# nanoporetech/isONclust2

Hardware: AMD Instinct MI355X
Metric: reads/s clustered (sahlin mode, k=11 w=15) (higher is better)
Workload: dtype u32

## Files before the change

### include/isonclust2_hip.h

```cpp
#ifndef ISONCLUST2_HIP_H
#define ISONCLUST2_HIP_H

#include <stddef.h>
#include <stdint.h>

#ifdef __cplusplus
extern "C" {
#endif

typedef struct ioc_ctx ioc_ctx;

typedef enum {
    IOC_OK = 0,
    IOC_ERR_ARG = -1,
    IOC_ERR_HIP = -2,
    IOC_ERR_STATE = -3,
    IOC_ERR_CAPACITY = -4,
    IOC_ERR_TABLE = -5,
    IOC_ERR_NO_DEVICE = -6,
    IOC_ERR_INPUT = -7
} ioc_status;

enum { IOC_MODE_SAHLIN = 0, IOC_MODE_FAST = 1, IOC_MODE_FURIOUS = 2, IOC_MODE_NONE = 3 };

typedef struct {
    int32_t k;
    int32_t w;
    int32_t min_shared;
    int32_t mode;
    double min_fraction;
    double mapped_threshold;
    double min_prob_no_hits;
    double aligned_threshold;
} ioc_params;

int ioc_ctx_create(int device, ioc_ctx** out);
void ioc_ctx_destroy(ioc_ctx* ctx);
int ioc_ctx_trim(ioc_ctx* ctx);
int ioc_ctx_prewarm(ioc_ctx* ctx, int32_t alignment_mode);
const char* ioc_last_error(const ioc_ctx* ctx);
int ioc_set_stream(ioc_ctx* ctx, void* hip_stream);
int ioc_synchronize(ioc_ctx* ctx);

int ioc_set_params(ioc_ctx* ctx, const ioc_params* p, const int32_t gap_limit[225]);

int ioc_queries_upload(ioc_ctx* ctx, int32_t n, const int64_t* off_fwd, const int64_t* off_rev,
                       const uint32_t* min_val, const uint32_t* min_pos, int64_t total,
                       const uint32_t* hpc_len, const uint8_t* err_cell, const uint32_t* min_total);
int ioc_queries_bind_device(ioc_ctx* ctx, int32_t n, const int64_t* d_off_fwd, const int64_t* d_off_rev,
                            const uint32_t* d_min_val, const uint32_t* d_min_pos, int64_t total,
                            const uint32_t* d_hpc_len, const uint8_t* d_err_cell,
                            const uint32_t* d_min_total, const int64_t* h_off_fwd,
                            const int64_t* h_off_rev);

int ioc_left_load(ioc_ctx* ctx, int32_t n_clusters, const uint8_t* cls_err_cell, int64_t n_keys,
                  const uint32_t* keys, const int64_t* offs, const uint32_t* postings);

int ioc_index_update(ioc_ctx* ctx, int32_t cls, const uint32_t* old_min, int64_t n_old, const uint32_t* new_min,
                     int64_t n_new, uint8_t new_err_cell);
int ioc_left_export(ioc_ctx* ctx, int64_t* n_keys, int64_t* n_postings, uint32_t* keys, int64_t* offs,
                    uint32_t* postings);

int ioc_index_build(ioc_ctx* ctx);
int ioc_score(ioc_ctx* ctx);
int ioc_resolve(ioc_ctx* ctx, int32_t* n_iter);
int ioc_get_decisions(ioc_ctx* ctx, int32_t* target, int8_t* strand, uint8_t* flags);
int ioc_get_cuts(ioc_ctx* ctx, int32_t* cut);
int ioc_force_decision(ioc_ctx* ctx, int32_t query, int32_t target, int32_t strand);
int ioc_clear_forced(ioc_ctx* ctx);
int ioc_set_aln_verdicts(ioc_ctx* ctx, const int32_t* target, const int8_t* strand);
#define IOC_TIE_SLOTS 16
int ioc_get_ties(ioc_ctx* ctx, uint32_t* count, uint32_t* keys);

int ioc_scored_candidates(ioc_ctx* ctx, int32_t q, int32_t cap, uint32_t* key, uint32_t* size);
int ioc_query_candidates(ioc_ctx* ctx, int32_t query, int32_t cap, int32_t* target, int8_t* strand,
                         uint32_t* size, uint32_t* first_index, uint32_t* total_mapped);

int ioc_index_export(ioc_ctx* ctx, int64_t* n_keys, int64_t* n_postings, uint32_t* keys,
                     int64_t* offs, uint32_t* postings);

int ioc_qual_scores(ioc_ctx* ctx, int32_t n, const int64_t* offs, const uint8_t* qual, int32_t k,
                    double* score, double* err_rate);
int ioc_extract_minimizers(ioc_ctx* ctx, int32_t n, const int64_t* offs, const uint8_t* seq,
                           const uint8_t* qual, int32_t k, int32_t w, uint32_t* hpc_len,
                           double* hpc_err, int64_t* off_fwd, int64_t* off_rev, int32_t* status);
int ioc_extracted_hpc_download(ioc_ctx* ctx, char* hpc_seq, char* hpc_qual, int64_t cap);
int ioc_extracted_download(ioc_ctx* ctx, uint32_t* min_val, uint32_t* min_pos, int64_t cap);
int ioc_queries_from_extracted(ioc_ctx* ctx, const uint8_t* keep, const uint8_t* err_cell,
                               const uint32_t* min_total);

typedef struct {
    float ms_build;
    float ms_score;
    float ms_resolve;
    int32_t resolve_iters;
    int32_t n_queries;
    int64_t n_minimizers;
    int64_t n_index_postings;
    int64_t n_candidates;
    int64_t n_mapped_evals;
    int64_t postings_traversed;
    float ms_align_fwd;
    float ms_align_trace;
    int64_t n_align_pairs;
    int64_t n_align_cells;
    int64_t n_align_refused;
    int32_t score_oob;
    int32_t score_oob_probe;
    int64_t align_arena_bytes;
    int32_t align_slices;
    int32_t align_version;
    int64_t n_align_cells_computed;
} ioc_timings;
int ioc_get_timings(ioc_ctx* ctx, ioc_timings* out);
int ioc_count_reference_postings(ioc_ctx* ctx, int64_t* n_postings);

int ioc_host_gap_limits(const char* table_path, int32_t k, int32_t w, double min_prob_no_hits,
                        int32_t* gap_limit, double* p_shared);
uint8_t ioc_host_err_cell(double err_rate);
uint32_t ioc_host_min_total(uint32_t hpc_len, double mapped_threshold);

int ioc_host_align(const char* query, int32_t qlen, const char* ref, int32_t rlen, int32_t match,
                   int32_t mismatch, int32_t gap_open, int32_t gap_extend, char* comp, int32_t comp_cap,
                   int32_t* score_out);
int ioc_host_align_ops(const char* query, int32_t qlen, const char* ref, int32_t rlen, int32_t match,
                       int32_t mismatch, int32_t gap_open, int32_t gap_extend, char* ops, int32_t ops_cap,
                       int32_t* score_out);
int64_t ioc_host_ops_to_cigar(const char* ops, int64_t len, char* out, int64_t cap);
int32_t ioc_host_gap_open(double e1_plus_e2);
double ioc_host_aln_ratio(const char* comp, int32_t comp_len, double e, uint32_t slen, uint32_t k);

typedef struct {
    int32_t query;
    int32_t ref;
    int32_t ref_revcomp;
    int32_t reserved;
    double e;
} ioc_aln_pair;
int ioc_align_set_pool(ioc_ctx* ctx, int32_t n_seqs, const char* seqs, const int64_t* offs);
int ioc_align_pairs(ioc_ctx* ctx, int32_t n_pairs, const ioc_aln_pair* pairs, int32_t k, int32_t match,
                    int32_t mismatch, int32_t gap_extend, int32_t* out_score, int64_t* out_windows,
                    double* out_ratio);
int64_t ioc_align_ops_bound(ioc_ctx* ctx, int32_t n_pairs, const ioc_aln_pair* pairs);
int ioc_align_pairs_ops(ioc_ctx* ctx, int32_t n_pairs, const ioc_aln_pair* pairs, int32_t k, int32_t match,
                        int32_t mismatch, int32_t gap_extend, int32_t* out_score, int64_t* out_windows,
                        double* out_ratio, char* out_ops, int64_t ops_cap, int64_t* ops_off);
int ioc_align_set_verdict_threshold(ioc_ctx* ctx, double aligned_threshold);

int64_t ioc_queries_generation(const ioc_ctx* ctx);
int64_t ioc_gather_records_device(ioc_ctx* ctx, int32_t n_idx, const int32_t* entries, uint32_t* d_out_min,
                                  uint32_t* d_out_pos, int64_t cap, int64_t* off_fwd, int64_t* off_rev);

typedef struct {
    int32_t n;
    const int64_t* off_fwd;
    const int64_t* off_rev;
    const uint32_t* min_val;
    const uint32_t* min_pos;
    int64_t total;
    const uint32_t* raw_len;
    const uint32_t* hpc_len;
    const double* score;
    const double* raw_err;
    const double* hpc_err;
    const uint8_t* state;
    double min_qual;
    const char* raw_seq;
    const int64_t* raw_off;
    const int32_t* n_members;
    int32_t depth;
    int32_t min_cls_size;
    const uint8_t* is_cluster;
    int32_t minimizers_on_device;
} ioc_batch_view;

typedef struct {
    int32_t n_clusters;
    const double* cls_hpc_err;
    int64_t n_keys;
    const uint32_t* keys;
    const int64_t* offs;
    const uint32_t* postings;
    const char* rep_seq;
    const int64_t* rep_off;
    const double* cls_raw_err;
} ioc_left_view;

typedef struct {
    int64_t n_clusters;
    int64_t n_joined;
    int64_t n_gated;
    int64_t n_tie_replays;
    int64_t n_aln_invoked;
    int32_t resolve_iters;
    int32_t aln_rounds;
    int64_t n_aln_pairs;
    int64_t n_aln_order_dep;
    int64_t n_cons_invoked;
    int64_t n_cons_restarts;
} ioc_cluster_stats;

int ioc_cluster_batch(ioc_ctx* ctx, const ioc_params* p, const char* table_path,
                      const ioc_batch_view* right, int32_t* out_cls, int8_t* out_strand,
                      ioc_cluster_stats* stats);
int ioc_cluster_merge(ioc_ctx* ctx, const ioc_params* p, const char* table_path, const ioc_left_view* left,
                      const ioc_batch_view* right, int32_t* out_cls, int8_t* out_strand,
                      ioc_cluster_stats* stats);
typedef struct {
    const char* raw_seq;
    int32_t raw_len;
    char raw_qual;
    double raw_err;
    double raw_score;
    const char* hpc_seq;
    int32_t hpc_len;
    double hpc_err;
    const uint32_t* fwd_min;
    const uint32_t* fwd_pos;
    int32_t n_fwd;
    const uint32_t* rev_min;
    const uint32_t* rev_pos;
    int32_t n_rev;
    int32_t entry;
} ioc_rep_record;
typedef struct {
    void* user;
    int (*create)(void* user, int side, int idx, const char* seq, int len);
    int (*size)(void* user, int side, int idx);
    int (*add)(void* user, int side, int idx, const char* seq, int len, unsigned weight);
    int (*consensus)(void* user, int side, int idx, char* out, int cap);
    int (*purge)(void* user, int side, int idx, const char* seq, int len, unsigned weight);
    void (*rep_changed)(void* user, int32_t cls, const ioc_rep_record* rec);
    const struct ioc_consensus_spec_ops* spec;
} ioc_consensus_ops;
typedef struct ioc_consensus_spec_ops {
    int (*create_tagged)(void* user, int side, int idx, const char* seq, int len, int tag);
    int (*add_tagged)(void* user, int side, int idx, const char* seq, int len, unsigned weight, int tag);
    int (*consensus_deferred)(void* user, int side, int idx, int tag);
    int (*flush)(void* user, int safe_tag);
    int (*collect)(void* user, int side, int idx, int tag, char* out, int cap);
    int (*rollback)(void* user, int first_tag);
    int (*commit)(void* user);
} ioc_consensus_spec_ops;
typedef struct {
    int32_t cons_min_size;
    int32_t cons_max_size;
    int32_t cons_period;
    int32_t left_depth;
    const int32_t* left_sizes;
} ioc_consensus_args;
int ioc_cluster_consensus(ioc_ctx* ctx, const ioc_params* p, const char* table_path, const ioc_left_view* left,
                          const ioc_batch_view* right, const ioc_consensus_args* args, const ioc_consensus_ops* ops,
                          int32_t* out_cls, int8_t* out_strand, ioc_cluster_stats* stats);

#define IOC_POA_LOCAL 0
#define IOC_POA_GLOBAL 1
#define IOC_POA_SEMI_GLOBAL 2
typedef struct ioc_poa ioc_poa;
int ioc_poa_create(ioc_ctx* ctx, int32_t m, int32_t n, int32_t g, int32_t e, int32_t q, int32_t c, ioc_poa** out);
int ioc_poa_create_mode(ioc_ctx* ctx, int32_t mode, int32_t m, int32_t n, int32_t g, int32_t e, int32_t q, int32_t c, ioc_poa** out);
void ioc_poa_destroy(ioc_poa* poa);
void ioc_poa_bind(ioc_poa* poa, ioc_consensus_ops* ops);
int ioc_poa_graph_export(ioc_poa* poa, int side, int idx, int32_t* n_nodes, int32_t* n_edges, char* bases, int32_t* rank,
                         int32_t* edge_from, int32_t* edge_to, int64_t* edge_w);
int ioc_poa_last_alignment(ioc_poa* poa, int32_t cap, int32_t* nodes, int32_t* pos, int32_t* score);
int64_t ioc_poa_graph_save(ioc_poa* poa, int side, int idx, uint8_t* out, int64_t cap);
int ioc_poa_graph_load(ioc_poa* poa, int side, int idx, const uint8_t* in, int64_t len);
int ioc_poa_graph_load_many(ioc_poa* poa, int side, int32_t count, const int32_t* idx, const uint8_t* const* in, const int64_t* len);

int ioc_cluster_resident(ioc_ctx* ctx, int32_t* out_cls, int8_t* out_strand, ioc_cluster_stats* stats);
int ioc_resident_set_sequences(ioc_ctx* ctx, const char* raw_seq, const int64_t* raw_off, const double* raw_err);

#define IOC_DIST_ID_BYTES 128
int ioc_dist_unique_id(uint8_t* id );
int ioc_dist_init(ioc_ctx* ctx, const uint8_t* id, int32_t rank, int32_t world);
int ioc_dist_shutdown(ioc_ctx* ctx);
int ioc_dist_info(const ioc_ctx* ctx, int32_t* rank, int32_t* world);
int ioc_dist_allgather_device(ioc_ctx* ctx, const void* d_send, void* d_recv, int64_t bytes_per_rank);
int ioc_dist_allgatherv_device(ioc_ctx* ctx, const void* d_send, void* d_recv, const int64_t* counts, const int64_t* displs,
                               int32_t esize);
int ioc_dist_allgather_i64(ioc_ctx* ctx, int64_t mine, int64_t* all );
int ioc_dist_allgatherv_host(ioc_ctx* ctx, const void* send, int64_t bytes, void* recv, int64_t* sizes);
int ioc_dist_allreduce_max(ioc_ctx* ctx, double* x);
int ioc_dist_barrier(ioc_ctx* ctx);
typedef struct {
    float ms_exchange_lists;
    double ms_merge;
    int64_t bytes_lists;
    int64_t bytes_records;
    int32_t sharded;
    int32_t exchanges;
} ioc_dist_merge_times;
#define IOC_XCHG_MAX_U8 0
#define IOC_XCHG_MIN_U32 1
#define IOC_XCHG_SUM_I32 2
typedef int (*ioc_exchange_fn)(void* user, void* d_buf, int64_t count, int32_t kind, void* hip_stream);
int ioc_set_shard(ioc_ctx* ctx, int32_t world, int32_t rank, ioc_exchange_fn fn, void* user);
int32_t ioc_shard_exchanges(const ioc_ctx* ctx);
int64_t ioc_shard_aligned_pairs(const ioc_ctx* ctx);
int ioc_dist_exchange(ioc_ctx* ctx, void* d_buf, int64_t count, int32_t kind);
int ioc_dist_set_shard(ioc_ctx* ctx, int32_t on);

int ioc_dist_merge(ioc_ctx* ctx, const ioc_params* p, const char* table_path, const ioc_batch_view* reps, int32_t min_cls_size,
                   int64_t out_cap, int32_t* out_cls, int8_t* out_strand, int64_t* out_counts, ioc_cluster_stats* stats,
                   ioc_dist_merge_times* times);

#ifdef __cplusplus
}
#endif
#endif
```

### isonclust2_amd/_lib.py

```python
import ctypes as C
import os

HERE = os.path.dirname(os.path.abspath(__file__))
LIB_PATH = os.environ.get("IOC_LIB", os.path.join(HERE, "libisonclust2_hip.so"))
TABLE_PATH = os.path.join(HERE, "data", "pmin_shared.bin")


class IocError(RuntimeError):
    def __init__(self, code, msg):
        super().__init__(f"isonclust2_hip error {code}: {msg}")
        self.code = code


class Params(C.Structure):
    _fields_ = [("k", C.c_int32), ("w", C.c_int32), ("min_shared", C.c_int32), ("mode", C.c_int32),
                ("min_fraction", C.c_double), ("mapped_threshold", C.c_double),
                ("min_prob_no_hits", C.c_double), ("aligned_threshold", C.c_double)]


class BatchView(C.Structure):
    _fields_ = [("n", C.c_int32), ("off_fwd", C.POINTER(C.c_int64)), ("off_rev", C.POINTER(C.c_int64)),
                ("min_val", C.POINTER(C.c_uint32)), ("min_pos", C.POINTER(C.c_uint32)),
                ("total", C.c_int64), ("raw_len", C.POINTER(C.c_uint32)),
                ("hpc_len", C.POINTER(C.c_uint32)), ("score", C.POINTER(C.c_double)),
                ("raw_err", C.POINTER(C.c_double)), ("hpc_err", C.POINTER(C.c_double)),
                ("state", C.POINTER(C.c_uint8)), ("min_qual", C.c_double),
                ("raw_seq", C.c_char_p), ("raw_off", C.POINTER(C.c_int64)),
                ("n_members", C.POINTER(C.c_int32)), ("depth", C.c_int32), ("min_cls_size", C.c_int32),
                ("is_cluster", C.POINTER(C.c_uint8)), ("minimizers_on_device", C.c_int32)]


class LeftView(C.Structure):
    _fields_ = [("n_clusters", C.c_int32), ("cls_hpc_err", C.POINTER(C.c_double)), ("n_keys", C.c_int64),
                ("keys", C.POINTER(C.c_uint32)), ("offs", C.POINTER(C.c_int64)),
                ("postings", C.POINTER(C.c_uint32)), ("rep_seq", C.c_char_p),
                ("rep_off", C.POINTER(C.c_int64)), ("cls_raw_err", C.POINTER(C.c_double))]


class ClusterStats(C.Structure):
    _fields_ = [("n_clusters", C.c_int64), ("n_joined", C.c_int64), ("n_gated", C.c_int64),
                ("n_tie_replays", C.c_int64), ("n_aln_invoked", C.c_int64),
                ("resolve_iters", C.c_int32), ("aln_rounds", C.c_int32), ("n_aln_pairs", C.c_int64),
                ("n_aln_order_dep", C.c_int64), ("n_cons_invoked", C.c_int64), ("n_cons_restarts", C.c_int64)]

    def as_dict(self):
        return {n: int(getattr(self, n)) for n, _ in self._fields_}


class RepRecord(C.Structure):
    _fields_ = [("raw_seq", C.POINTER(C.c_char)), ("raw_len", C.c_int32), ("raw_qual", C.c_char), ("raw_err", C.c_double),
                ("raw_score", C.c_double), ("hpc_seq", C.POINTER(C.c_char)), ("hpc_len", C.c_int32), ("hpc_err", C.c_double),
                ("fwd_min", C.POINTER(C.c_uint32)), ("fwd_pos", C.POINTER(C.c_uint32)), ("n_fwd", C.c_int32),
                ("rev_min", C.POINTER(C.c_uint32)), ("rev_pos", C.POINTER(C.c_uint32)), ("n_rev", C.c_int32),
                ("entry", C.c_int32)]


CONS_CREATE = C.CFUNCTYPE(C.c_int, C.c_void_p, C.c_int, C.c_int, C.POINTER(C.c_char), C.c_int)
CONS_SIZE = C.CFUNCTYPE(C.c_int, C.c_void_p, C.c_int, C.c_int)
CONS_ADD = C.CFUNCTYPE(C.c_int, C.c_void_p, C.c_int, C.c_int, C.POINTER(C.c_char), C.c_int, C.c_uint)
CONS_CONSENSUS = C.CFUNCTYPE(C.c_int, C.c_void_p, C.c_int, C.c_int, C.POINTER(C.c_char), C.c_int)
CONS_PURGE = C.CFUNCTYPE(C.c_int, C.c_void_p, C.c_int, C.c_int, C.POINTER(C.c_char), C.c_int, C.c_uint)
CONS_REP_CHANGED = C.CFUNCTYPE(None, C.c_void_p, C.c_int32, C.POINTER(RepRecord))


class ConsensusOps(C.Structure):
    _fields_ = [("user", C.c_void_p), ("create", CONS_CREATE), ("size", CONS_SIZE), ("add", CONS_ADD),
                ("consensus", CONS_CONSENSUS), ("purge", CONS_PURGE), ("rep_changed", CONS_REP_CHANGED),
                ("spec", C.c_void_p)]


class ConsensusArgs(C.Structure):
    _fields_ = [("cons_min_size", C.c_int32), ("cons_max_size", C.c_int32), ("cons_period", C.c_int32),
                ("left_depth", C.c_int32), ("left_sizes", C.POINTER(C.c_int32))]


class AlnPair(C.Structure):
    _fields_ = [("query", C.c_int32), ("ref", C.c_int32), ("ref_revcomp", C.c_int32), ("reserved", C.c_int32),
                ("e", C.c_double)]


class DistMergeTimes(C.Structure):
    _fields_ = [("ms_exchange_lists", C.c_float), ("ms_merge", C.c_double), ("bytes_lists", C.c_int64), ("bytes_records", C.c_int64),
                ("sharded", C.c_int32), ("exchanges", C.c_int32)]


EXCHANGE_FN = C.CFUNCTYPE(C.c_int, C.c_void_p, C.c_void_p, C.c_int64, C.c_int32, C.c_void_p)
XCHG_MAX_U8, XCHG_MIN_U32, XCHG_SUM_I32 = 0, 1, 2


class Timings(C.Structure):
    _fields_ = [("ms_build", C.c_float), ("ms_score", C.c_float), ("ms_resolve", C.c_float),
                ("resolve_iters", C.c_int32), ("n_queries", C.c_int32), ("n_minimizers", C.c_int64),
                ("n_index_postings", C.c_int64), ("n_candidates", C.c_int64),
                ("n_mapped_evals", C.c_int64), ("postings_traversed", C.c_int64),
                ("ms_align_fwd", C.c_float), ("ms_align_trace", C.c_float), ("n_align_pairs", C.c_int64),
                ("n_align_cells", C.c_int64),
                ("n_align_refused", C.c_int64), ("score_oob", C.c_int32), ("score_oob_probe", C.c_int32),
                ("align_arena_bytes", C.c_int64), ("align_slices", C.c_int32), ("align_version", C.c_int32),
                ("n_align_cells_computed", C.c_int64)]

    def as_dict(self):
        return {n: getattr(self, n) for n, _ in self._fields_}


SYMBOLS = [
    "ioc_ctx_create", "ioc_ctx_destroy", "ioc_ctx_trim", "ioc_ctx_prewarm", "ioc_last_error", "ioc_set_stream", "ioc_synchronize",
    "ioc_set_params", "ioc_queries_upload", "ioc_queries_bind_device", "ioc_left_load",
    "ioc_index_build", "ioc_score", "ioc_resolve", "ioc_get_decisions", "ioc_get_cuts", "ioc_force_decision",
    "ioc_clear_forced", "ioc_query_candidates", "ioc_index_export", "ioc_qual_scores",
    "ioc_extract_minimizers", "ioc_extracted_download", "ioc_extracted_hpc_download", "ioc_queries_from_extracted",
    "ioc_get_timings", "ioc_count_reference_postings", "ioc_host_gap_limits", "ioc_host_err_cell", "ioc_host_min_total",
    "ioc_cluster_batch", "ioc_cluster_merge", "ioc_cluster_resident", "ioc_host_align", "ioc_host_gap_open",
    "ioc_host_aln_ratio", "ioc_host_align_ops", "ioc_host_ops_to_cigar", "ioc_align_set_pool", "ioc_align_pairs", "ioc_align_ops_bound",
    "ioc_align_pairs_ops", "ioc_set_aln_verdicts", "ioc_get_ties", "ioc_resident_set_sequences",
    "ioc_index_update", "ioc_left_export", "ioc_cluster_consensus",
    "ioc_poa_create", "ioc_poa_create_mode", "ioc_poa_destroy", "ioc_poa_bind", "ioc_poa_graph_export", "ioc_poa_last_alignment",
    "ioc_poa_graph_save", "ioc_poa_graph_load", "ioc_poa_graph_load_many", "ioc_gather_records_device", "ioc_queries_generation", "ioc_scored_candidates",
    "ioc_dist_unique_id", "ioc_dist_init", "ioc_dist_shutdown", "ioc_dist_info", "ioc_dist_allgather_device",
    "ioc_dist_allgatherv_device", "ioc_dist_allgather_i64", "ioc_dist_allgatherv_host", "ioc_dist_allreduce_max",
    "ioc_dist_barrier", "ioc_dist_merge", "ioc_set_shard", "ioc_shard_exchanges", "ioc_shard_aligned_pairs", "ioc_dist_exchange", "ioc_dist_set_shard", "ioc_align_set_verdict_threshold",
]

_lib = None


def load():
    global _lib
    if _lib is not None:
        return _lib
    if not os.path.exists(LIB_PATH):
        raise IocError(-100, f"{LIB_PATH} is missing: run `python -c 'import __graft_entry__ as g; g.build()'` "
                             "(hipcc --offload-arch=gfx950); there is no CPU fallback")
    try:
        import torch
    except Exception:
        pass
    L = C.CDLL(LIB_PATH)
    vp, i32, i64 = C.c_void_p, C.c_int32, C.c_int64
    pi64, pu32, pu8 = C.POINTER(C.c_int64), C.POINTER(C.c_uint32), C.POINTER(C.c_uint8)
    pi32, pi8, pd = C.POINTER(C.c_int32), C.POINTER(C.c_int8), C.POINTER(C.c_double)
    L.ioc_ctx_create.argtypes = [i32, C.POINTER(vp)]
    L.ioc_ctx_destroy.argtypes = [vp]
    L.ioc_ctx_destroy.restype = None
    L.ioc_last_error.argtypes = [vp]
    L.ioc_last_error.restype = C.c_char_p
    L.ioc_set_stream.argtypes = [vp, vp]
    L.ioc_synchronize.argtypes = [vp]
    L.ioc_set_params.argtypes = [vp, C.POINTER(Params), pi32]
    L.ioc_queries_upload.argtypes = [vp, i32, pi64, pi64, pu32, pu32, i64, pu32, pu8, pu32]
    L.ioc_queries_bind_device.argtypes = [vp, i32, vp, vp, vp, vp, i64, vp, vp, vp, pi64, pi64]
    L.ioc_gather_records_device.argtypes = [vp, i32, pi32, vp, vp, i64, pi64, pi64]
    L.ioc_gather_records_device.restype = i64
    L.ioc_scored_candidates.argtypes = [vp, i32, i32, pu32, pu32]
    L.ioc_queries_generation.argtypes = [vp]
    L.ioc_queries_generation.restype = i64
    L.ioc_left_load.argtypes = [vp, i32, pu8, i64, pu32, pi64, pu32]
    L.ioc_index_update.argtypes = [vp, i32, pu32, i64, pu32, i64, C.c_uint8]
    L.ioc_left_export.argtypes = [vp, pi64, pi64, pu32, pi64, pu32]
    L.ioc_index_build.argtypes = [vp]
    L.ioc_score.argtypes = [vp]
    L.ioc_resolve.argtypes = [vp, pi32]
    L.ioc_get_decisions.argtypes = [vp, pi32, pi8, pu8]
    L.ioc_get_cuts.argtypes = [vp, pi32]
    L.ioc_force_decision.argtypes = [vp, i32, i32, i32]
    L.ioc_clear_forced.argtypes = [vp]
    L.ioc_query_candidates.argtypes = [vp, i32, i32, pi32, pi8, pu32, pu32, pu32]
    L.ioc_index_export.argtypes = [vp, pi64, pi64, pu32, pi64, pu32]
    L.ioc_qual_scores.argtypes = [vp, i32, pi64, pu8, i32, pd, pd]
    L.ioc_extract_minimizers.argtypes = [vp, i32, pi64, pu8, pu8, i32, i32, pu32, pd, pi64, pi64, pi32]
    L.ioc_extracted_download.argtypes = [vp, pu32, pu32, i64]
    L.ioc_extracted_hpc_download.argtypes = [vp, C.c_char_p, C.c_char_p, i64]
    L.ioc_queries_from_extracted.argtypes = [vp, pu8, pu8, pu32]
    L.ioc_get_timings.argtypes = [vp, C.POINTER(Timings)]
    L.ioc_count_reference_postings.argtypes = [vp, pi64]
    L.ioc_host_gap_limits.argtypes = [C.c_char_p, i32, i32, C.c_double, pi32, pd]
    L.ioc_host_err_cell.argtypes = [C.c_double]
    L.ioc_host_err_cell.restype = C.c_uint8
    L.ioc_host_min_total.argtypes = [C.c_uint32, C.c_double]
    L.ioc_host_min_total.restype = C.c_uint32
    L.ioc_cluster_batch.argtypes = [vp, C.POINTER(Params), C.c_char_p, C.POINTER(BatchView), pi32, pi8,
                                    C.POINTER(ClusterStats)]
    L.ioc_cluster_merge.argtypes = [vp, C.POINTER(Params), C.c_char_p, C.POINTER(LeftView), C.POINTER(BatchView),
                                    pi32, pi8, C.POINTER(ClusterStats)]
    L.ioc_cluster_consensus.argtypes = [vp, C.POINTER(Params), C.c_char_p, C.POINTER(LeftView), C.POINTER(BatchView),
                                        C.POINTER(ConsensusArgs), C.POINTER(ConsensusOps), pi32, pi8, C.POINTER(ClusterStats)]
    L.ioc_poa_create.argtypes = [vp, i32, i32, i32, i32, i32, i32, C.POINTER(vp)]
    L.ioc_poa_create_mode.argtypes = [vp, i32, i32, i32, i32, i32, i32, i32, C.POINTER(vp)]
    L.ioc_poa_destroy.argtypes = [vp]
    L.ioc_poa_destroy.restype = None
    L.ioc_poa_bind.argtypes = [vp, C.POINTER(ConsensusOps)]
    L.ioc_poa_bind.restype = None
    L.ioc_poa_graph_export.argtypes = [vp, C.c_int, C.c_int, pi32, pi32, C.c_char_p, pi32, pi32, pi32, pi64]
    L.ioc_poa_last_alignment.argtypes = [vp, i32, pi32, pi32, pi32]
    L.ioc_poa_graph_save.argtypes = [vp, C.c_int, C.c_int, pu8, i64]
    L.ioc_poa_graph_save.restype = C.c_int64
    L.ioc_poa_graph_load.argtypes = [vp, C.c_int, C.c_int, pu8, i64]
    L.ioc_poa_graph_load_many.argtypes = [vp, C.c_int, C.c_int32, C.POINTER(C.c_int32), C.POINTER(pu8), C.POINTER(i64)]
    L.ioc_host_align.argtypes = [C.c_char_p, i32, C.c_char_p, i32, i32, i32, i32, i32, C.c_char_p, i32, pi32]
    L.ioc_host_align_ops.argtypes = [C.c_char_p, i32, C.c_char_p, i32, i32, i32, i32, i32, C.c_char_p, i32, pi32]
    L.ioc_host_ops_to_cigar.argtypes = [C.c_char_p, i64, C.c_char_p, i64]
    L.ioc_host_ops_to_cigar.restype = C.c_int64
    L.ioc_host_gap_open.argtypes = [C.c_double]
    L.ioc_host_aln_ratio.argtypes = [C.c_char_p, i32, C.c_double, C.c_uint32, C.c_uint32]
    L.ioc_host_aln_ratio.restype = C.c_double
    L.ioc_cluster_resident.argtypes = [vp, pi32, pi8, C.POINTER(ClusterStats)]
    L.ioc_resident_set_sequences.argtypes = [vp, C.c_char_p, pi64, pd]
    L.ioc_set_aln_verdicts.argtypes = [vp, pi32, pi8]
    L.ioc_get_ties.argtypes = [vp, C.POINTER(C.c_uint32), C.POINTER(C.c_uint32)]
    L.ioc_align_set_pool.argtypes = [vp, i32, C.c_char_p, C.POINTER(C.c_int64)]
    L.ioc_align_pairs.argtypes = [vp, i32, C.POINTER(AlnPair), i32, i32, i32, i32, pi32, C.POINTER(C.c_int64),
                                  C.POINTER(C.c_double)]
    L.ioc_align_ops_bound.argtypes = [vp, i32, C.POINTER(AlnPair)]
    L.ioc_align_ops_bound.restype = C.c_int64
    L.ioc_align_pairs_ops.argtypes = [vp, i32, C.POINTER(AlnPair), i32, i32, i32, i32, pi32, C.POINTER(C.c_int64),
                                      C.POINTER(C.c_double), C.c_void_p, i64, C.POINTER(C.c_int64)]
    L.ioc_dist_unique_id.argtypes = [pu8]
    L.ioc_dist_init.argtypes = [vp, pu8, i32, i32]
    L.ioc_dist_shutdown.argtypes = [vp]
    L.ioc_dist_info.argtypes = [vp, pi32, pi32]
    L.ioc_dist_allgather_device.argtypes = [vp, vp, vp, i64]
    L.ioc_dist_allgatherv_device.argtypes = [vp, vp, vp, pi64, pi64, i32]
    L.ioc_dist_allgather_i64.argtypes = [vp, i64, pi64]
    L.ioc_dist_allgatherv_host.argtypes = [vp, vp, i64, vp, pi64]
    L.ioc_dist_allreduce_max.argtypes = [vp, pd]
    L.ioc_dist_barrier.argtypes = [vp]
    L.ioc_dist_merge.argtypes = [vp, C.POINTER(Params), C.c_char_p, C.POINTER(BatchView), i32, i64, pi32, pi8, pi64,
                                 C.POINTER(ClusterStats), C.POINTER(DistMergeTimes)]
    L.ioc_set_shard.argtypes = [vp, i32, i32, EXCHANGE_FN, vp]
    L.ioc_shard_exchanges.argtypes = [vp]
    L.ioc_shard_aligned_pairs.argtypes = [vp]
    L.ioc_shard_aligned_pairs.restype = C.c_int64
    L.ioc_dist_exchange.argtypes = [vp, vp, i64, i32]
    L.ioc_dist_set_shard.argtypes = [vp, i32]
    L.ioc_align_set_verdict_threshold.argtypes = [vp, C.c_double]
    _lib = L
    return L
```

### isonclust2_amd/csrc/ioc_align_gpu.hip

```cpp
#include <hip/hip_runtime.h>

#include <algorithm>
#include <chrono>
#include <cmath>
#include <cstdint>
#include <cstring>
#include <numeric>
#include <string>
#include <type_traits>
#include <vector>

#include "ioc_internal.h"

namespace {

constexpr int ALN_C = 8;
constexpr int ALN_MAXW = 8;
constexpr int ALN_NEG = INT32_MIN / 4;
constexpr uint32_t ALN_LEN_SHIFT = 26;

struct AlnPairDev {
    uint32_t q_off, n;
    uint32_t r_off, m;
    int32_t gap_open, ilimit;
// ... 743 lines not shown
                if (lane == 0) __hip_atomic_store(&xflag[uint64_t(wave) * nstrips + p], 1u, __ATOMIC_RELAXED, __HIP_MEMORY_SCOPE_AGENT);
            }
        }
        if (rounds > 1 || nwaves > 1) __syncthreads();
    }
    __syncthreads();

    if (xbad && lane == 0) atomicOr(X.err, 1u);
    const bool reducer = cross ? (grp + 1u == X.groups && wv == 0) : wave == 0;
    if (live && reducer) {
        if (cross) {
            uint32_t okf = 1;
            if (lane == 0) {
                for (uint32_t b2 = 0; b2 < nwaves && okf; ++b2) {
                    if (min(n, b2 * tpb * TILE) >= n) break;
                    uint32_t seen = 0;
                    for (uint32_t it = 0; it < (1u << 22); ++it) {
                        seen = __hip_atomic_load(&xflag[uint64_t(b2) * nstrips + (nstrips - 1u)], __ATOMIC_RELAXED, __HIP_MEMORY_SCOPE_AGENT);
                        if (seen) break;
                        __builtin_amdgcn_s_sleep(8);
                    }
                    if (!seen) okf = 0;
                }
                if (!okf) atomicOr(X.err, 1u);
            }
            __builtin_amdgcn_fence(__ATOMIC_ACQUIRE, "agent");
        }
        int br = 0;
        uint32_t bj = 0;
        for (uint32_t e = lane; e < nstrips * 64u; e += 64) {
            {
                const uint32_t ep = e >> 6, el = e & 63u;
                const uint32_t cpl = (narrow_last && ep + 1u == nstrips) ? 8u : uint32_t(FW_C);
                if (uint64_t(ep) * strip_cols + el * cpl >= m) continue;
            }
            const int2 x = mylrow[e];
            if (x.x > br || (x.x == br && uint32_t(x.y) < bj)) {
                br = x.x;
                bj = uint32_t(x.y);
            }
        }
        for (int o = 32; o > 0; o >>= 1) {
            const int s = __shfl_xor(br, o);
            const uint32_t j = __shfl_xor(bj, o);
            if (s > br || (s == br && j < bj)) {
                br = s;
                bj = j;
            }
        }
        if (lane == 0) {
            int fin = ALN_NEG;
            uint32_t bi = 0, bjj = m;
            for (uint32_t b2 = 0; b2 < nwaves; ++b2) {
                if (min(n, b2 * tpb * TILE) >= n) break;
                const int2 bb = cross ? X.best[uint64_t(pslot - X.first_pair) * nwaves + b2] : int2{s_best[slot * wpp + b2][0], s_best[slot * wpp + b2][1]};
                if (bb.x > fin) {
                    fin = bb.x;
                    bi = uint32_t(bb.y);
                }
            }
            if (br > fin) {
                fin = br;
                bi = n;
                bjj = bj;
            }
            ends[pid] = int4{fin, int(bi), int(bjj), 0};
        }
    }
}

struct WinStat {
    uint32_t wb = 0, pushed = 0, cnt = 0;
    __device__ __forceinline__ void push(uint32_t bit, uint32_t kmask, uint32_t k, int il)
    {
        wb = ((wb << 1) | bit) & kmask;
        ++pushed;
        if (pushed > k && int(__popc(wb)) >= il) ++cnt;
    }
    __device__ __forceinline__ void push_run(unsigned long long bits, uint32_t m, uint32_t kmask, uint32_t k, int il, uint32_t lane)
    {
        const unsigned long long upto = __brevll(bits << (63u - lane));
        const unsigned long long old = lane + 1u < 64u ? (unsigned long long)wb << (lane + 1u) : 0ull;
        const uint32_t win = uint32_t(old | upto) & kmask;
        const bool hit = lane < m && pushed + lane + 1u > k && int(__popc(win)) >= il;
        cnt += uint32_t(__popcll(__ballot(hit)));
        wb = uint32_t(__builtin_amdgcn_readlane(int(win), int(m - 1u)));
        pushed += m;
    }
    __device__ void blanks(uint32_t g, uint32_t kmask, uint32_t k, int il)
    {
        const uint32_t t = g < k ? g : k;
        for (uint32_t x = 0; x < t; ++x) push(0u, kmask, k, il);
        if (g > t) {
            const uint32_t rest = g - t;
            const uint32_t first_counted = pushed >= k ? 0u : k - pushed;
            pushed += rest;
            if (il <= 0 && rest > first_counted) cnt += rest - first_counted;
        }
    }
};

struct AlnOpsDev {
    uint8_t* buf;
    const uint64_t* end;
    uint32_t* len;
};

struct NoOpsDev {};
template <bool EMIT>
struct OpsOut {
    using Dev = NoOpsDev;
    __device__ __forceinline__ void begin(Dev, uint32_t, uint32_t) {}
    __device__ __forceinline__ void run(unsigned long long, uint32_t, uint32_t) {}
    __device__ __forceinline__ void step(uint8_t, uint32_t) {}
    __device__ __forceinline__ void fill(uint8_t, uint32_t, uint32_t) {}
    __device__ __forceinline__ void end(Dev, uint32_t, uint32_t) {}
    __device__ __forceinline__ void none(Dev, uint32_t) {}
};
template <>
struct OpsOut<true> {
    using Dev = AlnOpsDev;
    uint8_t* cur = nullptr;
    uint8_t* lo = nullptr;
    __device__ __forceinline__ void begin(const Dev& od, uint32_t pid, uint32_t room)
    {
        cur = od.buf + od.end[pid];
        lo = cur - room;
    }
    __device__ __forceinline__ void run(unsigned long long bits, uint32_t m, uint32_t lane)
    {
        if (lane < m && cur - 1 - lane >= lo) cur[-1 - int(lane)] = (bits >> lane) & 1ull ? uint8_t('=') : uint8_t('X');
        cur -= m;
    }
    __device__ __forceinline__ void step(uint8_t op, uint32_t lane)
    {
        if (lane == 0 && cur > lo) cur[-1] = op;
        cur -= 1;
    }
    __device__ __forceinline__ void fill(uint8_t op, uint32_t g, uint32_t lane)
    {
        const uint64_t room = uint64_t(cur > lo ? cur - lo : 0);
        for (uint32_t x = lane; x < g && x < room; x += 64) cur[-1 - int64_t(x)] = op;
        cur -= g;
    }
    __device__ __forceinline__ void end(const Dev& od, uint32_t pid, uint32_t lane)
    {
        if (lane == 0) od.len[pid] = cur >= lo ? uint32_t((od.buf + od.end[pid]) - cur) : 0xFFFFFFFFu;
    }
    __device__ __forceinline__ void none(const Dev& od, uint32_t pid) { od.len[pid] = 0u; }
};

constexpr int TR_WAVES = 4;
__device__ __forceinline__ void tr_wave_sync()
{
    __builtin_amdgcn_fence(__ATOMIC_RELEASE, "workgroup");
    __builtin_amdgcn_wave_barrier();
    __builtin_amdgcn_fence(__ATOMIC_ACQUIRE, "workgroup");
}

#define ALN_TRACE_KERNEL k_align_trace
#define ALN_TRACE_EMIT 0
#include "ioc_align_trace.inc"
#undef ALN_TRACE_KERNEL
#undef ALN_TRACE_EMIT
#define ALN_TRACE_KERNEL k_align_trace_ops
#define ALN_TRACE_EMIT 1
#include "ioc_align_trace.inc"
#undef ALN_TRACE_KERNEL
#undef ALN_TRACE_EMIT

__global__ void __launch_bounds__(256)
k_seq_flags(const uint8_t* __restrict__ pool, const int64_t* __restrict__ offs, uint8_t* __restrict__ flags)
{
    __shared__ uint32_t s_any;
    if (threadIdx.x == 0) s_any = 0;
    __syncthreads();
    const int64_t a = offs[blockIdx.x], b = offs[blockIdx.x + 1];
    uint32_t any = 0;
    for (int64_t i = a + threadIdx.x; i < b; i += 256) {
        const uint8_t ch = pool[i];
        any |= (ch != 'A' && ch != 'C' && ch != 'G' && ch != 'T') ? 1u : 0u;
    }
    if (any) s_any = 1;
    __syncthreads();
    if (threadIdx.x == 0) flags[blockIdx.x] = uint8_t(s_any);
}

int reserve(ioc_ctx* c, DevBuf& b, size_t bytes)
{
    if (bytes == 0) bytes = 16;
    if (b.cap >= bytes) return IOC_OK;
    if (b.p) {
        if (hipStreamSynchronize(c->stream) != hipSuccess) return ioc_fail(c, IOC_ERR_HIP, "stream synchronize failed");
        (void)hipFree(b.p);
        b.p = nullptr;
        b.cap = 0;
    }
    const size_t want = bytes + bytes / 8 + 256;
    const hipError_t e = hipMalloc(&b.p, want);
    if (e != hipSuccess) {
        b.p = nullptr;
        return ioc_fail(c, IOC_ERR_CAPACITY, "hipMalloc(" + std::to_string(want) + " B) failed: " + hipGetErrorString(e));
    }
    b.cap = want;
    ioc_poison(b.p, want);
    return IOC_OK;
}

#define ACHK(c, call)                                                                             \
    do {                                                                                          \
        hipError_t e__ = (call);                                                                  \
        if (e__ != hipSuccess)                                                                    \
            return ioc_fail((c), IOC_ERR_HIP, std::string(#call) + ": " + hipGetErrorString(e__)); \
    } while (0)

#include "ioc_align_v2.inc"


struct EventSet {
    std::vector<hipEvent_t> v;
    ~EventSet()
    {
        for (auto& e : v)
            if (e) (void)hipEventDestroy(e);
    }
};

void add_elapsed(ioc_ctx* c, const std::vector<hipEvent_t>& evs, size_t used)
{
    for (size_t x = 0; x + 2 < used && x + 2 < evs.size(); x += 3) {
        float a = 0, b = 0;
        if (hipEventElapsedTime(&a, evs[x], evs[x + 1]) == hipSuccess) c->tm.ms_align_fwd += a;
        if (hipEventElapsedTime(&b, evs[x + 1], evs[x + 2]) == hipSuccess) c->tm.ms_align_trace += b;
    }
}

int compute_units(const ioc_ctx* c)
{
    int n_cu = 256;
    (void)hipDeviceGetAttribute(&n_cu, hipDeviceAttributeMultiprocessorCount, c->device);
    return n_cu < 1 ? 256 : n_cu;
}

int ck_budget(ioc_ctx* c, uint64_t* budget)
{
    size_t free_b = 0, total_b = 0;
    ACHK(c, hipMemGetInfo(&free_b, &total_b));
    *budget = uint64_t(free_b + c->a_ck.cap) / 2;
    if (const char* e = getenv("IOC_ALIGN_CK_BUDGET_MB")) *budget = uint64_t(atoll(e)) << 20;
    return IOC_OK;
}


struct AlnOpsHost {
    uint8_t* buf;
    const int64_t* base;
    int64_t* len;
    double* ms_copy;
    int64_t* copied;
};

struct OpsRun {
    const AlnOpsHost* host;
    const uint32_t* back;
    std::vector<uint64_t> end;
    AlnOpsDev dev{};
    std::vector<uint8_t> stage;
    std::vector<uint32_t> len;
};

int ops_reserve(ioc_ctx* c, OpsRun& o, uint64_t max_slice_bytes)
{
    const size_t np = o.end.size(), tab = (np * 12 + 15) & ~size_t(15);
    const int r = reserve(c, c->a_ops, tab + size_t(max_slice_bytes));
    if (r != IOC_OK) return r;
    uint8_t* p = static_cast<uint8_t*>(c->a_ops.p);
    o.dev = AlnOpsDev{p + tab, reinterpret_cast<const uint64_t*>(p), reinterpret_cast<uint32_t*>(p + np * 8)};
    ACHK(c, hipMemcpyAsync(p, o.end.data(), np * 8, hipMemcpyHostToDevice, c->stream));
    return IOC_OK;
}

int ops_fetch(ioc_ctx* c, OpsRun& o, const std::vector<AlnPairDev>& dp, const uint32_t* ord, uint32_t cnt, uint64_t bytes)
{
    ACHK(c, hipStreamSynchronize(c->stream));
    const auto t0 = std::chrono::steady_clock::now();
    o.len.resize(dp.size());
    if (o.stage.size() < bytes) o.stage.resize(size_t(bytes));
    ACHK(c, hipMemcpy(o.len.data(), o.dev.len, dp.size() * 4, hipMemcpyDeviceToHost));
    ACHK(c, hipMemcpy(o.stage.data(), o.dev.buf, size_t(bytes), hipMemcpyDeviceToHost));
    for (uint32_t x = 0; x < cnt; ++x) {
        const uint32_t pid = ord[x], i = o.back[pid];
        const uint64_t L = o.len[pid];
        if (L == 0 || L > uint64_t(dp[pid].n) + dp[pid].m || L > o.end[pid]) continue;
        memcpy(o.host->buf + o.host->base[i], o.stage.data() + (o.end[pid] - L), size_t(L));
        o.host->len[i] = int64_t(L);
    }
    *o.host->ms_copy += std::chrono::duration<double, std::milli>(std::chrono::steady_clock::now() - t0).count();
    *o.host->copied += int64_t(bytes);
    return IOC_OK;
}


constexpr int P16_GUARD = 28000;

struct CorridorModel {
    const ioc_ctx* c;
    AlnParams P;
    double frac;
    bool fixed;
    bool fit_ok;
    double pair_frac(const AlnPairDev& d) const
    {
        if (fixed || !(P.match > 0)) return frac;
        const double e = double(d.e_sum);
        if (!(e > 0.0) || !(e < 1.0)) return frac;
        const int go = std::max(2, std::min(5, d.gap_open));
        double rho = double(P.match) - e * (double(P.match - P.mismatch) / 3.0 + 2.0 / 3.0 * double(go + P.match)), margin = 0.02;
        const ioc_ctx::CorridorFit& f = c->aln_fit[go - 2];
        if (fit_ok && f.n >= 64.0 && e >= f.e_lo - 0.02 && e <= f.e_hi + 0.02) {
            const double me = f.se / f.n, mr = f.sr / f.n, vee = f.see / f.n - me * me, ver = f.ser / f.n - me * mr, vrr = f.srr / f.n - mr * mr;
            const double slope = vee > 1e-9 ? ver / vee : 0.0;
            const double sd = std::sqrt(std::max(0.0, vrr - slope * ver));
            rho = mr + slope * (e - me) - 4.5 * std::max(sd, 0.004);
            margin = 0.003;
        }
        return std::max(0.03, std::min(0.45, 1.0 - rho / double(P.match) + margin));
    }
};

CorridorModel corridor_model(const ioc_ctx* c, const AlnParams& P, bool corridor)
{
    CorridorModel m{c, P, corridor ? 0.2 : 0.0, false, false};
    if (const char* e = getenv("IOC_ALIGN_CORRIDOR")) {
        m.frac = corridor ? std::max(0.0, std::min(1.0, atof(e))) : 0.0;
        m.fixed = true;
    }
    m.fit_ok = c->aln_fit_sig[0] == P.match && c->aln_fit_sig[1] == P.mismatch && c->aln_fit_sig[2] == P.gap_extend && !getenv("IOC_ALIGN_CORRIDOR_NO_FIT");
    return m;
}

uint32_t band_target(uint32_t ncouples, uint32_t few_limit, int occ, int n_cu)
{
    const uint32_t waves = uint32_t(occ) * uint32_t(n_cu) * uint32_t(V2_WAVES);
    uint32_t want = std::max(12u, std::min(uint32_t(V2_MAX_BANDS), (waves + ncouples - 1u) / std::max(1u, ncouples)));
    if (few_limit && ncouples <= few_limit) want = std::min(want, 17u);
    return want;
}

struct V2Plan {
    uint32_t cnt = 0, np = 0, ncouples = 0;
    std::vector<V2Couple> cps;
    std::vector<V2PairCk> pck;
    std::vector<V2PairEnd> pend;
    std::vector<uint64_t> cwords;
    uint32_t lrow_total = 0, best_total = 0, max_strips = 1;
    uint64_t tiles_skipped = 0, tiles_all = 0;
    std::vector<std::pair<uint32_t, uint32_t>> slices;
    uint64_t arena_words = 0, prof_total = 0;
    std::vector<std::vector<V2Item>> items;
    std::vector<uint32_t> n_probe;
    uint32_t max_items = 0, max_flags = 0, max_pairs = 0;
};

void plan_bands(V2Couple& cp, uint32_t ncoarse, uint32_t want_bands, bool corridor)
{
    const uint32_t wb = (corridor && ncoarse >= 16u) ? std::max(want_bands, 17u) : want_bands;
    const uint32_t reg = std::max<uint32_t>(want_bands > 16u ? 1u : 2u, (ncoarse + wb - 1) / wb);
    std::vector<uint32_t> hts;
    for (uint32_t left = ncoarse; left;) {
        const uint32_t hgt = std::min(reg, left);
        hts.push_back(hgt);
        left -= hgt;
    }
    while (hts.size() > size_t(V2_MAX_BANDS)) {
        const size_t mid = hts.size() / 2;
        hts[mid - 1] += hts[mid];
        hts.erase(hts.begin() + long(mid));
    }
    cp.nbands = uint32_t(hts.size());
    cp.tpb = reg;
    uint32_t acc = 0;
    for (uint32_t b = 0; b <= uint32_t(V2_MAX_BANDS); ++b) {
        cp.bstart[b] = uint16_t(std::min<uint32_t>(acc, 0xFFFFu));
        if (b < cp.nbands) acc += hts[b];
    }
}

uint32_t plan_corridor(V2Couple& cp, const std::vector<AlnPairDev>& dp, const CorridorModel& cm, uint32_t nmax, uint32_t mmax, int32_t cert[2])
{
    const AlnParams& P = cm.P;
    constexpr uint32_t probe_rows = 1024;
    cp.corridor = 0;
    for (uint32_t b = 0; b < uint32_t(V2_MAX_BANDS); ++b) {
        cp.plo[b] = 0;
        cp.phi[b] = uint16_t(std::min<uint32_t>(65535u, cp.nstrips - 1u));
    }
    const uint32_t strip_cols = 64u * FW_C;
    double frac = 0.0;
    for (int h = 0; h < 2; ++h)
        if (cp.pid[h] != 0xFFFFFFFFu) frac = std::max(frac, cm.pair_frac(dp[cp.pid[h]]));
    if (cm.frac <= 0.0) frac = 0.0;
    const uint32_t B = uint32_t(frac * double(std::max(nmax, mmax)));
    cp.b0 = B;
    int64_t beff = INT64_MAX;
    uint32_t skipped = 0;
    uint16_t lo[V2_MAX_BANDS], hi[V2_MAX_BANDS];
    bool fits = cm.frac > 0.0 && B >= strip_cols && cp.nstrips <= 65535u && cp.nbands <= uint32_t(V2_MAX_BANDS) && P.match > 0 && P.mismatch <= P.match &&
                P.gap_extend >= 0;
    for (int h = 0; fits && h < 2; ++h)
        if (cp.pid[h] != 0xFFFFFFFFu) fits = dp[cp.pid[h]].gap_open >= 0;
    for (uint32_t b = 0; fits && b < cp.nbands; ++b) {
        const uint32_t r0 = uint32_t(cp.bstart[b]) * uint32_t(CK2), r1 = std::min(nmax, uint32_t(cp.bstart[b + 1u]) * uint32_t(CK2));
        const uint32_t c_lo = r0 > B ? r0 - B : 0u, c_hi = std::min<uint64_t>(mmax, uint64_t(r1) + B);
        if (c_hi <= c_lo) {
            fits = false;
            break;
        }
        lo[b] = uint16_t(c_lo / strip_cols);
        hi[b] = uint16_t((c_hi - 1u) / strip_cols);
        skipped += lo[b] + (cp.nstrips - 1u - hi[b]);
        if (lo[b] > 0) beff = std::min<int64_t>(beff, int64_t(r0) - int64_t(lo[b]) * strip_cols);
        if ((uint64_t(hi[b]) + 1u) * strip_cols < mmax) beff = std::min<int64_t>(beff, int64_t(hi[b] + 1u) * strip_cols - int64_t(r1));
    }
    uint32_t pb = 0, ps = 0;
    if (fits) {
        while (pb + 1u < cp.nbands && uint32_t(cp.bstart[pb + 1u]) * uint32_t(CK2) < probe_rows) ++pb;
        const uint32_t R = uint32_t(cp.bstart[pb + 1u]) * uint32_t(CK2);
        ps = (R - 1u) / strip_cols;
        fits = pb + 1u < cp.nbands && R >= probe_rows;
        for (uint32_t b = 0; fits && b <= pb; ++b) fits = lo[b] == 0 && hi[b] >= ps;
        for (int h = 0; fits && h < 2; ++h)
            if (cp.pid[h] != 0xFFFFFFFFu) fits = dp[cp.pid[h]].n >= R && dp[cp.pid[h]].m > ps * strip_cols;
    }
    cp.probe_band = uint16_t(pb);
    cp.probe_strip = uint16_t(ps);
    if (fits && skipped * 5u >= cp.nbands * cp.nstrips && beff > 0 && beff < INT64_MAX) {
        cp.corridor = 1;
        for (uint32_t b = 0; b < cp.nbands; ++b) {
            cp.plo[b] = lo[b];
            cp.phi[b] = hi[b];
        }
    }
    for (int h = 0; h < 2; ++h) {
        cert[h] = INT32_MIN;
        if (cp.pid[h] == 0xFFFFFFFFu || !cp.corridor) continue;
        const AlnPairDev& d = dp[cp.pid[h]];
        cert[h] = int32_t(std::min<int64_t>(INT32_MAX, int64_t(P.match) * std::max<int64_t>(0, int64_t(std::max(d.n, d.m)) - beff - 1)));
    }
    return cp.corridor ? skipped : 0u;
}

uint64_t couple_words(V2Couple& cp, uint32_t nmax, uint32_t mmax)
{
    auto up4 = [](uint64_t x) { return (x + 3u) & ~uint64_t(3); };
    cp.mpad = uint32_t((uint64_t(mmax) + 15u) & ~uint64_t(15));
    cp.nq = (nmax + 3u) / 4u;
    const uint64_t ncr = (nmax - 1u) / CK2, ncc = (mmax - 1u) / CK2;
    uint64_t w = 0;
    cp.rdat = w;
    w += up4(ncr * 2u * cp.mpad);
    cp.rbase = w;
    w += up4(ncr * (cp.mpad / 16u) * 2u);
    cp.cdat = w;
    w += up4(ncc * uint64_t(cp.nq) * 8u);
    cp.cbase = w;
    w += up4(ncc * uint64_t(cp.nq) * 2u);
    return w;
}

void plan_couples(V2Plan& pl, const std::vector<AlnPairDev>& dp, const uint32_t* order, const CorridorModel& cm, uint32_t want_bands)
{
    pl.cps.resize(pl.ncouples);
    pl.pck.resize(pl.np);
    pl.pend.resize(pl.np);
    pl.cwords.resize(pl.ncouples);
    for (uint32_t k2 = 0; k2 < pl.ncouples; ++k2) {
        V2Couple& cp = pl.cps[k2];
        cp.pid[0] = order[2u * k2];
        cp.pid[1] = 2u * k2 + 1u < pl.cnt ? order[2u * k2 + 1u] : 0xFFFFFFFFu;
        uint32_t nmax = 0, mmax = 0;
        for (int h = 0; h < 2; ++h)
            if (cp.pid[h] != 0xFFFFFFFFu) {
                nmax = std::max(nmax, dp[cp.pid[h]].n);
                mmax = std::max(mmax, dp[cp.pid[h]].m);
            }
        cp.nstrips = (mmax + 64u * FW_C - 1) / (64u * FW_C);
        plan_bands(cp, (nmax + CK2 - 1) / CK2, want_bands, cm.frac > 0.0);
        int32_t cert[2];
        pl.tiles_skipped += plan_corridor(cp, dp, cm, nmax, mmax, cert);
        pl.tiles_all += uint64_t(cp.nbands) * cp.nstrips;
        pl.cwords[k2] = couple_words(cp, nmax, mmax);
        cp.prof = 0;
        pl.max_strips = std::max(pl.max_strips, cp.nstrips);
        for (int h = 0; h < 2; ++h) {
            cp.lrow0[h] = pl.lrow_total;
            cp.best0[h] = pl.best_total;
            if (cp.pid[h] == 0xFFFFFFFFu) continue;
            const AlnPairDev& d = dp[cp.pid[h]];
            const uint32_t nstr = (d.m + 64u * FW_C - 1) / (64u * FW_C);
            pl.pend[cp.pid[h]] = V2PairEnd{pl.lrow_total, pl.best_total, cp.nbands, k2, cert[h]};
            pl.lrow_total += nstr * 64u;
            pl.best_total += cp.nbands;
        }
    }
}

void slice_couples(V2Plan& pl, uint64_t budget, const std::vector<uint64_t>& cops)
{
    for (uint32_t first = 0; first < pl.ncouples;) {
        uint64_t used = 0;
        uint32_t k2 = first;
        uint64_t prof_used = 0;
        uint64_t ops_used = 0;
        while (k2 < pl.ncouples) {
            const uint64_t prof_k = uint64_t(pl.cps[k2].nstrips) * 2u * 5u * 64u, ops_k = cops.empty() ? 0u : cops[k2];
            if (k2 != first && (used + pl.cwords[k2]) * 4ull + (prof_used + prof_k) * sizeof(uint4) + ops_used + ops_k > budget) break;
            V2Couple& cp = pl.cps[k2];
            cp.prof = prof_used;
            prof_used += prof_k;
            cp.rdat += used;
            cp.rbase += used;
            cp.cdat += used;
            cp.cbase += used;
            for (int h = 0; h < 2; ++h)
                if (cp.pid[h] != 0xFFFFFFFFu) pl.pck[cp.pid[h]] = V2PairCk{cp.rdat, cp.rbase, cp.cdat, cp.cbase, cp.mpad, cp.nq, uint32_t(h), k2};
            used += pl.cwords[k2];
            ops_used += ops_k;
            ++k2;
        }
        pl.arena_words = std::max(pl.arena_words, used);
        pl.prof_total = std::max(pl.prof_total, prof_used);
        pl.slices.emplace_back(first, k2 - first);
        first = k2;
    }
}

void tile_lists(V2Plan& pl)
{
    pl.items.resize(pl.slices.size());
    pl.n_probe.assign(pl.slices.size(), 0);
    for (size_t si = 0; si < pl.slices.size(); ++si) {
        const uint32_t k_lo = pl.slices[si].first, k_hi = pl.slices[si].first + pl.slices[si].second;
        uint32_t nf = 0;
        auto& it = pl.items[si];
        uint32_t maxdiag = 0;
        size_t total_items = 0;
        for (uint32_t k2 = k_lo; k2 < k_hi; ++k2) {
            V2Couple& cp = pl.cps[k2];
            cp.flag0 = nf;
            nf += cp.nbands * cp.nstrips;
            total_items += size_t(cp.nbands) * cp.nstrips;
            maxdiag = std::max(maxdiag, cp.nbands + cp.nstrips - 2u);
        }
        it.reserve(total_items + 64u * pl.slices[si].second);
        for (uint32_t dg = 0; dg <= maxdiag; ++dg) {
            bool any = false;
            for (uint32_t k2 = k_lo; k2 < k_hi; ++k2) {
                const V2Couple& cp = pl.cps[k2];
                if (!cp.corridor || dg > uint32_t(cp.probe_band) + cp.probe_strip) continue;
                any = true;
                const uint32_t b_lo = dg >= uint32_t(cp.probe_strip) + 1u ? dg - cp.probe_strip : 0u, b_hi = std::min<uint32_t>(dg, cp.probe_band);
                for (uint32_t b = b_lo; b <= b_hi; ++b) it.push_back(V2Item{k2, uint16_t(b), uint16_t(dg - b)});
            }
            if (!any && dg > 64u) break;
        }
        pl.n_probe[si] = uint32_t(it.size());
        for (uint32_t dg = 0; dg <= maxdiag; ++dg)
            for (uint32_t k2 = k_lo; k2 < k_hi; ++k2) {
                const V2Couple& cp = pl.cps[k2];
                if (dg > cp.nbands + cp.nstrips - 2u) continue;
                const uint32_t b_lo = dg >= cp.nstrips ? dg - cp.nstrips + 1u : 0u, b_hi = std::min(dg, cp.nbands - 1u);
                for (uint32_t b = b_lo; b <= b_hi; ++b) it.push_back(V2Item{k2, uint16_t(b), uint16_t(dg - b)});
            }
        pl.max_items = std::max<uint32_t>(pl.max_items, uint32_t(it.size()));
        pl.max_flags = std::max(pl.max_flags, nf);
        pl.max_pairs = std::max(pl.max_pairs, std::min(pl.cnt, 2u * k_hi) - 2u * k_lo);
    }
}

struct V2Opts {
    int n_cu, occ, guard;
    uint32_t few_limit;
    uint32_t deadline;
    unsigned long long deadline_cycles;
    uint32_t help_wgs;
    bool side_help;
};

struct V2Dev {
    V2Couple* cps;
    V2PairCk* pck;
    V2PairEnd* pend;
    V2Item* items;
    int2 *lrow, *best;
    uint32_t* ctl;
    size_t ctl_words;
    V2Scratch *scratch, *hscratch;
    uint32_t* resume;
    uint32_t* park;
    uint32_t* early;
    uint32_t* gate;
    uint32_t* split;
    size_t resume_words;
};

int v2_tables(ioc_ctx* c, const V2Plan& pl, uint32_t help_wgs, V2Dev& t)
{
    hipStream_t s = c->stream;
    int r;
    const uint32_t ncouples = pl.ncouples, np = pl.np;
    const size_t tab_bytes = size_t(ncouples) * sizeof(V2Couple) + size_t(np) * (sizeof(V2PairCk) + sizeof(V2PairEnd)) + size_t(pl.max_items) * sizeof(V2Item) + 256;
    if ((r = reserve(c, c->a_cko, tab_bytes)) != IOC_OK) return r;
    uint8_t* tb = static_cast<uint8_t*>(c->a_cko.p);
    t.cps = reinterpret_cast<V2Couple*>(tb);
    t.pck = reinterpret_cast<V2PairCk*>(tb + size_t(ncouples) * sizeof(V2Couple));
    t.pend = reinterpret_cast<V2PairEnd*>(reinterpret_cast<uint8_t*>(t.pck) + size_t(np) * sizeof(V2PairCk));
    t.items = reinterpret_cast<V2Item*>(reinterpret_cast<uint8_t*>(t.pend) + size_t(np) * sizeof(V2PairEnd));
    ACHK(c, hipMemcpyAsync(t.cps, pl.cps.data(), size_t(ncouples) * sizeof(V2Couple), hipMemcpyHostToDevice, s));
    ACHK(c, hipMemcpyAsync(t.pck, pl.pck.data(), size_t(np) * sizeof(V2PairCk), hipMemcpyHostToDevice, s));
    ACHK(c, hipMemcpyAsync(t.pend, pl.pend.data(), size_t(np) * sizeof(V2PairEnd), hipMemcpyHostToDevice, s));
    if ((r = reserve(c, c->a_prof, size_t(pl.prof_total) * sizeof(uint4) + 256)) != IOC_OK) return r;
    if ((r = reserve(c, c->a_ends2, size_t(np) * sizeof(int4))) != IOC_OK) return r;
    if ((r = reserve(c, c->a_lrow, (size_t(pl.lrow_total) + pl.best_total + 16) * sizeof(int2))) != IOC_OK) return r;
    t.lrow = static_cast<int2*>(c->a_lrow.p);
    t.best = t.lrow + pl.lrow_total;
    t.ctl_words = ((16 + 2 * size_t(pl.max_flags) + np + 1) & ~size_t(1)) + 2;
    if ((r = reserve(c, c->a_xflags, t.ctl_words * 4)) != IOC_OK) return r;
    t.ctl = static_cast<uint32_t*>(c->a_xflags.p);
    const size_t n_scratch = size_t(pl.max_pairs) + size_t(help_wgs) * V2_NHELP * V2_HBUF;
    t.resume_words = size_t(np) * V2_RESUME_WORDS + 2u * (size_t(pl.max_pairs) + 1u) + 4u + size_t(np) * V2_SPLIT_WORDS;
    if ((r = reserve(c, c->a_bnd, n_scratch * sizeof(V2Scratch) + t.resume_words * 4)) != IOC_OK) return r;
    t.scratch = static_cast<V2Scratch*>(c->a_bnd.p);
    t.hscratch = t.scratch + pl.max_pairs;
    t.resume = reinterpret_cast<uint32_t*>(t.scratch + n_scratch);
    t.park = t.resume + size_t(np) * V2_RESUME_WORDS;
    t.early = t.park + size_t(pl.max_pairs) + 1u;
    t.gate = t.early + size_t(pl.max_pairs) + 1u;
    t.split = t.gate + 4u;
    return IOC_OK;
}

uint32_t v2_per_cu(const V2Plan& pl, size_t si, const V2Opts& o, bool few_couples)
{
    if (few_couples) return uint32_t(o.occ);
    uint64_t tiles = 0;
    uint32_t diags = 1;
    for (uint32_t k2 = pl.slices[si].first; k2 < pl.slices[si].first + pl.slices[si].second; ++k2) {
        const V2Couple& cp = pl.cps[k2];
        for (uint32_t b = 0; b < cp.nbands; ++b) tiles += uint32_t(cp.phi[b]) - uint32_t(cp.plo[b]) + 1u;
        diags = std::max(diags, cp.nbands + cp.nstrips - 1u);
    }
    const double x = double(tiles) / double(diags) / double(uint32_t(o.n_cu) * uint32_t(V2_WAVES));
    return x < 1.0 ? 1u : x < 2.75 ? std::min(2u, uint32_t(o.occ)) : uint32_t(o.occ);
}

int v2_slice(ioc_ctx* c, const V2Plan& pl, const V2Dev& t, size_t si, const V2Opts& o, const AlnParams& P, const uint32_t* d_order,
             int32_t* d_score, uint32_t* d_count, const hipEvent_t* ev, uint32_t* xe, const AlnOpsDev* od)
{
    hipStream_t s = c->stream;
    const uint32_t k_first = pl.slices[si].first, n_couples = pl.slices[si].second;
    const uint32_t first_pair = 2u * k_first, n_pairs = std::min(pl.cnt, 2u * (k_first + n_couples)) - first_pair;
    const uint32_t n_items = uint32_t(pl.items[si].size()), n_probe = pl.n_probe[si];
    const AlnPairDev* d_pairs = static_cast<const AlnPairDev*>(c->a_pairs.p);
    const uint8_t* d_pool = static_cast<const uint8_t*>(c->a_pool.p);
    uint32_t* d_ctl = t.ctl;
    const bool few_couples = n_couples <= o.few_limit;
    const uint32_t prog_every = few_couples ? 1u : 0u;
    ACHK(c, hipMemcpyAsync(t.items, pl.items[si].data(), size_t(n_items) * sizeof(V2Item), hipMemcpyHostToDevice, s));
    ACHK(c, hipMemcpyAsync(t.cps + k_first, pl.cps.data() + k_first, size_t(n_couples) * sizeof(V2Couple), hipMemcpyHostToDevice, s));
    hipLaunchKernelGGL(k_fwd2_prof, dim3(n_couples, pl.max_strips), dim3(128), 0, s, d_pairs, t.cps + k_first, d_pool, P, static_cast<uint4*>(c->a_prof.p));
    ACHK(c, hipGetLastError());
    ACHK(c, hipMemsetAsync(d_ctl, 0, t.ctl_words * 4, s));
    ACHK(c, hipMemsetAsync(t.resume, 0, t.resume_words * 4, s));
    if (pl.tiles_skipped)
        ACHK(c, hipMemsetAsync(t.lrow, 0x80, (size_t(pl.lrow_total) + pl.best_total) * sizeof(int2), s));
    if (getenv("IOC_ALIGN_V2_FAKE_TIMEOUT")) {
        const uint32_t one = 1;
        ACHK(c, hipMemcpyAsync(d_ctl + 1, &one, 4, hipMemcpyHostToDevice, s));
    }
    ACHK(c, hipEventRecord(ev[0], s));
    auto fwd = [&](decltype(&k_fwd2) kernel, uint32_t n_wg, const V2Item* items, uint32_t n) {
        hipLaunchKernelGGL(kernel, dim3(n_wg), dim3(64 * V2_WAVES), 0, s, d_pairs, t.cps, items, n, d_ctl, d_ctl + 16, d_ctl + 1, d_pool, P,
                           static_cast<uint32_t*>(c->a_ck.p), t.lrow, t.best, d_ctl + 16 + 2 * pl.max_flags, o.guard, static_cast<const uint4*>(c->a_prof.p),
                           reinterpret_cast<unsigned long long*>(d_ctl + t.ctl_words - 2), few_couples ? d_ctl + 16 + pl.max_flags : static_cast<uint32_t*>(nullptr),
                           prog_every);
    };
    if (n_probe) {
        fwd(k_fwd2, std::max(1u, std::min(uint32_t(o.occ) * uint32_t(o.n_cu), (n_probe + V2_WAVES - 1) / V2_WAVES)), t.items, n_probe);
        ACHK(c, hipGetLastError());
        hipLaunchKernelGGL(k_fwd2_probe, dim3(n_couples), dim3(64), 0, s, d_pairs, t.cps + k_first, t.pend, static_cast<const uint32_t*>(c->a_ck.p), P);
        ACHK(c, hipGetLastError());
        ACHK(c, hipMemsetAsync(d_ctl, 0, 4, s));
    }
    const uint32_t n_main = n_items - n_probe, per_cu = v2_per_cu(pl, si, o, few_couples);
    const uint32_t n_wg = std::max(1u, std::min(per_cu * uint32_t(o.n_cu), (n_main + V2_WAVES - 1) / V2_WAVES));
    fwd((per_cu <= 2 && !getenv("IOC_ALIGN_V2_NO_W2")) ? k_fwd2_w2 : k_fwd2, n_wg, t.items + n_probe, n_main);
    ACHK(c, hipGetLastError());
    const uint32_t n_help = std::min<uint32_t>(n_pairs, o.help_wgs);
    hipLaunchKernelGGL(k_fwd2_ends, dim3(n_pairs), dim3(64), 0, s, d_pairs, t.cps, d_order + first_pair, n_pairs, t.pend, t.lrow, t.best,
                       d_ctl + 16 + 2 * pl.max_flags, static_cast<int4*>(c->a_ends2.p), t.resume, t.early, o.side_help ? int(P.match) : 0, n_help);
    ACHK(c, hipGetLastError());
    ACHK(c, hipEventRecord(ev[1], s));
    auto help = [&](hipStream_t hs, uint32_t* list, uint32_t which, uint32_t* gate) {
        if (od)
            hipLaunchKernelGGL(k_trace2_help_ops, dim3(n_help), dim3(64 * V2_HWAVES), 0, hs, d_pairs, d_order + first_pair, d_pool, P,
                               static_cast<const uint32_t*>(c->a_ck.p), t.cps, t.pck, static_cast<const int4*>(c->a_ends2.p), t.scratch, t.hscratch,
                               t.resume, list, t.split, d_score, d_count, n_pairs, which, gate, *od);
        else
            hipLaunchKernelGGL(k_trace2_help, dim3(n_help), dim3(64 * V2_HWAVES), 0, hs, d_pairs, d_order + first_pair, d_pool, P,
                               static_cast<const uint32_t*>(c->a_ck.p), t.cps, t.pck, static_cast<const int4*>(c->a_ends2.p), t.scratch, t.hscratch,
                               t.resume, list, t.split, d_score, d_count, n_pairs, which, gate);
    };
    if (o.side_help) {
        ACHK(c, hipEventRecord(c->ev_side[0], s));
        ACHK(c, hipStreamWaitEvent(c->side_stream, c->ev_side[0], 0));
        help(c->side_stream, t.early, 2u, t.gate);
        ACHK(c, hipGetLastError());
        ACHK(c, hipEventRecord(c->ev_side[1], c->side_stream));
        hipLaunchKernelGGL(k_trace2_gate, dim3(1), dim3(1), 0, s, t.early, t.gate, n_help);
        ACHK(c, hipGetLastError());
    }
    if (od)
        hipLaunchKernelGGL(k_trace2_ops, dim3((n_pairs + TR_WAVES - 1) / TR_WAVES), dim3(64 * TR_WAVES), 0, s, d_pairs, d_order + first_pair, d_pool, P,
                           static_cast<const uint32_t*>(c->a_ck.p), t.cps, t.pck, static_cast<const int4*>(c->a_ends2.p), t.scratch, t.resume, t.park,
                           t.split, d_score, d_count, n_pairs, o.deadline, o.deadline_cycles, *od);
    else
        hipLaunchKernelGGL(k_trace2, dim3((n_pairs + TR_WAVES - 1) / TR_WAVES), dim3(64 * TR_WAVES), 0, s, d_pairs, d_order + first_pair, d_pool, P,
                           static_cast<const uint32_t*>(c->a_ck.p), t.cps, t.pck, static_cast<const int4*>(c->a_ends2.p), t.scratch, t.resume, t.park,
                           t.split, d_score, d_count, n_pairs, o.deadline, o.deadline_cycles);
    ACHK(c, hipGetLastError());
    if (o.side_help) ACHK(c, hipStreamWaitEvent(s, c->ev_side[1], 0));
    if (o.deadline) {
        help(s, t.park, 1u, nullptr);
        ACHK(c, hipGetLastError());
    }
    ACHK(c, hipEventRecord(ev[2], s));
    unsigned long long cells_done = 0;
    ACHK(c, hipMemcpyAsync(xe, d_ctl + 1, 4, hipMemcpyDeviceToHost, s));
    ACHK(c, hipMemcpyAsync(&cells_done, d_ctl + t.ctl_words - 2, 8, hipMemcpyDeviceToHost, s));
    ACHK(c, hipStreamSynchronize(s));
    c->tm.n_align_cells_computed += int64_t(cells_done);
    return IOC_OK;
}

int v2_report(ioc_ctx* c, const std::vector<AlnPairDev>& dp, const uint32_t* order, const V2Plan& pl, const V2Dev& t, size_t si, uint32_t deadline)
{
    const bool rates = getenv("IOC_V2_TRACE_RATES") != nullptr, times = getenv("IOC_V2_TRACE_TIMES") != nullptr;
    if (!rates && !times) return IOC_OK;
    const uint32_t np = pl.np, first_pair = 2u * pl.slices[si].first;
    const uint32_t n_pairs = std::min(pl.cnt, 2u * (pl.slices[si].first + pl.slices[si].second)) - first_pair;
    std::vector<int4> he(np);
    ACHK(c, hipMemcpy(he.data(), c->a_ends2.p, size_t(np) * sizeof(int4), hipMemcpyDeviceToHost));
    if (rates)
        for (uint32_t x = 0; x < n_pairs; ++x) {
            const uint32_t pid = order[first_pair + x];
            const AlnPairDev& d = dp[pid];
            fprintf(stderr, "[rate] e %.5f n %u m %u score %d per_base %.5f go %d flags %d corridor %u\n", double(d.e_sum), d.n, d.m, he[pid].x,
                    double(he[pid].x) / double(std::max(d.n, d.m)), d.gap_open, he[pid].w, pl.cps[pl.pend[pid].couple].corridor);
        }
    if (!times) return IOC_OK;
    std::vector<uint32_t> rw(size_t(np) * V2_RESUME_WORDS);
    ACHK(c, hipMemcpy(rw.data(), t.resume, rw.size() * 4, hipMemcpyDeviceToHost));
    std::vector<uint32_t> ids(n_pairs);
    for (uint32_t x = 0; x < n_pairs; ++x) ids[x] = order[first_pair + x];
    auto rec = [&](uint32_t pid, uint32_t w) { return rw[size_t(pid) * V2_RESUME_WORDS + w]; };
    auto cost = [&](uint32_t pid) { return (double(rec(pid, 8)) + double(rec(pid, 12))) * 256.0; };
    std::sort(ids.begin(), ids.end(), [&](uint32_t a, uint32_t b) { return cost(a) > cost(b); });
    double sum = 0;
    uint32_t parked = 0;
    for (uint32_t pid : ids) {
        sum += cost(pid);
        parked += rec(pid, 6) ? 1u : 0u;
    }
    fprintf(stderr, "[ioc] k_trace2: %u pairs, %u walks went on in the second launch (deadline %u blocks); mean %.3e cycles (s_memtime), slowest first:\n", n_pairs, parked,
            deadline, sum / n_pairs);
    auto line = [&](const char* tag, uint32_t pid) {
        const AlnPairDev& d = dp[pid];
        fprintf(stderr, "[ioc]   %s pair %u: %.3e + %.3e cycles, n %u m %u, blocks %u (%u on the diagonal) + %u (%u by helpers), tiles %u + %u, gap steps %u, windows %u\n", tag, pid,
                double(rec(pid, 8)) * 256.0, double(rec(pid, 12)) * 256.0, d.n, d.m, rec(pid, 9) & 0xFFFFu, rec(pid, 9) >> 16, rec(pid, 13) & 0xFFFFu, rec(pid, 13) >> 16,
                rec(pid, 10), rec(pid, 14), rec(pid, 11), rec(pid, 15));
    };
    {
        double pk_max = -1e9, un_min = 1e9, pk_sum = 0, un_sum = 0;
        uint32_t npk = 0, nun = 0;
        std::vector<double> pks, uns;
        for (uint32_t pid : ids) {
            const AlnPairDev& d = dp[pid];
            const double q = double(he[pid].x) / double(std::max(1u, std::min(d.n, d.m)));
            if (rec(pid, 6)) {
                pk_max = std::max(pk_max, q), pk_sum += q, ++npk;
                pks.push_back(q);
            } else {
                un_min = std::min(un_min, q), un_sum += q, ++nun;
                uns.push_back(q);
            }
        }
        std::sort(pks.begin(), pks.end());
        std::sort(uns.begin(), uns.end());
        auto qt = [](const std::vector<double>& v, double f) { return v.empty() ? 0.0 : v[std::min(v.size() - 1, size_t(f * double(v.size())))]; };
        fprintf(stderr, "[ioc]   forward score / shorter length: parked walks (%u) mean %.3f, 50 %% %.3f, 90 %% %.3f, 99 %% %.3f, max %.3f | others (%u) min %.3f, 1 %% %.3f, 10 %% %.3f, mean %.3f\n", npk,
                npk ? pk_sum / npk : 0.0, qt(pks, 0.5), qt(pks, 0.9), qt(pks, 0.99), pk_max, nun, un_min, qt(uns, 0.01), qt(uns, 0.1), nun ? un_sum / nun : 0.0);
    }
    for (uint32_t x = 0; x < std::min(n_pairs, 10u); ++x) line("", ids[x]);
    for (uint32_t qx : {n_pairs / 4u, n_pairs / 2u, 3u * n_pairs / 4u}) line("rank", ids[qx]);
    std::vector<uint32_t> sw(size_t(np) * V2_SPLIT_WORDS);
    ACHK(c, hipMemcpy(sw.data(), t.split, sw.size() * 4, hipMemcpyDeviceToHost));
    for (uint32_t l = 0; l < 2u; ++l) {
        auto cyc = [&](uint32_t pid) { return double(rec(pid, l ? 12 : 8)) * 256.0; };
        auto spl = [&](uint32_t pid, uint32_t w) { return sw[size_t(pid) * V2_SPLIT_WORDS + l * (V2_SPLIT_WORDS / 2u) + w]; };
        std::vector<uint32_t> in;
        for (uint32_t pid : ids)
            if (rec(pid, l ? 12 : 8)) in.push_back(pid);
        std::sort(in.begin(), in.end(), [&](uint32_t a, uint32_t b) { return cyc(a) > cyc(b); });
        double tot[8] = {};
        for (uint32_t pid : in) {
            tot[0] += cyc(pid);
            for (uint32_t w = 0; w < 3u; ++w) tot[1 + w] += double(spl(pid, w)) * 256.0;
            tot[4] += double(spl(pid, 3) & 0xFFFFu);
            tot[5] += double(spl(pid, 4));
            tot[6] += double(spl(pid, 5));
            tot[7] += double(spl(pid, 6));
        }
        const double nn = double(std::max<size_t>(1, in.size()));
        fprintf(stderr, "[ioc] split of %s: %zu walks; mean %.3e cycles: blocks %.1f %%, tile recomputation %.1f %%, walk loop %.1f %%; %.1f cycles per tile step; "
                        "blocks of <= 64 columns: %.2f per walk, %.1f %% of the block steps recomputed by walkers\n",
                l ? "k_trace2_help" : "k_trace2", in.size(), tot[0] / nn, 100.0 * tot[1] / std::max(1.0, tot[0]), 100.0 * tot[2] / std::max(1.0, tot[0]),
                100.0 * tot[3] / std::max(1.0, tot[0]), tot[2] / std::max(1.0, tot[7]), tot[4] / nn, 100.0 * tot[6] / std::max(1.0, tot[5]));
        for (size_t x = 0; x < std::min<size_t>(in.size(), 10); ++x) {
            const uint32_t pid = in[x];
            const uint32_t nb = l ? rec(pid, 13) & 0xFFFFu : rec(pid, 9) & 0xFFFFu;
            fprintf(stderr, "[ioc]   split pair %u: %.3e cycles: blocks %.3e, tiles %.3e, walk %.3e; blocks %u (<= 64 columns %u, <= 64 rows %u), own block steps %u (%u in thin), tiles %u, tile steps %u\n",
                    pid, cyc(pid), double(spl(pid, 0)) * 256.0, double(spl(pid, 1)) * 256.0, double(spl(pid, 2)) * 256.0, nb, spl(pid, 3) & 0xFFFFu, spl(pid, 3) >> 16,
                    spl(pid, 4), spl(pid, 5), rec(pid, l ? 14 : 10), spl(pid, 6));
        }
    }
    return IOC_OK;
}

int align_v2_run(ioc_ctx* c, const std::vector<AlnPairDev>& dp, const uint32_t* order, uint32_t cnt, const uint32_t* d_order,
                 const AlnParams& P, int32_t* d_score, uint32_t* d_count, bool corridor, bool* fell_back, OpsRun* ops)
{
    *fell_back = false;
    if (cnt == 0) return IOC_OK;
    int r;
    const auto t_plan0 = std::chrono::steady_clock::now();
    V2Opts o{};
    o.n_cu = compute_units(c);
    uint64_t budget = 0;
    if ((r = ck_budget(c, &budget)) != IOC_OK) return r;
    o.guard = P16_GUARD;
    if (const char* e = getenv("IOC_ALIGN_V2_GUARD")) o.guard = std::max(1, std::min(P16_GUARD, atoi(e)));
    o.few_limit = 128;
    if (const char* e = getenv("IOC_ALIGN_V2_FEW")) o.few_limit = uint32_t(std::max(0, atoi(e)));
    if (hipOccupancyMaxActiveBlocksPerMultiprocessor(&o.occ, reinterpret_cast<const void*>(k_fwd2), 64 * V2_WAVES, 0) != hipSuccess) o.occ = 0;
    (void)hipGetLastError();
    if (o.occ < 1) o.occ = 3;

    V2Plan pl;
    pl.cnt = cnt;
    pl.np = uint32_t(dp.size());
    pl.ncouples = (cnt + 1u) / 2u;
    plan_couples(pl, dp, order, corridor_model(c, P, corridor), band_target(pl.ncouples, o.few_limit, o.occ, o.n_cu));
    std::vector<uint64_t> cops;
    if (ops) {
        cops.assign(pl.ncouples, 0);
        for (uint32_t x = 0; x < cnt; ++x) cops[x / 2u] += uint64_t(dp[order[x]].n) + dp[order[x]].m;
    }
    slice_couples(pl, budget, cops);
    std::vector<uint64_t> slice_ops(pl.slices.size(), 0);
    if (ops) {
        ops->end.assign(dp.size(), 0);
        uint64_t most = 0;
        for (size_t si = 0; si < pl.slices.size(); ++si) {
            const uint32_t x0 = 2u * pl.slices[si].first, x1 = std::min(cnt, 2u * (pl.slices[si].first + pl.slices[si].second));
            for (uint32_t x = x0; x < x1; ++x) ops->end[order[x]] = slice_ops[si] += uint64_t(dp[order[x]].n) + dp[order[x]].m;
            most = std::max(most, slice_ops[si]);
        }
        if ((r = ops_reserve(c, *ops, most)) != IOC_OK) return r;
    }
    const auto t_res0 = std::chrono::steady_clock::now();
    if ((r = reserve(c, c->a_ck, size_t(pl.arena_words) * 4)) != IOC_OK) return r;
    c->tm.align_arena_bytes = int64_t(pl.arena_words) * 4;
    c->tm.align_slices = int32_t(pl.slices.size());
    c->tm.align_version = 2;
    if (getenv("IOC_TRACE"))
        fprintf(stderr, "[ioc]   aligner v2: %u couples, checkpoint arena %.1f MB (%zu slice(s)) reserved in %.3f ms; corridor: %llu of %llu tiles skipped\n", pl.ncouples,
                double(pl.arena_words) * 4e-6, pl.slices.size(), std::chrono::duration<double, std::milli>(std::chrono::steady_clock::now() - t_res0).count(),
                (unsigned long long)pl.tiles_skipped, (unsigned long long)pl.tiles_all);
    tile_lists(pl);

    o.deadline = 4;
    if (const char* e = getenv("IOC_TRACE2_DEADLINE")) o.deadline = uint32_t(std::max(0, atoi(e)));
    if (const char* e = getenv("IOC_TRACE2_CYCLES")) o.deadline_cycles = (unsigned long long)std::max(0.0, atof(e));
    o.help_wgs = o.deadline ? std::min<uint32_t>(pl.max_pairs, uint32_t(o.n_cu)) : 0u;
    V2Dev t{};
    if ((r = v2_tables(c, pl, o.help_wgs, t)) != IOC_OK) return r;
    o.side_help = o.deadline && !(getenv("IOC_TRACE2_EARLY") && atoi(getenv("IOC_TRACE2_EARLY")) == 0);
    if (o.side_help && !c->side_stream) {
        ACHK(c, hipStreamCreateWithFlags(&c->side_stream, hipStreamNonBlocking));
        for (auto& e : c->ev_side) ACHK(c, hipEventCreateWithFlags(&e, hipEventDisableTiming));
    }
    EventSet evs;
    evs.v.assign(pl.slices.size() * 3, nullptr);
    for (auto& e : evs.v) ACHK(c, hipEventCreate(&e));
    if (getenv("IOC_TRACE"))
        fprintf(stderr, "[ioc]   aligner v2: planning (couples, corridors, tile lists, tables) took the host %.3f ms\n",
                std::chrono::duration<double, std::milli>(std::chrono::steady_clock::now() - t_plan0).count());
    size_t evi = 0;
    bool bad = false;
    for (size_t si = 0; si < pl.slices.size() && !bad; ++si, evi += 3) {
        uint32_t xe = 0;
        if ((r = v2_slice(c, pl, t, si, o, P, d_order, d_score, d_count, &evs.v[evi], &xe, ops ? &ops->dev : nullptr)) != IOC_OK) return r;
        if (ops && !xe) {
            const uint32_t x0 = 2u * pl.slices[si].first, x1 = std::min(cnt, 2u * (pl.slices[si].first + pl.slices[si].second));
            if ((r = ops_fetch(c, *ops, dp, order + x0, x1 - x0, slice_ops[si])) != IOC_OK) return r;
        }
        if ((r = v2_report(c, dp, order, pl, t, si, o.deadline)) != IOC_OK) return r;
        bad = xe != 0;
    }
    add_elapsed(c, evs.v, evi);
    if (getenv("IOC_TRACE"))
        fprintf(stderr, "[ioc]   aligner v2: forward %.3f ms, traceback %.3f ms (device, all slices so far)%s\n", c->tm.ms_align_fwd,
                c->tm.ms_align_trace, bad ? " — a wait ran out: falling back to version 1" : "");
    *fell_back = bad;
    return IOC_OK;
}


enum class AlnRoute { normal, every_tile, v1_only };

struct AlnOut {
    int32_t* score;
    int64_t* windows;
    double* ratio;
    const AlnOpsHost* ops = nullptr;
    void set(size_t i, int32_t s, int64_t w, double r) const
    {
        if (score) score[i] = s;
        if (windows) windows[i] = w;
        if (ratio) ratio[i] = r;
    }
};

struct AlnBatch {
    std::vector<AlnPairDev> dp;
    std::vector<uint32_t> back;
    std::vector<uint32_t> order;
    uint32_t max_n = 1, max_m = 1;
};

int prepare_pairs(ioc_ctx* c, int32_t n_pairs, const ioc_aln_pair* pairs, const AlnParams& P, const AlnOut& out, AlnBatch& b)
{
    const int32_t n_seqs = c->aln_offs.empty() ? 0 : int32_t(c->aln_offs.size() - 1);
    const int32_t k = int32_t(P.k);
    b.dp.reserve(size_t(n_pairs));
    for (int32_t i = 0; i < n_pairs; ++i) {
        const ioc_aln_pair& a = pairs[i];
        if (a.query < 0 || a.query >= n_seqs || a.ref < 0 || a.ref >= n_seqs)
            return ioc_fail(c, IOC_ERR_ARG, "alignment pair refers to a sequence outside the pool");
        const int64_t n = c->aln_offs[size_t(a.query) + 1] - c->aln_offs[size_t(a.query)];
        const int64_t m = c->aln_offs[size_t(a.ref) + 1] - c->aln_offs[size_t(a.ref)];
        if (n + m >= (int64_t(1) << ALN_LEN_SHIFT))
            return ioc_fail(c, IOC_ERR_CAPACITY, "GPU aligner: sequences above 2^26 bases");
        const double limit = std::floor((1.0 - a.e) * double(k));
        const int32_t il = limit < -1.0 ? -1 : limit > 64.0 ? 64 : int32_t(limit);
        if (n == 0 || m == 0) {
            const int64_t len = n + m;
            const int64_t cnt = (il <= 0 && len > k) ? len - k : 0;
            out.set(size_t(i), 0, cnt, n == 0 ? 0.0 : double(cnt) / double(n));
            if (out.ops) {
                memset(out.ops->buf + out.ops->base[i], n ? 'i' : 'd', size_t(len));
                out.ops->len[i] = len;
            }
            continue;
        }
        AlnPairDev d{};
        d.q_off = uint32_t(c->aln_offs[size_t(a.query)]);
        d.n = uint32_t(n);
        d.r_off = uint32_t(c->aln_offs[size_t(a.ref)]);
        d.m = uint32_t(m);
        d.gap_open = ioc_host_gap_open(a.e);
        d.e_sum = float(a.e);
        d.ilimit = il;
        d.rc = a.ref_revcomp ? 1u : 0u;
        d.stop_at = 0;
        if (c->aln_verdict_thr > 0.0 && n > 0 && !out.ops) {
            double a0 = std::ceil(c->aln_verdict_thr * double(n));
            while (a0 > 0 && (a0 - 1.0) / double(n) >= c->aln_verdict_thr) a0 -= 1.0;
            while (a0 / double(n) < c->aln_verdict_thr) a0 += 1.0;
            d.stop_at = a0 >= 1.0 && a0 < 4.0e9 ? uint32_t(a0) : 0u;
        }
        {
            const int gd = d.gap_open - P.gap_extend, cm = P.match + 2 * P.gap_extend + gd, cx = P.mismatch + 2 * P.gap_extend + gd;
            const bool ok = !c->aln_other[size_t(a.query)] && !c->aln_other[size_t(a.ref)] && cm >= 0 && cm <= 255 &&
                            cx >= 0 && cx <= 255 && !getenv("IOC_ALIGN_NO_PROFILE");
            d.pad = ok ? 1u : 0u;
        }
        b.dp.push_back(d);
        b.back.push_back(uint32_t(i));
        b.max_n = std::max(b.max_n, d.n);
        b.max_m = std::max(b.max_m, d.m);
    }
    return IOC_OK;
}

void order_pairs(AlnBatch& b, const ioc_aln_pair* pairs)
{
    const std::vector<AlnPairDev>& dp = b.dp;
    const uint32_t np = uint32_t(dp.size());
    std::vector<uint32_t>& order = b.order;
    order.resize(np);
    std::iota(order.begin(), order.end(), 0u);
    std::stable_sort(order.begin(), order.end(), [&](uint32_t x, uint32_t y) {
        return uint64_t(dp[x].n) * dp[x].m > uint64_t(dp[y].n) * dp[y].m;
    });
    {
        auto rows = [&](uint32_t x) { return uint64_t((dp[x].n + 511u) / 512u); };
        auto cols = [&](uint32_t x) { return uint64_t((dp[x].m + 511u) / 512u); };
        std::stable_sort(order.begin(), order.end(), [&](uint32_t x, uint32_t y) {
            const uint64_t tx = rows(x) * cols(x), ty = rows(y) * cols(y);
            if (tx != ty) return tx > ty;
            if (rows(x) != rows(y)) return rows(x) > rows(y);
            return dp[x].e_sum > dp[y].e_sum;
        });
    }
    {
        std::vector<int32_t> hp;
        for (uint32_t x = 0; x < np; ++x)
            if (pairs[b.back[x]].reserved > 0) hp.push_back(pairs[b.back[x]].reserved);
        if (hp.size() >= 8 && !getenv("IOC_ALIGN_NO_HINTS")) {
            std::nth_element(hp.begin(), hp.begin() + long(hp.size() / 2), hp.end());
            const int64_t med = hp[hp.size() / 2];
            std::stable_partition(order.begin(), order.end(), [&](uint32_t x) {
                const int64_t h = pairs[b.back[x]].reserved;
                return !(h > 0 && h * 4 < med);
            });
        }
    }
    std::stable_partition(order.begin(), order.end(), [&](uint32_t x) { return dp[x].pad != 0; });
}

struct WavePlan {
    uint32_t waves;
    bool few_pairs;
};
WavePlan plan_waves(const AlnBatch& b, bool carry)
{
    const uint32_t np = uint32_t(b.dp.size());
    uint32_t waves = ALN_MAXW;
    if (const char* e = getenv("IOC_ALIGN_WAVES")) {
        const int v = atoi(e);
        if (v >= 1 && v <= ALN_MAXW) waves = uint32_t(v);
    } else {
        while (waves > 1 && uint64_t(np) * waves > 4096) waves >>= 1;
        if (carry) {
            while (waves > 1 && uint64_t(waves / 2) * 64 * ALN_C >= b.max_m) waves >>= 1;
        } else {
            const uint32_t strips = (b.max_m + 64 * FW_C - 1) / (64 * FW_C), tiles = (b.max_n + TILE - 1) / TILE;
            while (waves > 1 && (strips < 2 * waves || tiles < 2 * waves)) waves >>= 1;
        }
    }
    const bool few_pairs = !carry && !getenv("IOC_ALIGN_WAVES") && np <= 64 && waves >= 4 && !getenv("IOC_ALIGN_NO_CROSS_TAIL");
    return WavePlan{few_pairs ? 4u : waves, few_pairs};
}

int run_v2(ioc_ctx* c, const AlnBatch& b, const AlnParams& P, int32_t* d_score, uint32_t* d_count, AlnRoute route, uint32_t* n_v2, const AlnOpsHost* oh)
{
    const uint32_t np = uint32_t(b.dp.size());
    uint32_t n = 0;
    while (n < np && b.dp[b.order[n]].pad != 0) ++n;
    bool fell_back = false;
    OpsRun ops{oh, b.back.data()};
    const int r = align_v2_run(c, b.dp, b.order.data(), n, static_cast<const uint32_t*>(c->a_order.p), P, d_score, d_count, route != AlnRoute::every_tile,
                               &fell_back, oh ? &ops : nullptr);
    if (r != IOC_OK) return r;
    if (fell_back) {
        c->tm.n_align_refused += n;
        n = 0;
    }
    *n_v2 = n;
    return IOC_OK;
}

int run_carry(ioc_ctx* c, const AlnBatch& b, uint32_t waves, const AlnParams& P, int32_t* d_score, uint32_t* d_count)
{
    const uint32_t np = uint32_t(b.dp.size()), NT = waves * 64;
    const uint64_t bnd_stride = 2ull * 6ull * b.max_n;
    const uint64_t lrow_entries = uint64_t((b.max_m + NT * ALN_C - 1) / (NT * ALN_C)) * NT;
    const uint64_t lrow_stride = lrow_entries * 4ull;
    const uint64_t budget = 8ull << 30;
    const uint64_t per_pair = (bnd_stride + lrow_stride) * 4ull;
    const uint32_t slice = uint32_t(std::min<uint64_t>(np, std::max<uint64_t>(1, budget / per_pair)));
    int r;
    if ((r = reserve(c, c->a_bnd, size_t(slice) * bnd_stride * 4)) != IOC_OK) return r;
    if ((r = reserve(c, c->a_lrow, size_t(slice) * lrow_stride * 4)) != IOC_OK) return r;
    for (uint32_t first = 0; first < np; first += slice) {
        const uint32_t cnt = std::min(slice, np - first);
        hipLaunchKernelGGL(k_align_carry, dim3(cnt), dim3(NT), 0, c->stream, static_cast<const AlnPairDev*>(c->a_pairs.p),
                           static_cast<const uint32_t*>(c->a_order.p) + first, static_cast<const uint8_t*>(c->a_pool.p), P,
                           static_cast<uint32_t*>(c->a_bnd.p), bnd_stride, static_cast<uint32_t*>(c->a_lrow.p), lrow_stride, d_score, d_count);
        ACHK(c, hipGetLastError());
    }
    return IOC_OK;
}


size_t fwd_lds_limit(ioc_ctx* c, bool prof, const void* kfn, size_t fallback, size_t* stat)
{
    hipFuncAttributes fa{};
    *stat = fallback;
    if (hipFuncGetAttributes(&fa, kfn) == hipSuccess) *stat = fa.sharedSizeBytes;
    size_t& lim = prof ? c->aln_lds_max : c->aln_lds_max2;
    if (lim == 0) {
        int mx = 0;
        (void)hipDeviceGetAttribute(&mx, hipDeviceAttributeMaxSharedMemoryPerBlock, c->device);
        lim = 64 * 1024 > *stat ? 64 * 1024 - *stat : 1;
        if (mx > 72 * 1024 && hipFuncSetAttribute(kfn, hipFuncAttributeMaxDynamicSharedMemorySize, mx - int(*stat)) == hipSuccess)
            lim = size_t(mx) - *stat;
        (void)hipGetLastError();
    }
    return lim;
}

struct V1Plan {
    std::vector<AlnCk> cko;
    std::vector<std::pair<uint32_t, uint32_t>> slices;
    uint64_t arena = 0;
    uint32_t max_cnt = 0;
    std::vector<uint64_t> ops_end, slice_ops;
    uint64_t ops_most = 0;
};
uint64_t v1_row_units(const AlnPairDev& d) { return uint64_t((d.n - 1) / TILE) * row_pitch(d.m); }

V1Plan plan_v1(const AlnBatch& b, uint32_t n_v2, uint64_t budget, bool emit)
{
    const std::vector<AlnPairDev>& dp = b.dp;
    const uint32_t np = uint32_t(dp.size());
    V1Plan pl;
    pl.cko.resize(np);
    if (emit) pl.ops_end.assign(np, 0);
    for (uint32_t first = n_v2; first < np;) {
        uint64_t used = 0, ops_used = 0;
        uint32_t cnt = 0;
        while (first + cnt < np) {
            const AlnPairDev& d = dp[b.order[first + cnt]];
            const uint64_t u = v1_row_units(d) + uint64_t((d.m - 1) / TILE) * col_pitch(d.n);
            const uint64_t ops_u = emit ? uint64_t(d.n) + d.m : 0u;
            if (cnt > 0 && (used + u) * 8ull + ops_used + ops_u > budget) break;
            if (cnt > 0 && d.pad != dp[b.order[first]].pad) break;
            pl.cko[b.order[first + cnt]] = AlnCk{used, used + v1_row_units(d)};
            used += u;
            ops_used += ops_u;
            if (emit) pl.ops_end[b.order[first + cnt]] = ops_used;
            ++cnt;
        }
        pl.slice_ops.push_back(ops_used);
        pl.ops_most = std::max(pl.ops_most, ops_used);
        pl.arena = std::max(pl.arena, used);
        pl.slices.emplace_back(first, cnt);
        pl.max_cnt = std::max(pl.max_cnt, cnt);
        first += cnt;
    }
    return pl;
}

struct V1Fwd {
    ioc_ctx* c;
    bool prof;
    AlnParams P;
    uint64_t lrow_stride;
    int operator()(const uint32_t* o, uint32_t cnt, uint32_t wv, uint32_t wgw, uint32_t nwg, uint32_t nmain, uint32_t wtail, size_t lds,
                   uint32_t lrow_first, const AlnCross& X) const
    {
        const AlnPairDev* dpairs = static_cast<const AlnPairDev*>(c->a_pairs.p);
        const uint8_t* dpool = static_cast<const uint8_t*>(c->a_pool.p);
        int2* dck = static_cast<int2*>(c->a_ck.p);
        const AlnCk* dcko = static_cast<const AlnCk*>(c->a_cko.p);
        int2* lr = static_cast<int2*>(c->a_lrow.p) + uint64_t(lrow_first) * lrow_stride;
        int4* dends = static_cast<int4*>(c->a_ends2.p);
        if (prof)
            hipLaunchKernelGGL(k_align_fwd<true>, dim3(nwg), dim3(wgw * 64), lds, c->stream, dpairs, o, cnt, wv, nmain, wtail, dpool, P, dck, dcko, lr,
                               lrow_stride, dends, X);
        else
            hipLaunchKernelGGL(k_align_fwd<false>, dim3(nwg), dim3(wgw * 64), lds, c->stream, dpairs, o, cnt, wv, nmain, wtail, dpool, P, dck, dcko, lr,
                               lrow_stride, dends, X);
        ACHK(c, hipGetLastError());
        return IOC_OK;
    }
};

int v1_cross_tail(ioc_ctx* c, const AlnBatch& b, const V1Fwd& fwd, const std::pair<uint32_t, uint32_t>& sl, uint32_t waves, uint32_t wg_waves,
                  uint32_t n_main, uint32_t ppw, uint32_t groups, bool inl, size_t lds_pad, const void* kfn)
// ... 26 lines not shown
    }
    uint32_t xe = 0;
    ACHK(c, hipMemcpyAsync(&xe, X.err, 4, hipMemcpyDeviceToHost, s));
    ACHK(c, hipStreamSynchronize(s));
    if (xe) {
        if ((r = fwd(ord + first_cnt, rest, 4, 4, rest, rest, 4, 0, first_cnt, AlnCross{})) != IOC_OK) return r;
        c->tm.n_align_refused += rest;
    }
    return IOC_OK;
}

int v1_slice(ioc_ctx* c, const AlnBatch& b, const std::pair<uint32_t, uint32_t>& sl, const WavePlan& wp, const AlnParams& P, int n_cu,
             uint64_t lrow_stride, int32_t* d_score, uint32_t* d_count, const hipEvent_t* ev, const AlnOpsDev* od)
{
    hipStream_t s = c->stream;
    const uint32_t waves = wp.waves;
    const uint32_t* ord = static_cast<const uint32_t*>(c->a_order.p) + sl.first;
    const bool prof = b.dp[b.order[sl.first]].pad != 0;
    const void* kfn = prof ? reinterpret_cast<const void*>(k_align_fwd<true>) : reinterpret_cast<const void*>(k_align_fwd<false>);
    const V1Fwd fwd{c, prof, P, lrow_stride};
    size_t lds_pad = 0;
    const uint32_t wg_waves = waves > 4 ? waves : 4, ppw = wg_waves / waves;
    uint32_t n_wg = (sl.second + ppw - 1) / ppw, n_main = n_wg, wpp_tail = waves;
    {
        int occ = 0;
        if (hipOccupancyMaxActiveBlocksPerMultiprocessor(&occ, kfn, int(wg_waves * 64), 0) != hipSuccess) occ = 0;
        (void)hipGetLastError();
        const uint32_t gen = uint32_t(occ > 0 ? occ : 3) * uint32_t(n_cu);
        if (n_wg > gen && n_wg < gen + gen / 2 && 2 * waves <= wg_waves) {
            n_main = gen;
            wpp_tail = 2 * waves;
            const uint32_t rest = sl.second - n_main * ppw, ppw_tail = wg_waves / wpp_tail;
            n_wg = n_main + (rest + ppw_tail - 1) / ppw_tail;
        }
    }
    const uint32_t per_cu = (n_main + uint32_t(n_cu) - 1) / uint32_t(n_cu);
    if (per_cu * wg_waves < 32) {
        size_t stat = 0;
        const size_t lim = fwd_lds_limit(c, prof, kfn, 48 * 1024, &stat);
        const size_t want = size_t(160u * 1024u) * (2 * per_cu + 1) / (2 * per_cu * (per_cu + 1));
        lds_pad = want > stat + 1024 ? (want - stat - 512) & ~size_t(255) : 0;
        lds_pad = std::min(lds_pad, lim > 1 ? lim : 0);
    }
    ACHK(c, hipEventRecord(ev[0], s));
    uint32_t groups = 1;
    const bool force_cross = getenv("IOC_ALIGN_FORCE_CROSS") != nullptr || (wp.few_pairs && waves == 4);
    if (force_cross && wg_waves == 4) {
        n_main = 0;
        n_wg = 1;
    }
    const bool inl = !force_cross;
    if (n_main < n_wg && wg_waves == 4 && !getenv("IOC_ALIGN_NO_CROSS_TAIL")) {
        const AlnPairDev& big = b.dp[b.order[sl.first]];
        const uint32_t strips = (big.m + 64 * FW_C - 1) / (64 * FW_C), tiles = (big.n + TILE - 1) / TILE;
        groups = force_cross ? 4 : 2;
        if (const char* eg = getenv("IOC_ALIGN_CROSS_GROUPS")) groups = uint32_t(std::max(1, std::min(4, atoi(eg))));
        while (groups > 1 && (strips < 4 * groups || tiles < 8 * groups)) groups >>= 1;
        const uint32_t rest = sl.second - n_main * ppw;
        while (groups > 1 && uint64_t(rest) * groups > uint64_t(inl ? 2 : 1) * uint64_t(n_cu)) groups >>= 1;
    }
    int r;
    if (groups > 1) {
        if ((r = v1_cross_tail(c, b, fwd, sl, waves, wg_waves, n_main, ppw, groups, inl, lds_pad, kfn)) != IOC_OK) return r;
    } else {
        if (force_cross && n_main == 0) {
            n_wg = (sl.second + ppw - 1) / ppw;
            n_main = n_wg;
        }
        if ((r = fwd(ord, sl.second, waves, wg_waves, n_wg, n_main, wpp_tail, lds_pad, 0, AlnCross{})) != IOC_OK) return r;
    }
    ACHK(c, hipEventRecord(ev[1], s));
    const uint32_t tr_wg = (sl.second + TR_WAVES - 1) / TR_WAVES;
    if (od)
        hipLaunchKernelGGL(k_align_trace_ops, dim3(tr_wg), dim3(64 * TR_WAVES), 0, s, static_cast<const AlnPairDev*>(c->a_pairs.p), ord,
                           static_cast<const uint8_t*>(c->a_pool.p), P, static_cast<const int2*>(c->a_ck.p), static_cast<const AlnCk*>(c->a_cko.p),
                           static_cast<const int4*>(c->a_ends2.p), d_score, d_count, sl.second, *od);
    else
        hipLaunchKernelGGL(k_align_trace, dim3(tr_wg), dim3(64 * TR_WAVES), 0, s, static_cast<const AlnPairDev*>(c->a_pairs.p), ord,
                           static_cast<const uint8_t*>(c->a_pool.p), P, static_cast<const int2*>(c->a_ck.p), static_cast<const AlnCk*>(c->a_cko.p),
                           static_cast<const int4*>(c->a_ends2.p), d_score, d_count, sl.second);
    ACHK(c, hipGetLastError());
    ACHK(c, hipEventRecord(ev[2], s));
    return IOC_OK;
}

int run_v1(ioc_ctx* c, const AlnBatch& b, uint32_t n_v2, const WavePlan& wp, const AlnParams& P, int32_t* d_score, uint32_t* d_count, const AlnOpsHost* oh)
{
    hipStream_t s = c->stream;
    const uint32_t np = uint32_t(b.dp.size());
    int r;
    uint64_t budget = 0;
    if ((r = ck_budget(c, &budget)) != IOC_OK) return r;
    const uint64_t lrow_stride = uint64_t((b.max_m + 64 * FW_C - 1) / (64 * FW_C)) * 64;
    for (const AlnPairDev& d : b.dp)
        if (v1_row_units(d) >= (uint64_t(1) << 29))
            return ioc_fail(c, IOC_ERR_CAPACITY, "alignment of " + std::to_string(d.n) + " x " + std::to_string(d.m) + " bases: row checkpoints above 4 GB per pair");
    V1Plan pl = plan_v1(b, n_v2, budget, oh != nullptr);
    OpsRun ops{oh, b.back.data()};
    if (oh) {
        ops.end.swap(pl.ops_end);
        if ((r = ops_reserve(c, ops, pl.ops_most)) != IOC_OK) return r;
    }
    const auto t_res0 = std::chrono::steady_clock::now();
    if ((r = reserve(c, c->a_ck, size_t(pl.arena) * 8)) != IOC_OK) return r;
    c->tm.align_arena_bytes = int64_t(pl.arena) * 8;
    c->tm.align_slices = int32_t(pl.slices.size());
    c->tm.align_version = 1;
    if (getenv("IOC_TRACE"))
        fprintf(stderr, "[ioc]   aligner: checkpoint arena %.1f MB (%zu slice(s)) reserved in %.3f ms\n", double(pl.arena) * 8e-6, pl.slices.size(),
                std::chrono::duration<double, std::milli>(std::chrono::steady_clock::now() - t_res0).count());
    if ((r = reserve(c, c->a_cko, size_t(np) * sizeof(AlnCk))) != IOC_OK) return r;
    if ((r = reserve(c, c->a_ends2, size_t(np) * sizeof(int4))) != IOC_OK) return r;
    if ((r = reserve(c, c->a_lrow, size_t(pl.max_cnt) * lrow_stride * 8)) != IOC_OK) return r;
    ACHK(c, hipMemcpyAsync(c->a_cko.p, pl.cko.data(), size_t(np) * sizeof(AlnCk), hipMemcpyHostToDevice, s));
    const int n_cu = compute_units(c);
    EventSet evs;
    evs.v.assign(pl.slices.size() * 3, nullptr);
    for (auto& e : evs.v) ACHK(c, hipEventCreate(&e));
    for (size_t si = 0; si < pl.slices.size(); ++si) {
        if ((r = v1_slice(c, b, pl.slices[si], wp, P, n_cu, lrow_stride, d_score, d_count, &evs.v[3 * si], oh ? &ops.dev : nullptr)) != IOC_OK) return r;
        if (oh && (r = ops_fetch(c, ops, b.dp, b.order.data() + pl.slices[si].first, pl.slices[si].second, pl.slice_ops[si])) != IOC_OK) return r;
    }
    ACHK(c, hipStreamSynchronize(s));
    add_elapsed(c, evs.v, evs.v.size());
    if (getenv("IOC_TRACE"))
        fprintf(stderr, "[ioc]   aligner: forward %.3f ms, traceback %.3f ms (device, all slices so far)\n", c->tm.ms_align_fwd, c->tm.ms_align_trace);
    return IOC_OK;
}


void learn_corridor(ioc_ctx* c, const AlnBatch& b, const AlnParams& P, const std::vector<int32_t>& hs, const std::vector<uint32_t>& hc)
{
    if (c->aln_fit_sig[0] != P.match || c->aln_fit_sig[1] != P.mismatch || c->aln_fit_sig[2] != P.gap_extend) {
        for (auto& f : c->aln_fit) f = ioc_ctx::CorridorFit();
        c->aln_fit_sig[0] = P.match, c->aln_fit_sig[1] = P.mismatch, c->aln_fit_sig[2] = P.gap_extend;
    }
    for (size_t x = 0; x < b.dp.size(); ++x) {
        const AlnPairDev& d = b.dp[x];
        const uint32_t len = std::max(d.n, d.m);
        if (hc[x] == 0xFFFFFFFFu || len < 4096u || !(d.e_sum > 0.0f) || std::min(d.n, d.m) * 10u < len * 9u) continue;
        const double rho = double(hs[x]) / double(len), e = double(d.e_sum);
        if (rho * 2.0 < double(P.match)) continue;
        ioc_ctx::CorridorFit& f = c->aln_fit[std::max(2, std::min(5, d.gap_open)) - 2];
        if (f.n >= 1e6) continue;
        f.n += 1.0, f.se += e, f.sr += rho, f.see += e * e, f.ser += e * rho, f.srr += rho * rho;
        f.e_lo = std::min(f.e_lo, e), f.e_hi = std::max(f.e_hi, e);
    }
}

int read_results(ioc_ctx* c, const AlnBatch& b, uint32_t n_v2, const int32_t* d_score, const uint32_t* d_count, std::vector<int32_t>& hs,
                 std::vector<uint32_t>& hc)
{
    const uint32_t np = uint32_t(b.dp.size());
    c->tm.n_align_pairs += np;
    for (auto& d : b.dp) c->tm.n_align_cells += int64_t(d.n) * int64_t(d.m);
    for (uint32_t x = n_v2; x < np; ++x)
        c->tm.n_align_cells_computed += int64_t(b.dp[b.order[x]].n) * int64_t(b.dp[b.order[x]].m);
    hs.resize(np);
    hc.resize(np);
    ACHK(c, hipMemcpyAsync(hs.data(), d_score, size_t(np) * 4, hipMemcpyDeviceToHost, c->stream));
    ACHK(c, hipMemcpyAsync(hc.data(), d_count, size_t(np) * 4, hipMemcpyDeviceToHost, c->stream));
    ACHK(c, hipStreamSynchronize(c->stream));
    return IOC_OK;
}


int align_pairs(ioc_ctx* c, int32_t n_pairs, const ioc_aln_pair* pairs, int32_t k, int32_t match, int32_t mismatch, int32_t gap_extend,
                const AlnOut& out, AlnRoute route);

int align_again(ioc_ctx* c, const ioc_aln_pair* pairs, const std::vector<int32_t>& idx, const AlnParams& P, AlnRoute route, const AlnOut& out)
{
    std::vector<ioc_aln_pair> sub(idx.size());
    std::vector<int32_t> sc(idx.size());
    std::vector<int64_t> sw(idx.size());
    std::vector<double> sr(idx.size());
    for (size_t x = 0; x < idx.size(); ++x) sub[x] = pairs[idx[x]];
    std::vector<int64_t> sbase, slen(out.ops ? idx.size() : 0, 0);
    AlnOpsHost soh{};
    if (out.ops) {
        for (int32_t i : idx) sbase.push_back(out.ops->base[i]);
        soh = AlnOpsHost{out.ops->buf, sbase.data(), slen.data(), out.ops->ms_copy, out.ops->copied};
    }
    const int r = align_pairs(c, int32_t(sub.size()), sub.data(), int32_t(P.k), P.match, P.mismatch, P.gap_extend,
                              AlnOut{sc.data(), sw.data(), sr.data(), out.ops ? &soh : nullptr}, route);
    if (r != IOC_OK) return r;
    for (size_t x = 0; x < idx.size(); ++x) {
        out.set(size_t(idx[x]), sc[x], sw[x], sr[x]);
        if (out.ops) out.ops->len[idx[x]] = slen[x];
    }
    return IOC_OK;
}

int scatter_results(ioc_ctx* c, const AlnBatch& b, const ioc_aln_pair* pairs, bool v2, const AlnParams& P, const std::vector<int32_t>& hs,
                    const std::vector<uint32_t>& hc, const AlnOut& out)
{
    std::vector<int32_t> again;
    std::vector<int32_t> again_full;
    for (size_t x = 0; x < b.dp.size(); ++x) {
        const uint32_t i = b.back[x];
        if (v2 && hc[x] == 0xFFFFFFFFu && hs[x] == INT32_MIN) {
            again.push_back(int32_t(i));
            continue;
        }
        if (v2 && hc[x] == 0xFFFFFFFFu && hs[x] == INT32_MIN + 1) {
            again_full.push_back(int32_t(i));
            continue;
        }
        out.set(i, hs[x], int64_t(hc[x]), double(hc[x]) / double(b.dp[x].n));
    }
    int r;
    if (!again_full.empty()) {
        const int64_t pairs_so_far = c->tm.n_align_pairs, cells_so_far = c->tm.n_align_cells;
        if ((r = align_again(c, pairs, again_full, P, AlnRoute::every_tile, out)) != IOC_OK) return r;
        c->tm.n_align_pairs = pairs_so_far;
        c->tm.n_align_cells = cells_so_far;
        if (getenv("IOC_TRACE")) fprintf(stderr, "[ioc]   aligner v2: %zu of %zu pairs run again without a corridor\n", again_full.size(), b.dp.size());
    }
    if (!again.empty()) {
        if ((r = align_again(c, pairs, again, P, AlnRoute::v1_only, out)) != IOC_OK) return r;
        c->tm.n_align_refused += int64_t(again.size());
    }
    return IOC_OK;
}

int align_pairs(ioc_ctx* c, int32_t n_pairs, const ioc_aln_pair* pairs, int32_t k, int32_t match, int32_t mismatch, int32_t gap_extend,
                const AlnOut& out, AlnRoute route)
{
    if (!c || n_pairs < 0 || (n_pairs > 0 && !pairs)) return IOC_ERR_ARG;
    if (k < 1 || k > 32) return ioc_fail(c, IOC_ERR_CAPACITY, "GPU aligner: window length k must be in 1..32");
    ACHK(c, hipSetDevice(c->device));
    if (n_pairs == 0) return IOC_OK;
    const AlnParams P{match, mismatch, gap_extend, uint32_t(k), 1u << (32 - k)};
    AlnBatch b;
    int r;
    if ((r = prepare_pairs(c, n_pairs, pairs, P, out, b)) != IOC_OK) return r;
    const uint32_t np = uint32_t(b.dp.size());
    if (np == 0) return IOC_OK;
    order_pairs(b, pairs);
    const char* ev = getenv("IOC_ALIGN_VARIANT");
    const bool carry = ev && strcmp(ev, "carry") == 0 && !out.ops;
    const WavePlan wp = plan_waves(b, carry);
    if ((r = reserve(c, c->a_pairs, size_t(np) * sizeof(AlnPairDev))) != IOC_OK) return r;
    if ((r = reserve(c, c->a_order, size_t(np) * 4)) != IOC_OK) return r;
    if ((r = reserve(c, c->a_out, size_t(np) * 8)) != IOC_OK) return r;
    ACHK(c, hipMemcpyAsync(c->a_pairs.p, b.dp.data(), size_t(np) * sizeof(AlnPairDev), hipMemcpyHostToDevice, c->stream));
    ACHK(c, hipMemcpyAsync(c->a_order.p, b.order.data(), size_t(np) * 4, hipMemcpyHostToDevice, c->stream));
    int32_t* d_score = static_cast<int32_t*>(c->a_out.p);
    uint32_t* d_count = reinterpret_cast<uint32_t*>(d_score + np);
    const char* arena_mode = getenv("IOC_ALIGN_ARENA");
    const bool v2 = route != AlnRoute::v1_only && !carry && !getenv("IOC_ALIGN_V1") && !(arena_mode && strcmp(arena_mode, "fat") == 0);
    uint32_t n_v2 = 0;
    if (v2 && (r = run_v2(c, b, P, d_score, d_count, route, &n_v2, out.ops)) != IOC_OK) return r;
    if (carry)
        r = run_carry(c, b, wp.waves, P, d_score, d_count);
    else if (n_v2 < np)
        r = run_v1(c, b, n_v2, wp, P, d_score, d_count, out.ops);
    if (r != IOC_OK) return r;
    std::vector<int32_t> hs;
    std::vector<uint32_t> hc;
    if ((r = read_results(c, b, n_v2, d_score, d_count, hs, hc)) != IOC_OK) return r;
    if (v2 && route == AlnRoute::normal) learn_corridor(c, b, P, hs, hc);
    return scatter_results(c, b, pairs, v2, P, hs, hc, out);
}

}

extern "C" {

int ioc_align_set_pool(ioc_ctx* c, int32_t n_seqs, const char* seqs, const int64_t* offs)
{
    if (!c || n_seqs < 0 || (n_seqs > 0 && (!seqs || !offs))) return IOC_ERR_ARG;
    ACHK(c, hipSetDevice(c->device));
    c->res_pool_ready = false;
    c->aln_offs.assign(offs, offs + (n_seqs > 0 ? n_seqs + 1 : 0));
    if (n_seqs == 0) return IOC_OK;
    if (offs[0] != 0) return ioc_fail(c, IOC_ERR_ARG, "sequence pool offsets must start at 0");
    for (int32_t i = 0; i < n_seqs; ++i)
        if (offs[i + 1] < offs[i]) return ioc_fail(c, IOC_ERR_ARG, "sequence pool offsets must be ascending");
    const int64_t total = offs[n_seqs];
    if (total >= (int64_t(1) << 32)) return ioc_fail(c, IOC_ERR_CAPACITY, "sequence pool above 4 GiB");
    int r = reserve(c, c->a_pool, size_t(total));
    if (r != IOC_OK) return r;
    ACHK(c, hipMemcpyAsync(c->a_pool.p, seqs, size_t(total), hipMemcpyHostToDevice, c->stream));
    if ((r = reserve(c, c->a_ends, size_t(n_seqs + 1) * 8 + size_t(n_seqs))) != IOC_OK) return r;
    int64_t* d_offs = static_cast<int64_t*>(c->a_ends.p);
    uint8_t* d_flags = reinterpret_cast<uint8_t*>(d_offs + n_seqs + 1);
    ACHK(c, hipMemcpyAsync(d_offs, offs, size_t(n_seqs + 1) * 8, hipMemcpyHostToDevice, c->stream));
    hipLaunchKernelGGL(k_seq_flags, dim3(uint32_t(n_seqs)), dim3(256), 0, c->stream,
                       static_cast<const uint8_t*>(c->a_pool.p), d_offs, d_flags);
    ACHK(c, hipGetLastError());
    c->aln_other.assign(size_t(n_seqs), 0);
    ACHK(c, hipMemcpyAsync(c->aln_other.data(), d_flags, size_t(n_seqs), hipMemcpyDeviceToHost, c->stream));
    ACHK(c, hipStreamSynchronize(c->stream));
    return IOC_OK;
}

int ioc_align_set_verdict_threshold(ioc_ctx* c, double aligned_threshold)
{
    if (!c) return IOC_ERR_ARG;
    c->aln_verdict_thr = aligned_threshold > 0.0 ? aligned_threshold : -1.0;
    return IOC_OK;
}

int ioc_align_pairs(ioc_ctx* c, int32_t n_pairs, const ioc_aln_pair* pairs, int32_t k, int32_t match, int32_t mismatch,
                    int32_t gap_extend, int32_t* out_score, int64_t* out_windows, double* out_ratio)
{
    return align_pairs(c, n_pairs, pairs, k, match, mismatch, gap_extend, AlnOut{out_score, out_windows, out_ratio}, AlnRoute::normal);
}

int64_t ioc_align_ops_bound(ioc_ctx* c, int32_t n_pairs, const ioc_aln_pair* pairs)
{
    if (!c || n_pairs < 0 || (n_pairs > 0 && !pairs)) return IOC_ERR_ARG;
    const int64_t n_seqs = c->aln_offs.empty() ? 0 : int64_t(c->aln_offs.size()) - 1;
    int64_t bound = 0;
    for (int32_t i = 0; i < n_pairs; ++i) {
        const ioc_aln_pair& a = pairs[i];
        if (a.query < 0 || a.query >= n_seqs || a.ref < 0 || a.ref >= n_seqs) return ioc_fail(c, IOC_ERR_ARG, "alignment pair refers to a sequence outside the pool");
        bound += (c->aln_offs[size_t(a.query) + 1] - c->aln_offs[size_t(a.query)]) + (c->aln_offs[size_t(a.ref) + 1] - c->aln_offs[size_t(a.ref)]);
    }
    return bound;
}

int ioc_align_pairs_ops(ioc_ctx* c, int32_t n_pairs, const ioc_aln_pair* pairs, int32_t k, int32_t match, int32_t mismatch,
                        int32_t gap_extend, int32_t* out_score, int64_t* out_windows, double* out_ratio, char* out_ops, int64_t ops_cap,
                        int64_t* ops_off)
{
    if (!c || n_pairs < 0 || (n_pairs > 0 && !pairs) || !ops_off || ops_cap < 0 || (ops_cap > 0 && !out_ops)) return IOC_ERR_ARG;
    const int64_t bound = ioc_align_ops_bound(c, n_pairs, pairs);
    if (bound < 0) return int(bound);
    if (ops_cap < bound) return ioc_fail(c, IOC_ERR_CAPACITY, "ioc_align_pairs_ops: ops_cap " + std::to_string(ops_cap) + " below the bound " + std::to_string(bound));
    std::vector<int64_t> base(size_t(n_pairs) + 1, 0), len(size_t(n_pairs), 0);
    for (int32_t i = 0; i < n_pairs; ++i)
        base[size_t(i) + 1] = base[size_t(i)] + (c->aln_offs[size_t(pairs[i].query) + 1] - c->aln_offs[size_t(pairs[i].query)]) +
                              (c->aln_offs[size_t(pairs[i].ref) + 1] - c->aln_offs[size_t(pairs[i].ref)]);
    double ms_copy = 0;
    int64_t copied = 0;
    const AlnOpsHost oh{reinterpret_cast<uint8_t*>(out_ops), base.data(), len.data(), &ms_copy, &copied};
    const int r = align_pairs(c, n_pairs, pairs, k, match, mismatch, gap_extend, AlnOut{out_score, out_windows, out_ratio, &oh}, AlnRoute::normal);
    if (r != IOC_OK) return r;
    ops_off[0] = 0;
    for (int32_t i = 0; i < n_pairs; ++i) {
        if (len[size_t(i)] > 0 && ops_off[i] != base[size_t(i)]) memmove(out_ops + ops_off[i], out_ops + base[size_t(i)], size_t(len[size_t(i)]));
        ops_off[i + 1] = ops_off[i] + len[size_t(i)];
    }
    if (getenv("IOC_TRACE"))
        fprintf(stderr, "[ioc]   aligner: operation bytes: %.1f MB copied from the device in %.3f ms, %.1f MB packed\n", double(copied) * 1e-6, ms_copy,
                double(ops_off[n_pairs]) * 1e-6);
    return IOC_OK;
}

hipError_t iock_warm_align()
{
    hipFuncAttributes a;
    return hipFuncGetAttributes(&a, reinterpret_cast<const void*>(k_fwd2_ends));
}

}
```

### isonclust2_amd/csrc/ioc_align_v2.inc

```

constexpr int CK2 = 512;
constexpr int V2_WAVES = 4;
constexpr int V2_BLK_C = 8;
constexpr int V2_MAX_BANDS = 40;
static_assert(CK2 % TILE == 0 && CK2 == 64 * V2_BLK_C, "block geometry");

struct V2Couple {
    uint32_t pid[2];
    uint32_t nbands, nstrips;
    uint32_t tpb;
    uint32_t flag0;
    uint32_t mpad;
    uint32_t nq;
    uint64_t rdat;
    uint64_t rbase;
    uint64_t cdat;
    uint64_t cbase;
    uint64_t prof;
    uint32_t lrow0[2];
    uint32_t best0[2];
    uint16_t bstart[V2_MAX_BANDS + 1];
    uint16_t plo[V2_MAX_BANDS], phi[V2_MAX_BANDS];
    uint32_t corridor;
    uint16_t probe_band, probe_strip;
    uint32_t b0;
};

struct V2Item {
    uint32_t couple;
    uint16_t band, strip;
};

struct V2PairCk {
    uint64_t rdat, rbase, cdat, cbase;
    uint32_t mpad, nq, half, couple;
};


__device__ __forceinline__ bool v2_wait(const uint32_t* flag, uint32_t* err)
{
    uint32_t seen = 0;
    for (uint32_t it = 0; it < (1u << 22); ++it) {
        seen = uint32_t(__builtin_amdgcn_readfirstlane(int(__hip_atomic_load(flag, __ATOMIC_RELAXED, __HIP_MEMORY_SCOPE_AGENT))));
        if (seen) break;
        if ((it & 255u) == 255u && __builtin_amdgcn_readfirstlane(int(__hip_atomic_load(err, __ATOMIC_RELAXED, __HIP_MEMORY_SCOPE_AGENT)))) break;
        __builtin_amdgcn_s_sleep(8);
    }
    if (!seen) __hip_atomic_store(err, 1u, __ATOMIC_RELAXED, __HIP_MEMORY_SCOPE_AGENT);
    return seen != 0;
}

__device__ __forceinline__ bool v2_wait_rows(const uint32_t* prog, const uint32_t* flag, uint32_t need, uint32_t* err, uint32_t& avail)
{
    bool ok = false;
    for (uint32_t it = 0; it < (1u << 22); ++it) {
        const uint32_t f = uint32_t(__builtin_amdgcn_readfirstlane(int(__hip_atomic_load(flag, __ATOMIC_RELAXED, __HIP_MEMORY_SCOPE_AGENT))));
        const uint32_t g = uint32_t(__builtin_amdgcn_readfirstlane(int(__hip_atomic_load(prog, __ATOMIC_RELAXED, __HIP_MEMORY_SCOPE_AGENT))));
        if (f || g >= need) {
            ok = true;
            avail = f ? 0xFFFFFFFFu : g;
            break;
        }
        if ((it & 255u) == 255u && __builtin_amdgcn_readfirstlane(int(__hip_atomic_load(err, __ATOMIC_RELAXED, __HIP_MEMORY_SCOPE_AGENT)))) break;
        __builtin_amdgcn_s_sleep(4);
    }
    if (!ok) __hip_atomic_store(err, 1u, __ATOMIC_RELAXED, __HIP_MEMORY_SCOPE_AGENT);
    return ok;
}

__device__ __forceinline__ uint32_t v2_dequeue(uint32_t* queue)
{
    uint32_t x = 0, one = 1;
    unsigned long long save;
    asm volatile(
        "s_mov_b64 %1, exec\n\t"
        "s_mov_b64 exec, 1\n\t"
        "global_atomic_add %0, %2, %3, off sc0\n\t"
        "s_waitcnt vmcnt(0)\n\t"
        "s_mov_b64 exec, %1"
        : "+v"(x), "=&s"(save)
        : "v"(queue), "v"(one)
        : "memory");
    return uint32_t(__builtin_amdgcn_readfirstlane(int(x)));
}

typedef unsigned short v2u __attribute__((ext_vector_type(2)));
__device__ __forceinline__ v2u as_v2u(uint32_t x) { return __builtin_bit_cast(v2u, x); }
__device__ __forceinline__ uint32_t u32_of(v2u x) { return __builtin_bit_cast(uint32_t, x); }
__device__ __forceinline__ uint32_t umax2(uint32_t a, uint32_t b) { return u32_of(__builtin_elementwise_max(as_v2u(a), as_v2u(b))); }
__device__ __forceinline__ uint32_t umin2(uint32_t a, uint32_t b) { return u32_of(__builtin_elementwise_min(as_v2u(a), as_v2u(b))); }
__device__ __forceinline__ uint32_t usubs2(uint32_t a, uint32_t b) { return u32_of(__builtin_elementwise_sub_sat(as_v2u(a), as_v2u(b))); }
__device__ __forceinline__ uint32_t clampu16(int v) { return uint32_t(min(max(v, 0), 65535)); }
__device__ __forceinline__ uint32_t packu(uint32_t lo, uint32_t hi) { return lo | (hi << 16); }
__device__ __forceinline__ int v2_half(uint32_t w, int h) { return h ? int(w >> 16) : int(w & 0xFFFFu); }
constexpr int U16_BIAS = 32768;

__device__ __forceinline__ void cells_u16(uint32_t (&Hq)[FW_C], uint32_t (&F)[FW_C], const uint4& xa, const uint4& xb, uint32_t& hql, uint32_t& el,
                                          uint32_t dgq, uint32_t gd2)
{
    const uint32_t xl[FW_C / 4] = {xa.x, xa.y, xa.z, xa.w}, xh[FW_C / 4] = {xb.x, xb.y, xb.z, xb.w};
    uint32_t T[FW_C];
#pragma unroll
    for (int c = 0; c < FW_C; ++c) {
        const uint32_t Fn = umax2(F[c], Hq[c]);
        const uint32_t sel = 0x0c000c00u | uint32_t(4 + (c & 3)) << 16 | uint32_t(c & 3);
        const uint32_t inc = __builtin_amdgcn_perm(xh[c >> 2], xl[c >> 2], sel);
        T[c] = umax2((c ? Hq[c - 1] : dgq) + inc, Fn);
        F[c] = Fn;
    }
    uint32_t e = el, h = hql;
#pragma unroll
    for (int c = 0; c < FW_C; ++c) {
        e = umax2(e, h);
        h = umax2(T[c], e) - gd2;
        Hq[c] = h;
    }
    hql = h;
    el = e;
}

__device__ __forceinline__ uint32_t v2_par(uint32_t lds_byte_addr)
{
    uint32_t x;
    asm volatile("ds_read_b32 %0, %1\n\ts_waitcnt lgkmcnt(0)" : "=v"(x) : "v"(lds_byte_addr) : "memory");
    return x;
}

__device__ __forceinline__ void v2_lds_store(uint32_t lds_byte_addr, uint32_t v)
{
    asm volatile("ds_write_b32 %0, %1\n\ts_waitcnt lgkmcnt(0)" : : "v"(lds_byte_addr), "v"(v) : "memory");
}

enum V2Par : uint32_t {
    VP_N0 = 0, VP_N1, VP_M0, VP_M1, VP_GD0, VP_GD1, VP_LROW0, VP_LROW1, VP_BEST0, VP_BEST1, VP_PID0, VP_PID1,
    VP_RDAT_LO, VP_RDAT_HI, VP_RBASE_LO, VP_RBASE_HI, VP_CDAT_LO, VP_CDAT_HI, VP_CBASE_LO, VP_CBASE_HI,
    VP_MPAD, VP_NQ, VP_FLAG, VP_BAND, VP_STRIP, VP_COLIN_LO, VP_COLIN_HI, VP_RHI0, VP_RHI1, VP_COUNT = 32
};

__global__ void __launch_bounds__(128)
k_fwd2_prof(const AlnPairDev* __restrict__ pairs, const V2Couple* __restrict__ couples, const uint8_t* __restrict__ pool, AlnParams P, uint4* __restrict__ prof)
{
    const V2Couple& cp = couples[blockIdx.x];
    const uint32_t p = blockIdx.y;
    if (p >= cp.nstrips) return;
    const uint32_t h = threadIdx.x >> 6, lane = threadIdx.x & 63u;
    const bool have = cp.pid[h] != 0xFFFFFFFFu;
    const AlnPairDev pr = pairs[have ? cp.pid[h] : cp.pid[0]];
    const uint32_t m = have ? pr.m : 0u;
    const uint8_t* r = pool + pr.r_off;
    const int ge = P.gap_extend, gd = pr.gap_open - ge;
    const int cm = P.match + 2 * ge + gd, cx = P.mismatch + 2 * ge + gd;
    const uint32_t jb = p * (64u * FW_C) + lane * FW_C;
    uint32_t rpk[FW_C / 4];
#pragma unroll
    for (int c4 = 0; c4 < FW_C / 4; ++c4) {
        uint32_t w = 0;
#pragma unroll
        for (int e = 0; e < 4; ++e) w |= (have ? ref_byte(r, m, pr.rc, jb + c4 * 4 + e) : 0u) << (8 * e);
        rpk[c4] = w;
    }
    const uint32_t bases = 'A' | ('C' << 8) | ('G' << 16) | ('T' << 24);
    uint4* out = prof + cp.prof + (uint64_t(p) * 2u + h) * 5u * 64u + lane;
#pragma unroll
    for (int code = 0; code < 5; ++code) {
        const uint32_t b = code < 4 ? (bases >> (8 * code)) & 0xFFu : 0x100u;
        uint32_t w4[FW_C / 4];
#pragma unroll
        for (int c4 = 0; c4 < FW_C / 4; ++c4) {
            uint32_t w = 0;
#pragma unroll
            for (int e = 0; e < 4; ++e) w |= uint32_t(((rpk[c4] >> (8 * e)) & 0xFFu) == b ? cm : cx) << (8 * e);
            w4[c4] = w;
        }
        out[uint32_t(code) * 64u] = uint4{w4[0], w4[1], w4[2], w4[3]};
    }
}

static __device__ __forceinline__ void
v2_fwd_body(const AlnPairDev* __restrict__ pairs, const V2Couple* __restrict__ couples, const V2Item* __restrict__ items, uint32_t n_items,
       uint32_t* __restrict__ queue, uint32_t* __restrict__ flags, uint32_t* __restrict__ err, const uint8_t* __restrict__ pool, AlnParams P,
       uint32_t* __restrict__ arena, int2* __restrict__ lrow, int2* __restrict__ bandbest, uint32_t* __restrict__ ovf_out, int guard,
       const uint4* __restrict__ prof, unsigned long long* __restrict__ cells_done, uint32_t* __restrict__ prog, uint32_t prog_every)
{
    __shared__ __attribute__((aligned(16))) uint32_t s_look_all[V2_WAVES][3][128];
    __shared__ __attribute__((aligned(16))) uint32_t s_prof_all[V2_WAVES][2][5][64][4];
    __shared__ uint32_t s_par_all[V2_WAVES][VP_COUNT];
    const uint32_t lane = threadIdx.x & 63u;
    const uint32_t wv = uint32_t(__builtin_amdgcn_readfirstlane(int(threadIdx.x >> 6)));
    uint32_t(*s_look)[128] = s_look_all[wv];
    uint32_t* s_par = s_par_all[wv];
    const uint32_t par_addr = uint32_t(reinterpret_cast<uintptr_t>(s_par));
    auto par = [&](uint32_t k) -> uint32_t { return v2_par(par_addr + 4u * k); };
    auto par64 = [&](uint32_t k) -> uint64_t { return uint64_t(par(k)) | (uint64_t(par(k + 1u)) << 32); };
    constexpr uint32_t strip_cols = 64u * FW_C;
    const int ge = P.gap_extend;
    auto qcode = [](uint32_t ch) -> uint32_t {
        const uint32_t code = ch == 'A' ? 0u : ch == 'C' ? 1u : ch == 'G' ? 2u : ch == 'T' ? 3u : 4u;
        return code * 1024u;
    };
    uint32_t it = v2_dequeue(queue);
    while (it < n_items) {
        uint32_t band, p, r_lo, nblk[2];
        bool vh[2], last_band[2];
        bool left_ok = true;
        bool top_none = false;
        bool left_rows = false;
        uint32_t left_idx = 0, nblk_band = 0, left_avail = 0;
        const uint8_t* q[2];
        int base[2];
        uint32_t gd2;
        uint32_t Hp[FW_C], F[FW_C];
        uint32_t dg;
        uint64_t cb_off = 0;
        uint64_t co_off = 0;
        uint64_t rd_off = 0;
        uint64_t rb_off = 0;
        uint32_t mpad = 0, ncr = 0;
        {
            const V2Item item = items[it];
            const V2Couple cp = couples[item.couple];
            band = item.band;
            p = item.strip;
            if (p < cp.plo[band] || p > cp.phi[band] ||
                __builtin_amdgcn_readfirstlane(int(__hip_atomic_load(&flags[cp.flag0 + band * cp.nstrips + p], __ATOMIC_RELAXED, __HIP_MEMORY_SCOPE_AGENT))) != 0) {
                it = v2_dequeue(queue);
                continue;
            }
            const bool top_in = band > 0 && p >= cp.plo[band - 1u] && p <= cp.phi[band - 1u];
            const bool left_in = p > cp.plo[band];
            left_ok = p == 0 || left_in;
            top_none = band > 0 && !top_in;
            const bool corner_in = band > 0 && p > 0 && p - 1u >= cp.plo[band - 1u] && p - 1u <= cp.phi[band - 1u];
            if (top_in) (void)v2_wait(&flags[cp.flag0 + (band - 1u) * cp.nstrips + p], err);
            left_rows = prog != nullptr && left_in;
            left_idx = cp.flag0 + band * cp.nstrips + (p - 1u);
            {
                const uint32_t rows_b = min(max(cp.pid[0] != 0xFFFFFFFFu ? pairs[cp.pid[0]].n : 0u, cp.pid[1] != 0xFFFFFFFFu ? pairs[cp.pid[1]].n : 0u),
                                            uint32_t(cp.bstart[band + 1u]) * uint32_t(CK2));
                const uint32_t r0_b = uint32_t(cp.bstart[band]) * uint32_t(CK2);
                nblk_band = rows_b > r0_b ? (rows_b - r0_b + FW_R - 1) / FW_R : 0u;
            }
            if (left_in && !left_rows) (void)v2_wait(&flags[left_idx], err);
            if (left_rows) (void)v2_wait_rows(&prog[left_idx], &flags[left_idx], min(32u, nblk_band), err, left_avail);
            __builtin_amdgcn_fence(__ATOMIC_ACQUIRE, "agent");
            r_lo = uint32_t(cp.bstart[band]) * uint32_t(CK2);
            const uint32_t jb = p * strip_cols + lane * FW_C;
            uint32_t n[2], m[2], r_hi[2];
            int gd[2];
#pragma unroll
            for (int h = 0; h < 2; ++h) {
                const bool have = cp.pid[h] != 0xFFFFFFFFu;
                const AlnPairDev pr = pairs[have ? cp.pid[h] : cp.pid[0]];
                n[h] = have ? pr.n : 0u;
                m[h] = have ? pr.m : 0u;
                q[h] = pool + pr.q_off;
                gd[h] = pr.gap_open - ge;
                r_hi[h] = min(n[h], uint32_t(cp.bstart[band + 1u]) * uint32_t(CK2));
                nblk[h] = r_hi[h] > r_lo ? (r_hi[h] - r_lo + FW_R - 1) / FW_R : 0u;
                const uint32_t nstr = (m[h] + strip_cols - 1) / strip_cols;
                vh[h] = have && p < nstr && nblk[h] > 0;
                last_band[h] = vh[h] && r_hi[h] == n[h];
            }
            gd2 = packu(uint32_t(gd[0]), uint32_t(gd[1]));
            mpad = cp.mpad;
            rd_off = cp.rdat + jb;
            rb_off = cp.rbase + uint64_t(jb / 16u) * 2u;
            {
                uint32_t nmx = max(n[0], n[1]);
                ncr = nmx ? (nmx - 1u) / uint32_t(CK2) : 0u;
            }
            {
                const uint64_t e0 = uint64_t((jb + FW_C) / CK2 - ((jb + FW_C) >= uint32_t(CK2) ? 1u : 0u)) * cp.nq + r_lo / 4u;
                co_off = cp.cdat + e0 * 8u;
                cb_off = cp.cbase + e0 * 2u;
            }
            const uint64_t colin = p ? uint64_t(p * (strip_cols / CK2) - 1u) * cp.nq : 0;
            __builtin_amdgcn_fence(__ATOMIC_RELEASE, "workgroup");
            __builtin_amdgcn_wave_barrier();
            if (lane == 0) {
                s_par[VP_N0] = n[0];
                s_par[VP_N1] = n[1];
                s_par[VP_M0] = m[0];
                s_par[VP_M1] = m[1];
                s_par[VP_GD0] = uint32_t(gd[0]);
                s_par[VP_GD1] = uint32_t(gd[1]);
                s_par[VP_LROW0] = cp.lrow0[0];
                s_par[VP_LROW1] = cp.lrow0[1];
                s_par[VP_BEST0] = cp.best0[0];
                s_par[VP_BEST1] = cp.best0[1];
                s_par[VP_PID0] = cp.pid[0];
                s_par[VP_PID1] = cp.pid[1];
                s_par[VP_RDAT_LO] = uint32_t(cp.rdat);
                s_par[VP_RDAT_HI] = uint32_t(cp.rdat >> 32);
                s_par[VP_RBASE_LO] = uint32_t(cp.rbase);
                s_par[VP_RBASE_HI] = uint32_t(cp.rbase >> 32);
                s_par[VP_CDAT_LO] = uint32_t(cp.cdat);
                s_par[VP_CDAT_HI] = uint32_t(cp.cdat >> 32);
                s_par[VP_CBASE_LO] = uint32_t(cp.cbase);
                s_par[VP_CBASE_HI] = uint32_t(cp.cbase >> 32);
                s_par[VP_MPAD] = cp.mpad;
                s_par[VP_NQ] = cp.nq;
                s_par[VP_FLAG] = cp.flag0 + band * cp.nstrips + p;
                s_par[VP_BAND] = band;
                s_par[VP_STRIP] = p;
                s_par[VP_COLIN_LO] = uint32_t(colin);
                s_par[VP_COLIN_HI] = uint32_t(colin >> 32);
                s_par[VP_RHI0] = r_hi[0];
                s_par[VP_RHI1] = r_hi[1];
            }
            int Ha[2][FW_C], Fa[2][FW_C], dga[2];
#pragma unroll
            for (int h = 0; h < 2; ++h) {
                if (!vh[h]) {
#pragma unroll
                    for (int c = 0; c < FW_C; ++c) Ha[h][c] = Fa[h][c] = 0;
                    dga[h] = 0;
                } else if (r_lo > 0 && !top_in) {
#pragma unroll
                    for (int c = 0; c < FW_C; ++c) Ha[h][c] = Fa[h][c] = ALN_NEG;
                    dga[h] = ALN_NEG;
                } else if (r_lo == 0) {
                    const int b0 = ge * int(jb) - gd[h];
#pragma unroll
                    for (int c = 0; c < FW_C; ++c) {
                        Ha[h][c] = b0 + ge * (c + 1);
                        Fa[h][c] = ALN_NEG;
                    }
                    dga[h] = b0;
                } else {
                    const uint32_t ckr = r_lo / CK2 - 1u;
                    const uint32_t* rh = arena + cp.rdat + uint64_t(2u * ckr) * cp.mpad;
                    const uint32_t* rf = rh + cp.mpad;
                    const int2* rb = reinterpret_cast<const int2*>(arena + cp.rbase) + uint64_t(ckr) * (cp.mpad / 16u);
                    const int2 bb = jb < cp.mpad ? rb[jb / 16u] : int2{0, 0};
                    const int bs = h ? bb.y : bb.x;
#pragma unroll
                    for (int c = 0; c < FW_C; ++c) {
                        int2 v{0, 0};
                        if (jb + c < m[h]) v = int2{v2_half(rh[jb + c], h) + bs, v2_half(rf[jb + c], h) + bs};
                        Ha[h][c] = v.x;
                        Fa[h][c] = v.y;
                    }
                    if (lane == 0 && p > 0 && !corner_in) {
                        dga[h] = ALN_NEG;
                    } else if (jb > 0 && jb <= m[h]) {
                        const int2 bl = rb[(jb - 1u) / 16u];
                        dga[h] = v2_half(rh[jb - 1u], h) + (h ? bl.y : bl.x);
                    } else {
                        dga[h] = ge * int(r_lo) - gd[h];
                    }
                }
                if (vh[h] && r_lo > 0 && !top_in) {
                    const uint64_t e = colin + r_lo / 4u;
                    const uint32_t* d = arena + cp.cdat + e * 8u;
                    const int2 bb = reinterpret_cast<const int2*>(arena + cp.cbase)[e];
                    base[h] = v2_half(d[0], h) + (h ? bb.y : bb.x) - U16_BIAS;
                } else
                base[h] = __builtin_amdgcn_readfirstlane(Ha[h][0]) - U16_BIAS;
            }
#pragma unroll
            for (int c = 0; c < FW_C; ++c) {
                const bool in0 = vh[0] && jb + c < m[0], in1 = vh[1] && jb + c < m[1];
                Hp[c] = packu(in0 ? clampu16(Ha[0][c] - base[0]) : uint32_t(U16_BIAS), in1 ? clampu16(Ha[1][c] - base[1]) : uint32_t(U16_BIAS));
                F[c] = packu(in0 ? clampu16(Fa[0][c] - base[0]) : uint32_t(U16_BIAS), in1 ? clampu16(Fa[1][c] - base[1]) : uint32_t(U16_BIAS));
            }
            dg = packu(clampu16(dga[0] - base[0]), clampu16(dga[1] - base[1]));
            {
                const uint4* pp = prof + cp.prof + uint64_t(p) * (2u * 5u * 64u) + lane;
#pragma unroll
                for (int h = 0; h < 2; ++h)
#pragma unroll
                    for (int code = 0; code < 5; ++code) {
                        const uint4 w = pp[(uint32_t(h) * 5u + uint32_t(code)) * 64u];
                        *reinterpret_cast<uint4*>(&s_prof_all[wv][h][code][lane][0]) = w;
                    }
            }
        }
        const uint32_t jb = p * strip_cols + lane * FW_C;
        const uint32_t nsteps = max(nblk[0], nblk[1]) + 63u;
        uint32_t lanef = 0;
        int lastc[2];
        uint32_t ncl[2];
        bool strip_has_lastc = false;
        __builtin_amdgcn_fence(__ATOMIC_RELEASE, "workgroup");
        __builtin_amdgcn_wave_barrier();
        __builtin_amdgcn_fence(__ATOMIC_ACQUIRE, "workgroup");
        {
            const uint32_t jr = jb + FW_C;
            bool any_right = false;
#pragma unroll
            for (int h = 0; h < 2; ++h) {
                const uint32_t mh = par(VP_M0 + h);
                const bool hc = vh[h] && jb < mh;
                ncl[h] = vh[h] ? min(64u, (mh - p * strip_cols + FW_C - 1) / FW_C) : 0u;
                lastc[h] = (vh[h] && mh - 1 >= jb && mh - 1 < jb + FW_C) ? int(mh - 1 - jb) : -1;
                strip_has_lastc = strip_has_lastc || (vh[h] && uint64_t(p + 1u) * strip_cols >= mh);
                any_right = any_right || (vh[h] && jr < mh);
                lanef |= (hc ? 1u : 0u) << h;
                lanef |= (lastc[h] >= 0 ? 4u : 0u) << h;
            }
            if ((jr % CK2) == 0 && any_right) lanef |= 16u;
        }
        const uint8_t* profA = reinterpret_cast<const uint8_t*>(&s_prof_all[wv][0][0][lane][0]);
        const uint8_t* profB = reinterpret_cast<const uint8_t*>(&s_prof_all[wv][1][0][lane][0]);
        auto left_edge = [&](int h, uint32_t row) {
            int2 v{ge * int(row + 1) - int(par(VP_GD0 + h)), ALN_NEG};
            if (!left_ok) v = int2{ALN_NEG, ALN_NEG};
            else if (vh[h] && p > 0 && row < par(VP_RHI0 + h)) {
                const uint64_t e = par64(VP_COLIN_LO) + row / 4u;
                const uint32_t* d = arena + par64(VP_CDAT_LO) + e * 8u;
                const int2 bb = reinterpret_cast<const int2*>(arena + par64(VP_CBASE_LO))[e];
                const int bs = h ? bb.y : bb.x;
                v = int2{v2_half(d[row & 3u], h) + bs, v2_half(d[4u + (row & 3u)], h) + bs};
            }
            return v;
        };
        uint32_t qn = 0;
        int2 en[2] = {{0, 0}, {0, 0}};
        uint32_t hl[FW_R], el[FW_R];
        uint32_t qc[FW_R];
#pragma unroll
        for (int rr = 0; rr < FW_R; ++rr) {
            hl[rr] = packu(U16_BIAS, U16_BIAS);
            el[rr] = 0;
            qc[rr] = 0;
        }
        auto publish = [&](uint32_t blk) {
            s_look[0][(blk & 1u) * 64u + lane] = packu(clampu16(en[0].x - base[0]), clampu16(en[1].x - base[1]));
            s_look[1][(blk & 1u) * 64u + lane] = packu(clampu16(en[0].y - base[0]), clampu16(en[1].y - base[1]));
            s_look[2][(blk & 1u) * 64u + lane] = qn;
        };
        auto fetch = [&](uint32_t blk) {
            const uint32_t row = r_lo + blk * 64u + lane;
            uint32_t qq[2];
#pragma unroll
            for (int h = 0; h < 2; ++h) {
                qq[h] = qcode((vh[h] && row < par(VP_RHI0 + h)) ? q[h][row] : 0u);
                en[h] = left_edge(h, row);
            }
            qn = qq[0] | (qq[1] << 16);
        };
        fetch(0);
        publish(0);
        fetch(1);
        __builtin_amdgcn_fence(__ATOMIC_RELEASE, "workgroup");
        __builtin_amdgcn_wave_barrier();
        __builtin_amdgcn_fence(__ATOMIC_ACQUIRE, "workgroup");
        uint4 nxh, nxe, nxq;
        nxh = *reinterpret_cast<const uint4*>(&s_look[0][0]);
        nxe = *reinterpret_cast<const uint4*>(&s_look[1][0]);
        nxq = *reinterpret_cast<const uint4*>(&s_look[2][0]);
        {
            const uint32_t q4[FW_R] = {nxq.x, nxq.y, nxq.z, nxq.w};
#pragma unroll
            for (int rr = 0; rr < FW_R; ++rr) qc[rr] = from_left_or(qc[rr], q4[rr]);
        }
        int bc[2] = {ALN_NEG, ALN_NEG};
        uint32_t bc_i[2] = {0, 0};
        uint32_t ovf = 0;

        auto step = [&](const uint32_t s, auto first) __attribute__((always_inline)) {
            if (decltype(first)::value && (s & (64 / FW_R - 1)) == 0) {
                if (s) {
                    int dl[2];
#pragma unroll
                    for (int h = 0; h < 2; ++h) {
                        const uint32_t lr = s + 1u > nblk[h] ? min(63u, s + 1u - nblk[h]) : 0u;
                        const int ref = __builtin_amdgcn_readlane(int(Hp[0]), int(lr));
                        dl[h] = max(v2_half(uint32_t(ref), h) - U16_BIAS, 0);
                        if (!vh[h] || lr >= ncl[h]) dl[h] = 0;
                        base[h] += dl[h];
                    }
                    const uint32_t d2 = packu(uint32_t(dl[0]), uint32_t(dl[1]));
                    {
                        uint32_t mx = Hp[0], mn = Hp[0];
#pragma unroll
                        for (int c = 1; c < FW_C; ++c) {
                            mx = umax2(mx, Hp[c]);
                            mn = umin2(mn, Hp[c]);
                        }
                        const int bi = int(s) - int(lane);
#pragma unroll
                        for (int h = 0; h < 2; ++h) {
                            const int hi_v = v2_half(mx, h) - U16_BIAS, lo_v = v2_half(mn, h) - U16_BIAS;
                            if ((lanef >> h & 1u) && bi >= (top_none ? 1 : 0) && uint32_t(bi) < nblk[h] && (hi_v > guard || lo_v < -guard)) {
#ifdef IOC_V2_GUARD_DEBUG
                                if (!(ovf >> h & 1u)) printf("guard: item %u band %u strip %u half %d lane %u step %u hi %d lo %d left_ok %d base %d\n", it, band, p, h, lane, s, hi_v, lo_v, int(left_ok), base[h]);
#endif
                                ovf |= 1u << h;
                            }
                        }
                    }
#pragma unroll
                    for (int c = 0; c < FW_C; ++c) {
                        Hp[c] = usubs2(Hp[c], d2);
                        F[c] = usubs2(F[c], d2);
                    }
                    dg = usubs2(dg, d2);
#pragma unroll
                    for (int rr = 0; rr < FW_R; ++rr) {
                        hl[rr] = usubs2(hl[rr], d2);
                        el[rr] = usubs2(el[rr], d2);
                    }
                    nxh = uint4{usubs2(nxh.x, d2), usubs2(nxh.y, d2), usubs2(nxh.z, d2), usubs2(nxh.w, d2)};
                    nxe = uint4{usubs2(nxe.x, d2), usubs2(nxe.y, d2), usubs2(nxe.z, d2), usubs2(nxe.w, d2)};
                    const uint32_t cur = ((s / (64 / FW_R)) & 1u) * 64u + lane;
                    s_look[0][cur] = usubs2(s_look[0][cur], d2);
                    s_look[1][cur] = usubs2(s_look[1][cur], d2);
                }
                const uint32_t blk = s / (64 / FW_R) + 1u;
                if (prog != nullptr && s >= 64u && (prog_every <= 1u || (s / 16u) % prog_every == 0u)) {
                    asm volatile("s_waitcnt vmcnt(0)" ::: "memory");
                    __builtin_amdgcn_fence(__ATOMIC_RELEASE, "agent");
                    asm volatile("s_waitcnt vmcnt(0)" ::: "memory");
                    __hip_atomic_store(&prog[uint32_t(__builtin_amdgcn_readfirstlane(int(par(VP_FLAG))))], s - 63u, __ATOMIC_RELAXED, __HIP_MEMORY_SCOPE_AGENT);
                }
                publish(blk);
                if (left_rows) {
                    const uint32_t need_rows = min(16u * (blk + 2u), nblk_band);
                    if (need_rows > left_avail) {
                        (void)v2_wait_rows(&prog[left_idx], &flags[left_idx], need_rows, err, left_avail);
                        __builtin_amdgcn_fence(__ATOMIC_ACQUIRE, "agent");
                    }
                }
                fetch(blk + 1u);
            }
            {
                const uint32_t h4[FW_R] = {nxh.x, nxh.y, nxh.z, nxh.w}, e4[FW_R] = {nxe.x, nxe.y, nxe.z, nxe.w};
#pragma unroll
                for (int rr = 0; rr < FW_R; ++rr) {
                    hl[rr] = from_left_or(hl[rr], h4[rr]);
                    el[rr] = from_left_or(el[rr], e4[rr]);
                }
                const uint32_t nx = ((s + 1u) * FW_R) & 127u;
                nxh = *reinterpret_cast<const uint4*>(&s_look[0][nx]);
                nxe = *reinterpret_cast<const uint4*>(&s_look[1][nx]);
                nxq = *reinterpret_cast<const uint4*>(&s_look[2][nx]);
            }
            const int bi = int(s) - int(lane);
            bool act[2];
#pragma unroll
            for (int h = 0; h < 2; ++h) act[h] = (lanef >> h & 1u) && bi >= 0 && uint32_t(bi) < nblk[h];
            if (act[0] || act[1]) {
                const bool special = strip_has_lastc || (last_band[0] && s + 1u >= nblk[0] && s + 1u - nblk[0] < 64u) ||
                                     (last_band[1] && s + 1u >= nblk[1] && s + 1u - nblk[1] < 64u);
                auto row_cells = [&](int rr) __attribute__((always_inline)) {
                    const uint32_t hl_in = hl[rr];
                    const uint4 xa = *reinterpret_cast<const uint4*>(profA + (qc[rr] & 0xFFFFu));
                    const uint4 xb = *reinterpret_cast<const uint4*>(profB + (qc[rr] >> 16));
                    cells_u16(Hp, F, xa, xb, hl[rr], el[rr], dg, gd2);
                    dg = hl_in;
                };
#pragma unroll
                for (int rr = 0; rr < FW_R; ++rr) {
                    row_cells(rr);
                    if (special) {

#pragma unroll
                        for (int h = 0; h < 2; ++h) {
                            const uint32_t i = r_lo + uint32_t(bi) * FW_R + rr;
                            const uint32_t nh = par(VP_N0 + h), mh = par(VP_M0 + h);
                            const int gdh = int(par(VP_GD0 + h));
                            if (act[h] && i < nh) {
                                if (lastc[h] >= 0) {
                                    const uint32_t lc = uint32_t(lastc[h]);
                                    const bool b0 = lc & 1u, b1 = lc & 2u, b2 = lc & 4u, b3 = lc & 8u;
                                    const uint32_t s0 = b0 ? Hp[1] : Hp[0], s1 = b0 ? Hp[3] : Hp[2], s2 = b0 ? Hp[5] : Hp[4], s3 = b0 ? Hp[7] : Hp[6],
                                                   s4 = b0 ? Hp[9] : Hp[8], s5 = b0 ? Hp[11] : Hp[10], s6 = b0 ? Hp[13] : Hp[12], s7 = b0 ? Hp[15] : Hp[14];
                                    const uint32_t u0 = b1 ? s1 : s0, u1 = b1 ? s3 : s2, u2 = b1 ? s5 : s4, u3 = b1 ? s7 : s6;
                                    const uint32_t v0 = b2 ? u1 : u0, v1 = b2 ? u3 : u2;
                                    int hm = v2_half(b3 ? v1 : v0, h) + base[h];
                                    hm += gdh - ge * int(i + 1u + mh);
                                    if (hm > bc[h]) {
                                        bc[h] = hm;
                                        bc_i[h] = i + 1u;
                                    }
                                }
                                if (i + 1u == nh) {
                                    int br = ALN_NEG;
                                    uint32_t bj = 0;
                                    const int b0 = base[h] + gdh - ge * int(nh + jb);
#pragma unroll
                                    for (int c = 0; c < FW_C; ++c) {
                                        const int ht = v2_half(Hp[c], h) + b0 - ge * (c + 1);
                                        if (jb + c < mh && ht > br) {
                                            br = ht;
                                            bj = jb + c + 1;
                                        }
                                    }
                                    lrow[par(VP_LROW0 + h) + p * 64u + lane] = int2{br, int(bj)};
                                }
                            }
                        }
                    }
                }
                const uint32_t ib = uint32_t(bi);
                if (lanef & 16u) {
                    uint32_t* d = arena + co_off + uint64_t(ib) * 8u;
                    uint4* co = reinterpret_cast<uint4*>(d);
                    co[0] = uint4{hl[0], hl[1], hl[2], hl[3]};
                    co[1] = uint4{el[0], el[1], el[2], el[3]};
                    reinterpret_cast<int2*>(arena + cb_off)[ib] = int2{base[0], base[1]};
                }
                const uint32_t i1 = (ib + 1u) * FW_R;
                if ((i1 % CK2) == 0) {
                    const uint32_t ckr1 = (r_lo + i1) / CK2;
                    if (ckr1 <= ncr) {
                        uint32_t* rh = arena + rd_off + uint64_t(2u * (ckr1 - 1u)) * mpad;
                        uint4* oh = reinterpret_cast<uint4*>(rh);
                        uint4* of = reinterpret_cast<uint4*>(rh + mpad);
#pragma unroll
                        for (int c = 0; c < FW_C; c += 4) {
                            oh[c / 4] = uint4{Hp[c], Hp[c + 1], Hp[c + 2], Hp[c + 3]};
                            of[c / 4] = uint4{F[c], F[c + 1], F[c + 2], F[c + 3]};
                        }
                        reinterpret_cast<int2*>(arena + rb_off)[uint64_t(ckr1 - 1u) * (mpad / 16u)] = int2{base[0], base[1]};
                    }
                }
            }
            {
                const uint32_t q4[FW_R] = {nxq.x, nxq.y, nxq.z, nxq.w};
#pragma unroll
                for (int rr = 0; rr < FW_R; ++rr) qc[rr] = from_left_or(qc[rr], q4[rr]);
            }
        };
        {
            uint32_t s = 0;
            for (; s + 1u < nsteps; s += 2) {
                step(s, std::true_type{});
                step(s + 1u, std::false_type{});
            }
            for (; s < nsteps; ++s) step(s, std::true_type{});
        }
#pragma unroll
        for (int h = 0; h < 2; ++h) {
            if (lastc[h] >= 0) bandbest[par(VP_BEST0 + h) + band] = int2{bc[h], int(bc_i[h])};
            if ((ovf >> h) & 1u) {
                const uint32_t pidh = par(VP_PID0 + h);
                if (pidh != 0xFFFFFFFFu) atomicOr(&ovf_out[pidh], 1u);
            }
        }
        if (lane == 0) {
            unsigned long long cells = 0;
#pragma unroll
            for (int h = 0; h < 2; ++h)
                if (vh[h]) cells += (unsigned long long)(par(VP_RHI0 + h) - r_lo) * (unsigned long long)min(strip_cols, par(VP_M0 + h) - p * strip_cols);
            atomicAdd(cells_done, cells);
        }
        const uint32_t my_flag = uint32_t(__builtin_amdgcn_readfirstlane(int(par(VP_FLAG))));
        asm volatile("s_waitcnt vmcnt(0)" ::: "memory");
        __builtin_amdgcn_fence(__ATOMIC_RELEASE, "agent");
        asm volatile("s_waitcnt vmcnt(0)" ::: "memory");
        __hip_atomic_store(&flags[my_flag], 1u, __ATOMIC_RELAXED, __HIP_MEMORY_SCOPE_AGENT);
        it = v2_dequeue(queue);
    }
}

#define V2_FWD_ARGS                                                                                                                        \
    const AlnPairDev *__restrict__ pairs, const V2Couple *__restrict__ couples, const V2Item *__restrict__ items, uint32_t n_items,        \
        uint32_t *__restrict__ queue, uint32_t *__restrict__ flags, uint32_t *__restrict__ err, const uint8_t *__restrict__ pool, AlnParams P, \
        uint32_t *__restrict__ arena, int2 *__restrict__ lrow, int2 *__restrict__ bandbest, uint32_t *__restrict__ ovf_out, int guard,     \
        const uint4 *__restrict__ prof, unsigned long long *__restrict__ cells_done, uint32_t *__restrict__ prog, uint32_t prog_every
__global__ void __launch_bounds__(64 * V2_WAVES) __attribute__((amdgpu_waves_per_eu(3, 8))) k_fwd2(V2_FWD_ARGS)
{
    v2_fwd_body(pairs, couples, items, n_items, queue, flags, err, pool, P, arena, lrow, bandbest, ovf_out, guard, prof, cells_done, prog, prog_every);
}
__global__ void __launch_bounds__(64 * V2_WAVES) __attribute__((amdgpu_waves_per_eu(2, 2))) k_fwd2_w2(V2_FWD_ARGS)
{
    v2_fwd_body(pairs, couples, items, n_items, queue, flags, err, pool, P, arena, lrow, bandbest, ovf_out, guard, prof, cells_done, prog, prog_every);
}


struct V2PairEnd {
    uint32_t lrow0, best0, nbands, couple;
    int32_t cert;
};
constexpr uint32_t V2_RESUME_WORDS = 16;
constexpr uint32_t V2_SPLIT_WORDS = 16;

__global__ void __launch_bounds__(64)
k_fwd2_probe(const AlnPairDev* __restrict__ pairs, V2Couple* __restrict__ couples, V2PairEnd* __restrict__ pe, const uint32_t* __restrict__ arena, AlnParams P)
{
    V2Couple& cp = couples[blockIdx.x];
    if (!cp.corridor) return;
    const uint32_t lane = threadIdx.x;
    const uint32_t strip_cols = 64u * FW_C;
    const uint32_t R = uint32_t(cp.bstart[cp.probe_band + 1u]) * uint32_t(CK2);
    const uint32_t ckr = R / uint32_t(CK2) - 1u;
    const uint32_t* rh = arena + cp.rdat + uint64_t(2u * ckr) * cp.mpad;
    const int2* rb = reinterpret_cast<const int2*>(arena + cp.rbase) + uint64_t(ckr) * (cp.mpad / 16u);
    bool wrong = false;
    uint32_t nmax = 0, mmax = 0, need = 0, need_raw = 0;
    for (int h = 0; h < 2; ++h) {
        if (cp.pid[h] == 0xFFFFFFFFu) continue;
        const AlnPairDev pr = pairs[cp.pid[h]];
        nmax = max(nmax, pr.n);
        mmax = max(mmax, pr.m);
        const int gd = pr.gap_open - P.gap_extend;
        int mx = INT32_MIN;
        const uint32_t x0 = uint32_t(cp.probe_strip) * strip_cols, x1 = min(pr.m, x0 + strip_cols);
        for (uint32_t x = x0 + lane; x < x1; x += 64) {
            const int2 bb = rb[x / 16u];
            mx = max(mx, v2_half(rh[x], h) + (h ? bb.y : bb.x) + gd - P.gap_extend * int(R + x + 1u));
        }
        for (int o = 32; o > 0; o >>= 1) mx = max(mx, __shfl_xor(mx, o));
        if (pr.n < R || x1 <= x0 || mx < P.match * int(R) / 4) {
            wrong = true;
        } else {
            const float len = float(max(pr.n, pr.m)), rate = float(mx) / float(R);
            const float b = len - 0.97f * rate * float(min(pr.n, pr.m)) / float(P.match) + 512.0f;
            need = max(need, uint32_t(max(b, 0.0f)));
            need_raw = max(need_raw, uint32_t(max(len - rate * float(min(pr.n, pr.m)) / float(P.match), 0.0f)));
        }
    }
    const uint32_t len_max = max(nmax, mmax);
    const uint32_t B0 = cp.b0;
    if (!wrong && need_raw > B0 && need > B0) {
        if (float(need) > 0.4f * float(len_max)) {
            wrong = true;
        } else if (lane == 0) {
            long long beff = 0x7FFFFFFFFFFFll;
            uint32_t skipped = 0;
            for (uint32_t b = 0; b < cp.nbands; ++b) {
                const uint32_t r0 = uint32_t(cp.bstart[b]) * uint32_t(CK2), r1 = min(nmax, uint32_t(cp.bstart[b + 1u]) * uint32_t(CK2));
                const uint32_t c_lo = r0 > need ? r0 - need : 0u;
                const unsigned long long c_hi = min((unsigned long long)mmax, (unsigned long long)r1 + need);
                const uint32_t lo = c_lo / strip_cols, hi = uint32_t((max(c_hi, 1ull) - 1ull) / strip_cols);
                cp.plo[b] = uint16_t(min(lo, uint32_t(cp.plo[b])));
                cp.phi[b] = uint16_t(max(hi, uint32_t(cp.phi[b])));
                skipped += uint32_t(cp.plo[b]) + (cp.nstrips - 1u - uint32_t(cp.phi[b]));
                if (cp.plo[b] > 0) beff = min(beff, (long long)r0 - (long long)cp.plo[b] * strip_cols);
                if ((unsigned long long)(uint32_t(cp.phi[b]) + 1u) * strip_cols < mmax) beff = min(beff, (long long)(uint32_t(cp.phi[b]) + 1u) * strip_cols - (long long)r1);
            }
            for (int h = 0; h < 2; ++h)
                if (cp.pid[h] != 0xFFFFFFFFu) {
                    const AlnPairDev pr = pairs[cp.pid[h]];
                    const long long ct = (long long)P.match * max(0ll, (long long)max(pr.n, pr.m) - beff - 1ll);
                    pe[cp.pid[h]].cert = beff == 0x7FFFFFFFFFFFll ? INT32_MIN : int32_t(min(ct, 0x7FFFFFFFll));
                }
            if (skipped * 5u < cp.nbands * cp.nstrips) cp.corridor = 2u;
        }
    }
    __builtin_amdgcn_fence(__ATOMIC_RELEASE, "workgroup");
    __builtin_amdgcn_wave_barrier();
    if ((wrong || __hip_atomic_load(&cp.corridor, __ATOMIC_RELAXED, __HIP_MEMORY_SCOPE_WORKGROUP) == 2u) && lane == 0) {
        for (uint32_t b = 0; b < uint32_t(V2_MAX_BANDS); ++b) {
            cp.plo[b] = 0;
            cp.phi[b] = uint16_t(min(65535u, cp.nstrips - 1u));
        }
        cp.corridor = 0;
        for (int h = 0; h < 2; ++h)
            if (cp.pid[h] != 0xFFFFFFFFu) pe[cp.pid[h]].cert = INT32_MIN;
    }
}

__global__ void __launch_bounds__(64)
k_fwd2_ends(const AlnPairDev* __restrict__ pairs, const V2Couple* __restrict__ couples, const uint32_t* __restrict__ order, uint32_t count, const V2PairEnd* __restrict__ pe,
            const int2* __restrict__ lrow, const int2* __restrict__ bandbest, const uint32_t* __restrict__ ovf, int4* __restrict__ ends,
            uint32_t* __restrict__ resume, uint32_t* __restrict__ early, const int route_below, const uint32_t route_cap)
{
    const uint32_t pslot = blockIdx.x;
    if (pslot >= count) return;
    const uint32_t pid = order[pslot], lane = threadIdx.x;
    const AlnPairDev pr = pairs[pid];
    const V2PairEnd e = pe[pid];
    const uint32_t n = pr.n, m = pr.m;
    const uint32_t nstrips = (m + 64u * FW_C - 1) / (64u * FW_C);
    int br = 0;
    uint32_t bj = 0;
    for (uint32_t x = lane; x < nstrips * 64u; x += 64) {
        if (uint64_t(x) * FW_C >= m) continue;
        const int2 v = lrow[e.lrow0 + x];
        if (v.x > br || (v.x == br && uint32_t(v.y) < bj)) {
            br = v.x;
            bj = uint32_t(v.y);
        }
    }
    for (int o = 32; o > 0; o >>= 1) {
        const int s = __shfl_xor(br, o);
        const uint32_t j = __shfl_xor(bj, o);
        if (s > br || (s == br && j < bj)) {
            br = s;
            bj = j;
        }
    }
    if (lane == 0) {
        int fin = ALN_NEG;
        uint32_t bi = 0, bjj = m;
        for (uint32_t b = 0; b < e.nbands; ++b) {
            if (uint64_t(couples[e.couple].bstart[b]) * CK2 >= n) break;
            const int2 bb = bandbest[e.best0 + b];
            if (bb.x > fin) {
                fin = bb.x;
                bi = uint32_t(bb.y);
            }
        }
        if (br > fin) {
            fin = br;
            bi = n;
            bjj = bj;
        }
        const bool refuted = e.cert != INT32_MIN && fin <= e.cert;
        ends[pid] = int4{fin, int(bi), int(bjj), int(ovf[pid] & 1u) | (refuted ? 2 : 0)};
        if (route_below > 0 && pr.stop_at && !(ovf[pid] & 1u) && !refuted && min(n, m) >= 8u * uint32_t(CK2) &&
            (fin < route_below * int(min(n, m)) / 4 || count <= route_cap)) {
            const uint32_t slot = atomicAdd(&early[0], 1u);
            if (slot < route_cap) {
                resume[size_t(pid) * V2_RESUME_WORDS + 6] = 2u;
                early[1u + slot] = pslot;
            }
        }
    }
}

struct V2Scratch {
    int2 frow[CK2 / TILE][CK2 + 8];
    int2 fcol[CK2 / TILE][CK2];
};

__device__ __forceinline__ int2 v2_ld(const int2* p)
{
    const int x = __hip_atomic_load(&p->x, __ATOMIC_RELAXED, __HIP_MEMORY_SCOPE_AGENT);
    const int y = __hip_atomic_load(&p->y, __ATOMIC_RELAXED, __HIP_MEMORY_SCOPE_AGENT);
    return int2{x, y};
}

constexpr uint32_t V2_NROLE = 5, V2_NHELP = 2 * V2_NROLE, V2_HBUF = 2, V2_HWAVES = 1 + V2_NHELP;
enum V2Help : uint32_t { VH_SEQ = 0, VH_RB, VH_CB, VH_I, VH_J, VH_QUIT, VH_WORK = 8 , VH_SLOT = VH_WORK + 3 * V2_NHELP ,
                         VH_COUNT = VH_SLOT + 3 * V2_NHELP * V2_HBUF };

template <bool HELP, bool EMIT>
__device__ __forceinline__ void trace2_body(const AlnPairDev* __restrict__ pairs, const uint32_t* __restrict__ order, const uint8_t* __restrict__ pool,
                                            const AlnParams& P, const uint32_t* __restrict__ arena, const V2Couple* __restrict__ couples, const V2PairCk* __restrict__ pck,
                                            const int4* __restrict__ ends, V2Scratch* __restrict__ scratch, V2Scratch* __restrict__ hscratch,
                                            uint32_t* __restrict__ resume, uint32_t* __restrict__ park, uint32_t* __restrict__ split,
                                            int32_t* __restrict__ out_score, uint32_t* __restrict__ out_count, const uint32_t count, const uint32_t max_blocks,
                                            const unsigned long long max_cycles, const uint32_t pslot, const uint32_t wv, const uint32_t want,
                                            const typename OpsOut<EMIT>::Dev od)
{
    constexpr int NW = HELP ? int(V2_HWAVES) : TR_WAVES, NDIRS = HELP ? 1 : TR_WAVES;
    constexpr uint32_t B_LEFT = uint32_t(CK2) * 8u, B_Q = uint32_t(CK2) * 4u, B_PROF = 5u * 64u * uint32_t(V2_BLK_C / 4) * 4u;
    constexpr uint32_t D_BYTES = uint32_t(TILE) * uint32_t(TR_C) / 4u * 64u * 2u;
    constexpr uint32_t U_BYTES = (B_LEFT + B_Q + B_PROF) > D_BYTES + uint32_t(TILE) ? (B_LEFT + B_Q + B_PROF) : D_BYTES + uint32_t(TILE);
    __shared__ __attribute__((aligned(16))) uint8_t s_union_all[NW][U_BYTES];
    __shared__ __attribute__((aligned(16))) uint8_t s_tile_all[NDIRS][uint32_t(TILE) * 12u];
    __shared__ uint32_t s_help[VH_COUNT];
    if (pslot >= count) return;
    uint16_t(*dirs)[64] = reinterpret_cast<uint16_t(*)[64]>(&s_union_all[wv][0]);
    int2* const b_left = reinterpret_cast<int2*>(&s_union_all[wv][0]);
    uint32_t* const b_q = reinterpret_cast<uint32_t*>(&s_union_all[wv][B_LEFT]);
    uint32_t* const b_prof = reinterpret_cast<uint32_t*>(&s_union_all[wv][B_LEFT + B_Q]);
    struct TRec {
        int hq, e;
        uint32_t q;
    };
    static_assert(sizeof(TRec) == 12, "a row's record");
    TRec* const s_rec = reinterpret_cast<TRec*>(&s_tile_all[HELP ? 0u : wv][0]);
    uint8_t* const s_rb = &s_union_all[wv][D_BYTES];
    const uint32_t pid = order[pslot];
    const AlnPairDev pr = pairs[pid];
    const V2PairCk ck = pck[pid];
    const int hf = int(ck.half);
    const bool corridor = __builtin_amdgcn_readfirstlane(int(couples[ck.couple].corridor)) != 0;
    uint32_t* const rs = resume + size_t(pid) * V2_RESUME_WORDS;
    {
        const uint32_t fl = uint32_t(__builtin_amdgcn_readfirstlane(int(rs[6])));
        if (HELP ? fl != want : fl == 2u) return;
    }
    V2Scratch* scp = &scratch[pslot];
    const unsigned long long t_begin = __builtin_amdgcn_s_memtime();
    uint32_t n_blocks = 0, n_diag = 0, n_tiles = 0, n_gapsteps = 0;
    unsigned long long t_blk = 0, t_tile = 0, t_walk = 0;
    uint32_t n_thin_c = 0, n_thin_r = 0, n_bsteps = 0, n_bsteps_thin = 0, n_tsteps = 0;
    uint32_t* const sp = split + size_t(pid) * V2_SPLIT_WORDS + (HELP ? V2_SPLIT_WORDS / 2u : 0u);
    auto split_out = [&]() {
        sp[0] = uint32_t(t_blk >> 8);
        sp[1] = uint32_t(t_tile >> 8);
        sp[2] = uint32_t(t_walk >> 8);
        sp[3] = n_thin_c | (n_thin_r << 16);
        sp[4] = n_bsteps;
        sp[5] = n_bsteps_thin;
        sp[6] = n_tsteps;
    };
    const uint32_t n = pr.n, m = pr.m;
    const int go = pr.gap_open, il = pr.ilimit;
    const uint8_t* __restrict__ q = pool + pr.q_off;
    const uint8_t* __restrict__ r = pool + pr.r_off;
    const uint32_t lane = threadIdx.x & 63u;
    const uint32_t k = P.k, kmask = k >= 32 ? 0xFFFFFFFFu : ((1u << k) - 1u);
    const int4 en = ends[pid];
    if (en.w & 3) {
        if (lane == 0) {
            out_score[pid] = (en.w & 1) ? INT32_MIN : INT32_MIN + 1;
            out_count[pid] = 0xFFFFFFFFu;
            OpsOut<EMIT>{}.none(od, pid);
        }
        return;
    }
    const int gd = go - P.gap_extend, ge = P.gap_extend;
    FwdConst K;
    K.ge = ge;
    K.gd = gd;
    K.cm = P.match + 2 * ge + gd;
    K.cx = P.mismatch + 2 * ge + gd;
    uint32_t i = uint32_t(en.y), j = uint32_t(en.z);
    int state = 0;
    WinStat ws;
    OpsOut<EMIT> ops;
    ops.begin(od, pid, n + m);
    if (!EMIT && HELP && want == 1u) {
        i = rs[0];
        j = rs[1];
        state = int(rs[2]);
        ws.wb = rs[3];
        ws.pushed = rs[4];
        ws.cnt = rs[5];
    } else {
        ws.blanks((m - j) + (n - i), kmask, k, il);
        ops.fill('d', m - j, lane);
        ops.fill('i', n - i, lane);
    }
    uint32_t blk_r = 0xFFFFFFFFu, blk_c = 0xFFFFFFFFu;
    auto coarse_row = [&](uint32_t R, uint32_t x) {
        const uint32_t ckr = R / CK2 - 1u;
        const uint32_t* rh = arena + ck.rdat + uint64_t(2u * ckr) * ck.mpad;
        const int2 bb = reinterpret_cast<const int2*>(arena + ck.rbase)[uint64_t(ckr) * (ck.mpad / 16u) + x / 16u];
        const int bs = hf ? bb.y : bb.x;
        return int2{v2_half(rh[x], hf) + bs, v2_half(rh[ck.mpad + x], hf) + bs};
    };
    auto coarse_col = [&](uint32_t C, uint32_t y) {
        const uint64_t e = uint64_t(C / CK2 - 1u) * ck.nq + y / 4u;
        const uint32_t* d = arena + ck.cdat + e * 8u;
        const int2 bb = reinterpret_cast<const int2*>(arena + ck.cbase)[e];
        const int bs = hf ? bb.y : bb.x;
        return int2{v2_half(d[y & 3u], hf) + bs, v2_half(d[4u + (y & 3u)], hf) + bs};
    };

    auto recompute_block_c = [&](auto cpl, const uint32_t Rb, const uint32_t Cb, const uint32_t brows, const uint32_t bcols, V2Scratch& dst) __attribute__((always_inline)) {
        constexpr int BC = decltype(cpl)::value;
        const uint32_t ln = opaque(lane);
        bool top_ok = true, left_ok = true, corner_ok = true;
        if (corridor) {
            const V2Couple& cq = couples[ck.couple];
            auto band_of = [&](uint32_t row) {
                const uint32_t cr = row / uint32_t(CK2);
                uint32_t b = 0;
                while (b + 1u < cq.nbands && uint32_t(cq.bstart[b + 1u]) <= cr) ++b;
                return b;
            };
            auto in = [&](uint32_t b, uint32_t p) { return p >= cq.plo[b] && p <= cq.phi[b]; };
            const uint32_t ps = Cb / (64u * FW_C), pl = Cb ? (Cb - 1u) / (64u * FW_C) : 0u;
            const uint32_t bb = band_of(Rb), bt = Rb ? band_of(Rb - 1u) : 0u;
            if (Rb) top_ok = in(bt, ps);
            if (Cb) left_ok = in(bb, pl);
            if (Rb && Cb) corner_ok = in(bt, pl);
        }
        for (uint32_t x = ln; x <= bcols; x += 64) {
            int2 v;
            if (Rb == 0)
                v = int2{ge * int(Cb + x) - gd, ALN_NEG};
            else if (Cb + x == 0)
                v = int2{ge * int(Rb) - gd, ALN_NEG};
            else if (x ? top_ok : corner_ok)
                v = coarse_row(Rb, Cb + x - 1u);
            else
                v = int2{ALN_NEG, ALN_NEG};
            dst.frow[0][x] = v;
        }
        for (uint32_t y = ln; y < brows; y += 64) {
            int2 v{ge * int(Rb + y + 1) - gd, ALN_NEG};
            if (Cb) v = left_ok ? coarse_col(Cb, Rb + y) : int2{ALN_NEG, ALN_NEG};
            dst.fcol[0][y] = v;
// ... 496 lines not shown
```

Before: 63050.

## Merge runs of consecutive bands into one aligner work item with per-band flag publishing

The v2 wavefront aligner now groups up to a run of consecutive bands (default 4) of a strip into a single work item instead of one item per band-strip tile. Within a run, the kernel waits on the left neighbour's flags and publishes each band's completion flag mid-run, so downstream tiles can still start early. The goal is to cut per-item dequeue, setup and flag overhead and to keep the DP state in registers across band boundaries. The cost is longer serial items and less available parallelism, plus an extra memset of lrow when runs are used. It also adds a host-side plan checker and env overrides for band count and per-CU occupancy.

Result: slower. 55050 (-12.7%).

```diff
diff --git a/include/isonclust2_hip.h b/include/isonclust2_hip.h
--- a/include/isonclust2_hip.h
+++ b/include/isonclust2_hip.h
@@ -127,6 +127,8 @@
                        int32_t mismatch, int32_t gap_open, int32_t gap_extend, char* ops, int32_t ops_cap,
                        int32_t* score_out);
 int64_t ioc_host_ops_to_cigar(const char* ops, int64_t len, char* out, int64_t cap);
+int ioc_host_align_plan_check(int32_t n_pairs, const int32_t* qlen, const int32_t* rlen, double corridor, int32_t want_bands,
+                              int32_t run, int32_t widen, int64_t* out);
 int32_t ioc_host_gap_open(double e1_plus_e2);
 double ioc_host_aln_ratio(const char* comp, int32_t comp_len, double e, uint32_t slen, uint32_t k);
 
diff --git a/isonclust2_amd/_lib.py b/isonclust2_amd/_lib.py
--- a/isonclust2_amd/_lib.py
+++ b/isonclust2_amd/_lib.py
@@ -119,6 +119,7 @@
     "ioc_dist_unique_id", "ioc_dist_init", "ioc_dist_shutdown", "ioc_dist_info", "ioc_dist_allgather_device",
     "ioc_dist_allgatherv_device", "ioc_dist_allgather_i64", "ioc_dist_allgatherv_host", "ioc_dist_allreduce_max",
     "ioc_dist_barrier", "ioc_dist_merge", "ioc_set_shard", "ioc_shard_exchanges", "ioc_shard_aligned_pairs", "ioc_dist_exchange", "ioc_dist_set_shard", "ioc_align_set_verdict_threshold",
+    "ioc_host_align_plan_check",
 ]
 
 _lib = None
@@ -233,5 +234,7 @@
     L.ioc_dist_exchange.argtypes = [vp, vp, i64, i32]
     L.ioc_dist_set_shard.argtypes = [vp, i32]
     L.ioc_align_set_verdict_threshold.argtypes = [vp, C.c_double]
+    if hasattr(L, "ioc_host_align_plan_check"):
+        L.ioc_host_align_plan_check.argtypes = [i32, pi32, pi32, C.c_double, i32, i32, i32, pi64]
     _lib = L
     return L
diff --git a/isonclust2_amd/csrc/ioc_align_gpu.hip b/isonclust2_amd/csrc/ioc_align_gpu.hip
--- a/isonclust2_amd/csrc/ioc_align_gpu.hip
+++ b/isonclust2_amd/csrc/ioc_align_gpu.hip
@@ -1069,6 +1069,7 @@
 
 
 constexpr int P16_GUARD = 28000;
+constexpr uint32_t V2_RUN_DEFAULT = 4;
 
 struct CorridorModel {
     const ioc_ctx* c;
@@ -1111,6 +1112,7 @@
     const uint32_t waves = uint32_t(occ) * uint32_t(n_cu) * uint32_t(V2_WAVES);
     uint32_t want = std::max(12u, std::min(uint32_t(V2_MAX_BANDS), (waves + ncouples - 1u) / std::max(1u, ncouples)));
     if (few_limit && ncouples <= few_limit) want = std::min(want, 17u);
+    if (const char* e = getenv("IOC_ALIGN_V2_BANDS")) want = uint32_t(std::max(1, std::min(int(V2_MAX_BANDS), atoi(e))));
     return want;
 }
 
@@ -1126,6 +1128,7 @@
     uint64_t arena_words = 0, prof_total = 0;
     std::vector<std::vector<V2Item>> items;
     std::vector<uint32_t> n_probe;
+    std::vector<uint32_t> run;
     uint32_t max_items = 0, max_flags = 0, max_pairs = 0;
 };
 
@@ -1302,12 +1305,22 @@
     }
 }
 
-void tile_lists(V2Plan& pl)
+bool corridor_monotone(const V2Couple& cp)
+{
+    for (uint32_t b = 0; b + 1u < cp.nbands; ++b)
+        if (cp.plo[b] > cp.plo[b + 1u] || cp.phi[b] > cp.phi[b + 1u]) return false;
+    return true;
+}
+
+void tile_lists(V2Plan& pl, uint32_t run, uint32_t few_limit)
 {
     pl.items.resize(pl.slices.size());
     pl.n_probe.assign(pl.slices.size(), 0);
+    pl.run.assign(pl.slices.size(), 1u);
     for (size_t si = 0; si < pl.slices.size(); ++si) {
         const uint32_t k_lo = pl.slices[si].first, k_hi = pl.slices[si].first + pl.slices[si].second;
+        const uint32_t G = pl.slices[si].second <= few_limit ? 1u : std::max(1u, std::min(run, uint32_t(V2_MAX_BANDS)));
+        pl.run[si] = G;
         uint32_t nf = 0;
         auto& it = pl.items[si];
         uint32_t maxdiag = 0;
@@ -1335,9 +1348,10 @@
         for (uint32_t dg = 0; dg <= maxdiag; ++dg)
             for (uint32_t k2 = k_lo; k2 < k_hi; ++k2) {
                 const V2Couple& cp = pl.cps[k2];
-                if (dg > cp.nbands + cp.nstrips - 2u) continue;
-                const uint32_t b_lo = dg >= cp.nstrips ? dg - cp.nstrips + 1u : 0u, b_hi = std::min(dg, cp.nbands - 1u);
-                for (uint32_t b = b_lo; b <= b_hi; ++b) it.push_back(V2Item{k2, uint16_t(b), uint16_t(dg - b)});
+                const uint32_t nsb = (cp.nbands + G - 1u) / G;
+                if (dg > nsb + cp.nstrips - 2u) continue;
+                const uint32_t b_lo = dg >= cp.nstrips ? dg - cp.nstrips + 1u : 0u, b_hi = std::min(dg, nsb - 1u);
+                for (uint32_t b = b_lo; b <= b_hi; ++b) it.push_back(V2Item{k2, uint16_t(b * G), uint16_t(dg - b)});
             }
         pl.max_items = std::max<uint32_t>(pl.max_items, uint32_t(it.size()));
         pl.max_flags = std::max(pl.max_flags, nf);
@@ -1345,9 +1359,81 @@
     }
 }
 
+int plan_check(const int32_t* n, const int32_t* m, int32_t n_pairs, double corridor, uint32_t want_bands, uint32_t run, bool widen, int64_t* out)
+{
+    V2Plan pl;
+    std::vector<AlnPairDev> dp(static_cast<size_t>(n_pairs));
+    std::vector<uint32_t> order(static_cast<size_t>(n_pairs));
+    for (int32_t i = 0; i < n_pairs; ++i) {
+        if (n[i] <= 0 || m[i] <= 0) return IOC_ERR_ARG;
+        dp[size_t(i)] = AlnPairDev{};
+        dp[size_t(i)].n = uint32_t(n[i]);
+        dp[size_t(i)].m = uint32_t(m[i]);
+        dp[size_t(i)].gap_open = 3;
+        order[size_t(i)] = uint32_t(i);
+    }
+    pl.cnt = pl.np = uint32_t(n_pairs);
+    pl.ncouples = (pl.cnt + 1u) / 2u;
+    CorridorModel cm{nullptr, AlnParams{}, std::max(0.0, std::min(1.0, corridor)), true, false};
+    cm.P.match = 2;
+    cm.P.mismatch = -2;
+    cm.P.gap_extend = 1;
+    plan_couples(pl, dp, order.data(), cm, want_bands ? want_bands : 17u);
+    slice_couples(pl, ~uint64_t(0) >> 2, {});
+    tile_lists(pl, run, 0u);
+    out[0] = out[1] = out[2] = out[3] = 0;
+    for (const V2Couple& cp : pl.cps)
+        if (!corridor_monotone(cp)) return IOC_ERR_STATE;
+    for (size_t si = 0; si < pl.slices.size(); ++si) {
+        const auto& it = pl.items[si];
+        std::vector<uint8_t> flag(pl.max_flags, 0), held(pl.max_flags, 0);
+        for (uint32_t x = 0; x < pl.n_probe[si]; ++x) {
+            const V2Couple& cp = pl.cps[it[x].couple];
+            const uint32_t f = cp.flag0 + uint32_t(it[x].band) * cp.nstrips + it[x].strip;
+            if (it[x].strip < cp.plo[it[x].band] || it[x].strip > cp.phi[it[x].band]) ++out[1];
+            ++held[f];
+            flag[f] = 1;
+        }
+        if (widen)
+            for (uint32_t k2 = pl.slices[si].first; k2 < pl.slices[si].first + pl.slices[si].second; ++k2)
+                for (uint32_t b = 0; b < uint32_t(V2_MAX_BANDS); ++b) {
+                    pl.cps[k2].plo[b] = 0;
+                    pl.cps[k2].phi[b] = uint16_t(std::min(65535u, pl.cps[k2].nstrips - 1u));
+                }
+        for (size_t x = pl.n_probe[si]; x < it.size(); ++x) {
+            const V2Couple& cp = pl.cps[it[x].couple];
+            const uint32_t p = it[x].strip;
+            auto in = [&](uint32_t b, uint32_t q) { return q >= cp.plo[b] && q <= cp.phi[b]; };
+            auto at = [&](uint32_t b, uint32_t q) { return cp.flag0 + b * cp.nstrips + q; };
+            uint32_t first = 0, last = 0;
+            if (!v2_clip(cp.plo, cp.phi, cp.nbands, uint32_t(it[x].band), pl.run[si], p, [&](uint32_t b) { return flag[at(b, p)] != 0; }, first, last)) continue;
+            ++out[3];
+            bool early = first > 0 && in(first - 1u, p) && !flag[at(first - 1u, p)];
+            for (uint32_t b = first; b <= last; ++b) {
+                if (!in(b, p)) ++out[1];
+                if (p > 0 && in(b, p - 1u) && !flag[at(b, p - 1u)]) early = true;
+                ++held[at(b, p)];
+            }
+            for (uint32_t b = first; b <= last; ++b) flag[at(b, p)] = 1;
+            if (early) ++out[2];
+        }
+        for (uint32_t k2 = pl.slices[si].first; k2 < pl.slices[si].first + pl.slices[si].second; ++k2) {
+            const V2Couple& cp = pl.cps[k2];
+            for (uint32_t b = 0; b < cp.nbands; ++b)
+                for (uint32_t q = 0; q < cp.nstrips; ++q) {
+                    const uint32_t h = held[cp.flag0 + b * cp.nstrips + q];
+                    const bool inside = q >= cp.plo[b] && q <= cp.phi[b];
+                    if (inside ? h != 1u : h != 0u) ++out[inside ? 0 : 1];
+                }
+        }
+    }
+    return IOC_OK;
+}
+
 struct V2Opts {
     int n_cu, occ, guard;
     uint32_t few_limit;
+    uint32_t run;
     uint32_t deadline;
     unsigned long long deadline_cycles;
     uint32_t help_wgs;
@@ -1410,6 +1496,7 @@
 uint32_t v2_per_cu(const V2Plan& pl, size_t si, const V2Opts& o, bool few_couples)
 {
     if (few_couples) return uint32_t(o.occ);
+    if (const char* e = getenv("IOC_ALIGN_V2_PER_CU")) return uint32_t(std::max(1, std::min(o.occ, atoi(e))));
     uint64_t tiles = 0;
     uint32_t diags = 1;
     for (uint32_t k2 = pl.slices[si].first; k2 < pl.slices[si].first + pl.slices[si].second; ++k2) {
@@ -1439,21 +1526,21 @@
     ACHK(c, hipGetLastError());
     ACHK(c, hipMemsetAsync(d_ctl, 0, t.ctl_words * 4, s));
     ACHK(c, hipMemsetAsync(t.resume, 0, t.resume_words * 4, s));
-    if (pl.tiles_skipped)
+    if (pl.tiles_skipped || pl.run[si] > 1u)
         ACHK(c, hipMemsetAsync(t.lrow, 0x80, (size_t(pl.lrow_total) + pl.best_total) * sizeof(int2), s));
     if (getenv("IOC_ALIGN_V2_FAKE_TIMEOUT")) {
         const uint32_t one = 1;
         ACHK(c, hipMemcpyAsync(d_ctl + 1, &one, 4, hipMemcpyHostToDevice, s));
     }
     ACHK(c, hipEventRecord(ev[0], s));
-    auto fwd = [&](decltype(&k_fwd2) kernel, uint32_t n_wg, const V2Item* items, uint32_t n) {
+    auto fwd = [&](decltype(&k_fwd2) kernel, uint32_t n_wg, const V2Item* items, uint32_t n, uint32_t run) {
         hipLaunchKernelGGL(kernel, dim3(n_wg), dim3(64 * V2_WAVES), 0, s, d_pairs, t.cps, items, n, d_ctl, d_ctl + 16, d_ctl + 1, d_pool, P,
                            static_cast<uint32_t*>(c->a_ck.p), t.lrow, t.best, d_ctl + 16 + 2 * pl.max_flags, o.guard, static_cast<const uint4*>(c->a_prof.p),
                            reinterpret_cast<unsigned long long*>(d_ctl + t.ctl_words - 2), few_couples ? d_ctl + 16 + pl.max_flags : static_cast<uint32_t*>(nullptr),
-                           prog_every);
+                           prog_every, run);
     };
     if (n_probe) {
-        fwd(k_fwd2, std::max(1u, std::min(uint32_t(o.occ) * uint32_t(o.n_cu), (n_probe + V2_WAVES - 1) / V2_WAVES)), t.items, n_probe);
+        fwd(k_fwd2, std::max(1u, std::min(uint32_t(o.occ) * uint32_t(o.n_cu), (n_probe + V2_WAVES - 1) / V2_WAVES)), t.items, n_probe, 1u);
         ACHK(c, hipGetLastError());
         hipLaunchKernelGGL(k_fwd2_probe, dim3(n_couples), dim3(64), 0, s, d_pairs, t.cps + k_first, t.pend, static_cast<const uint32_t*>(c->a_ck.p), P);
         ACHK(c, hipGetLastError());
@@ -1461,7 +1548,7 @@
     }
     const uint32_t n_main = n_items - n_probe, per_cu = v2_per_cu(pl, si, o, few_couples);
     const uint32_t n_wg = std::max(1u, std::min(per_cu * uint32_t(o.n_cu), (n_main + V2_WAVES - 1) / V2_WAVES));
-    fwd((per_cu <= 2 && !getenv("IOC_ALIGN_V2_NO_W2")) ? k_fwd2_w2 : k_fwd2, n_wg, t.items + n_probe, n_main);
+    fwd((per_cu <= 2 && !getenv("IOC_ALIGN_V2_NO_W2")) ? k_fwd2_w2 : k_fwd2, n_wg, t.items + n_probe, n_main, pl.run[si]);
     ACHK(c, hipGetLastError());
     const uint32_t n_help = std::min<uint32_t>(n_pairs, o.help_wgs);
     hipLaunchKernelGGL(k_fwd2_ends, dim3(n_pairs), dim3(64), 0, s, d_pairs, t.cps, d_order + first_pair, n_pairs, t.pend, t.lrow, t.best,
@@ -1654,7 +1741,11 @@
         fprintf(stderr, "[ioc]   aligner v2: %u couples, checkpoint arena %.1f MB (%zu slice(s)) reserved in %.3f ms; corridor: %llu of %llu tiles skipped\n", pl.ncouples,
                 double(pl.arena_words) * 4e-6, pl.slices.size(), std::chrono::duration<double, std::milli>(std::chrono::steady_clock::now() - t_res0).count(),
                 (unsigned long long)pl.tiles_skipped, (unsigned long long)pl.tiles_all);
-    tile_lists(pl);
+    o.run = V2_RUN_DEFAULT;
+    if (const char* e = getenv("IOC_ALIGN_V2_RUN")) o.run = atoi(e) <= 0 ? uint32_t(V2_MAX_BANDS) : uint32_t(atoi(e));
+    for (const V2Couple& cp : pl.cps)
+        if (!corridor_monotone(cp)) return ioc_fail(c, IOC_ERR_STATE, "aligner v2: a corridor that narrows and widens again");
+    tile_lists(pl, o.run, o.few_limit);
 
     o.deadline = 4;
     if (const char* e = getenv("IOC_TRACE2_DEADLINE")) o.deadline = uint32_t(std::max(0, atoi(e)));
@@ -2287,6 +2378,13 @@
     return IOC_OK;
 }
 
+int ioc_host_align_plan_check(int32_t n_pairs, const int32_t* qlen, const int32_t* rlen, double corridor, int32_t want_bands, int32_t run,
+                              int32_t widen, int64_t* out)
+{
+    if (n_pairs <= 0 || !qlen || !rlen || !out || want_bands < 0) return IOC_ERR_ARG;
+    return plan_check(qlen, rlen, n_pairs, corridor, uint32_t(want_bands), run <= 0 ? uint32_t(V2_MAX_BANDS) : uint32_t(run), widen != 0, out);
+}
+
 int ioc_align_pairs(ioc_ctx* c, int32_t n_pairs, const ioc_aln_pair* pairs, int32_t k, int32_t match, int32_t mismatch,
                     int32_t gap_extend, int32_t* out_score, int64_t* out_windows, double* out_ratio)
 {
diff --git a/isonclust2_amd/csrc/ioc_align_v2.inc b/isonclust2_amd/csrc/ioc_align_v2.inc
--- a/isonclust2_amd/csrc/ioc_align_v2.inc
+++ b/isonclust2_amd/csrc/ioc_align_v2.inc
@@ -31,6 +31,20 @@
     uint16_t band, strip;
 };
 
+template <class Done>
+__host__ __device__ inline bool v2_clip(const uint16_t* plo, const uint16_t* phi, uint32_t nbands, uint32_t band0, uint32_t G, uint32_t p, Done done,
+                                        uint32_t& first, uint32_t& last)
+{
+    const uint32_t end = band0 + G < nbands ? band0 + G : nbands;
+    uint32_t b = band0;
+    while (b < end && (p < plo[b] || p > phi[b] || done(b))) ++b;
+    if (b >= end) return false;
+    first = b;
+    while (b + 1u < end && p >= plo[b + 1u] && p <= phi[b + 1u]) ++b;
+    last = b;
+    return true;
+}
+
 struct V2PairCk {
     uint64_t rdat, rbase, cdat, cbase;
     uint32_t mpad, nq, half, couple;
@@ -134,8 +148,10 @@
 enum V2Par : uint32_t {
     VP_N0 = 0, VP_N1, VP_M0, VP_M1, VP_GD0, VP_GD1, VP_LROW0, VP_LROW1, VP_BEST0, VP_BEST1, VP_PID0, VP_PID1,
     VP_RDAT_LO, VP_RDAT_HI, VP_RBASE_LO, VP_RBASE_HI, VP_CDAT_LO, VP_CDAT_HI, VP_CBASE_LO, VP_CBASE_HI,
-    VP_MPAD, VP_NQ, VP_FLAG, VP_BAND, VP_STRIP, VP_COLIN_LO, VP_COLIN_HI, VP_RHI0, VP_RHI1, VP_COUNT = 32
+    VP_MPAD, VP_NQ, VP_FLAG, VP_BAND, VP_STRIP, VP_COLIN_LO, VP_COLIN_HI, VP_RHI0, VP_RHI1,
+    VP_NSTRIPS, VP_RUN_N, VP_LEFT_END, VP_RUN_JW, VP_RUN_JP, VP_RUN_END0, VP_COUNT = VP_RUN_END0 + V2_MAX_BANDS
 };
+constexpr uint32_t V2_NEVER = 0xFFFFFFFFu;
 
 __global__ void __launch_bounds__(128)
 k_fwd2_prof(const AlnPairDev* __restrict__ pairs, const V2Couple* __restrict__ couples, const uint8_t* __restrict__ pool, AlnParams P, uint4* __restrict__ prof)
@@ -180,7 +196,7 @@
 v2_fwd_body(const AlnPairDev* __restrict__ pairs, const V2Couple* __restrict__ couples, const V2Item* __restrict__ items, uint32_t n_items,
        uint32_t* __restrict__ queue, uint32_t* __restrict__ flags, uint32_t* __restrict__ err, const uint8_t* __restrict__ pool, AlnParams P,
        uint32_t* __restrict__ arena, int2* __restrict__ lrow, int2* __restrict__ bandbest, uint32_t* __restrict__ ovf_out, int guard,
-       const uint4* __restrict__ prof, unsigned long long* __restrict__ cells_done, uint32_t* __restrict__ prog, uint32_t prog_every)
+       const uint4* __restrict__ prof, unsigned long long* __restrict__ cells_done, uint32_t* __restrict__ prog, uint32_t prog_every, uint32_t run_bands)
 {
     __shared__ __attribute__((aligned(16))) uint32_t s_look_all[V2_WAVES][3][128];
     __shared__ __attribute__((aligned(16))) uint32_t s_prof_all[V2_WAVES][2][5][64][4];
@@ -201,8 +217,9 @@
     uint32_t it = v2_dequeue(queue);
     while (it < n_items) {
         uint32_t band, p, r_lo, nblk[2];
+        uint32_t wait_blk = V2_NEVER;
+        uint32_t pub_step = V2_NEVER;
         bool vh[2], last_band[2];
-        bool left_ok = true;
         bool top_none = false;
         bool left_rows = false;
         uint32_t left_idx = 0, nblk_band = 0, left_avail = 0;
@@ -219,16 +236,24 @@
         {
             const V2Item item = items[it];
             const V2Couple cp = couples[item.couple];
-            band = item.band;
+            const V2Couple* const gc = &couples[item.couple];
             p = item.strip;
-            if (p < cp.plo[band] || p > cp.phi[band] ||
-                __builtin_amdgcn_readfirstlane(int(__hip_atomic_load(&flags[cp.flag0 + band * cp.nstrips + p], __ATOMIC_RELAXED, __HIP_MEMORY_SCOPE_AGENT))) != 0) {
-                it = v2_dequeue(queue);
-                continue;
-            }
+            uint32_t b_last = 0;
+            {
+                auto done = [&](uint32_t b) {
+                    return __builtin_amdgcn_readfirstlane(int(__hip_atomic_load(&flags[cp.flag0 + b * cp.nstrips + p], __ATOMIC_RELAXED, __HIP_MEMORY_SCOPE_AGENT))) != 0;
+                };
+                band = 0;
+                if (!v2_clip(gc->plo, gc->phi, cp.nbands, uint32_t(item.band), prog != nullptr ? 1u : run_bands, p, done, band, b_last)) {
+                    it = v2_dequeue(queue);
+                    continue;
+                }
+                band = uint32_t(__builtin_amdgcn_readfirstlane(int(band)));
+                b_last = uint32_t(__builtin_amdgcn_readfirstlane(int(b_last)));
+            }
+            const uint32_t run_n = b_last - band + 1u;
             const bool top_in = band > 0 && p >= cp.plo[band - 1u] && p <= cp.phi[band - 1u];
             const bool left_in = p > cp.plo[band];
-            left_ok = p == 0 || left_in;
             top_none = band > 0 && !top_in;
             const bool corner_in = band > 0 && p > 0 && p - 1u >= cp.plo[band - 1u] && p - 1u <= cp.phi[band - 1u];
             if (top_in) (void)v2_wait(&flags[cp.flag0 + (band - 1u) * cp.nstrips + p], err);
@@ -244,6 +269,18 @@
             if (left_rows) (void)v2_wait_rows(&prog[left_idx], &flags[left_idx], min(32u, nblk_band), err, left_avail);
             __builtin_amdgcn_fence(__ATOMIC_ACQUIRE, "agent");
             r_lo = uint32_t(cp.bstart[band]) * uint32_t(CK2);
+            const uint32_t r_end = uint32_t(gc->bstart[b_last + 1u]) * uint32_t(CK2);
+            uint32_t left_end = V2_NEVER;
+            if (p > 0) {
+                uint32_t jl = band;
+                while (jl <= b_last && p > uint32_t(gc->plo[jl])) ++jl;
+                left_end = uint32_t(gc->bstart[jl]) * uint32_t(CK2);
+            }
+            if (run_n > 1u) {
+                const uint32_t e0 = uint32_t(gc->bstart[band + 1u]) * uint32_t(CK2);
+                pub_step = (e0 - r_lo) / uint32_t(FW_R) + 62u;
+                if (e0 < left_end && p > 0) wait_blk = (e0 - r_lo) / 64u;
+            }
             const uint32_t jb = p * strip_cols + lane * FW_C;
             uint32_t n[2], m[2], r_hi[2];
             int gd[2];
@@ -255,7 +292,7 @@
                 m[h] = have ? pr.m : 0u;
                 q[h] = pool + pr.q_off;
                 gd[h] = pr.gap_open - ge;
-                r_hi[h] = min(n[h], uint32_t(cp.bstart[band + 1u]) * uint32_t(CK2));
+                r_hi[h] = min(n[h], r_end);
                 nblk[h] = r_hi[h] > r_lo ? (r_hi[h] - r_lo + FW_R - 1) / FW_R : 0u;
                 const uint32_t nstr = (m[h] + strip_cols - 1) / strip_cols;
                 vh[h] = have && p < nstr && nblk[h] > 0;
@@ -307,7 +344,13 @@
                 s_par[VP_COLIN_HI] = uint32_t(colin >> 32);
                 s_par[VP_RHI0] = r_hi[0];
                 s_par[VP_RHI1] = r_hi[1];
-            }
+                s_par[VP_NSTRIPS] = cp.nstrips;
+                s_par[VP_RUN_N] = run_n;
+                s_par[VP_LEFT_END] = left_end;
+                s_par[VP_RUN_JW] = 0;
+                s_par[VP_RUN_JP] = 0;
+            }
+            if (lane < run_n) s_par[VP_RUN_END0 + lane] = (uint32_t(gc->bstart[band + lane + 1u]) * uint32_t(CK2) - r_lo) / 64u;
             int Ha[2][FW_C], Fa[2][FW_C], dga[2];
 #pragma unroll
             for (int h = 0; h < 2; ++h) {
@@ -403,9 +446,9 @@
         }
         const uint8_t* profA = reinterpret_cast<const uint8_t*>(&s_prof_all[wv][0][0][lane][0]);
         const uint8_t* profB = reinterpret_cast<const uint8_t*>(&s_prof_all[wv][1][0][lane][0]);
-        auto left_edge = [&](int h, uint32_t row) {
+        auto left_edge = [&](int h, uint32_t row, bool lok) {
             int2 v{ge * int(row + 1) - int(par(VP_GD0 + h)), ALN_NEG};
-            if (!left_ok) v = int2{ALN_NEG, ALN_NEG};
+            if (!lok) v = int2{ALN_NEG, ALN_NEG};
             else if (vh[h] && p > 0 && row < par(VP_RHI0 + h)) {
                 const uint64_t e = par64(VP_COLIN_LO) + row / 4u;
                 const uint32_t* d = arena + par64(VP_CDAT_LO) + e * 8u;
@@ -432,11 +475,12 @@
         };
         auto fetch = [&](uint32_t blk) {
             const uint32_t row = r_lo + blk * 64u + lane;
+            const bool lok = r_lo + blk * 64u < uint32_t(__builtin_amdgcn_readfirstlane(int(par(VP_LEFT_END))));
             uint32_t qq[2];
 #pragma unroll
             for (int h = 0; h < 2; ++h) {
                 qq[h] = qcode((vh[h] && row < par(VP_RHI0 + h)) ? q[h][row] : 0u);
-                en[h] = left_edge(h, row);
+                en[h] = left_edge(h, row, lok);
             }
             qn = qq[0] | (qq[1] << 16);
         };
@@ -485,7 +529,7 @@
                             const int hi_v = v2_half(mx, h) - U16_BIAS, lo_v = v2_half(mn, h) - U16_BIAS;
                             if ((lanef >> h & 1u) && bi >= (top_none ? 1 : 0) && uint32_t(bi) < nblk[h] && (hi_v > guard || lo_v < -guard)) {
 #ifdef IOC_V2_GUARD_DEBUG
-                                if (!(ovf >> h & 1u)) printf("guard: item %u band %u strip %u half %d lane %u step %u hi %d lo %d left_ok %d base %d\n", it, band, p, h, lane, s, hi_v, lo_v, int(left_ok), base[h]);
+                                if (!(ovf >> h & 1u)) printf("guard: item %u band %u strip %u half %d lane %u step %u hi %d lo %d base %d\n", it, band, p, h, lane, s, hi_v, lo_v, base[h]);
 #endif
                                 ovf |= 1u << h;
                             }
@@ -522,6 +566,17 @@
                         (void)v2_wait_rows(&prog[left_idx], &flags[left_idx], need_rows, err, left_avail);
                         __builtin_amdgcn_fence(__ATOMIC_ACQUIRE, "agent");
                     }
+                }
+                if (blk + 1u == wait_blk) {
+                    const uint32_t j = uint32_t(__builtin_amdgcn_readfirstlane(int(par(VP_RUN_JW)))) + 1u;
+                    const uint32_t fl = uint32_t(__builtin_amdgcn_readfirstlane(int(par(VP_FLAG) + j * par(VP_NSTRIPS)))) - 1u;
+                    (void)v2_wait(&flags[fl], err);
+                    __builtin_amdgcn_fence(__ATOMIC_ACQUIRE, "agent");
+                    v2_lds_store(par_addr + 4u * VP_RUN_JW, j);
+                    const uint32_t e = uint32_t(__builtin_amdgcn_readfirstlane(int(par(VP_RUN_END0 + j))));
+                    const bool more = j + 1u < uint32_t(__builtin_amdgcn_readfirstlane(int(par(VP_RUN_N)))) &&
+                                      r_lo + e * 64u < uint32_t(__builtin_amdgcn_readfirstlane(int(par(VP_LEFT_END))));
+                    wait_blk = more ? e : V2_NEVER;
                 }
                 fetch(blk + 1u);
             }
@@ -623,6 +678,17 @@
 #pragma unroll
                 for (int rr = 0; rr < FW_R; ++rr) qc[rr] = from_left_or(qc[rr], q4[rr]);
             }
+            if (decltype(first)::value && s == pub_step) {
+                const uint32_t j = uint32_t(__builtin_amdgcn_readfirstlane(int(par(VP_RUN_JP))));
+                const uint32_t fl = uint32_t(__builtin_amdgcn_readfirstlane(int(par(VP_FLAG) + j * par(VP_NSTRIPS))));
+                asm volatile("s_waitcnt vmcnt(0)" ::: "memory");
+                __builtin_amdgcn_fence(__ATOMIC_RELEASE, "agent");
+                asm volatile("s_waitcnt vmcnt(0)" ::: "memory");
+                __hip_atomic_store(&flags[fl], 1u, __ATOMIC_RELAXED, __HIP_MEMORY_SCOPE_AGENT);
+                v2_lds_store(par_addr + 4u * VP_RUN_JP, j + 1u);
+                const bool more = j + 2u < uint32_t(__builtin_amdgcn_readfirstlane(int(par(VP_RUN_N))));
+                pub_step = more ? uint32_t(__builtin_amdgcn_readfirstlane(int(par(VP_RUN_END0 + j + 1u)))) * (64u / uint32_t(FW_R)) + 62u : V2_NEVER;
+            }
         };
         {
             uint32_t s = 0;
@@ -647,7 +713,7 @@
                 if (vh[h]) cells += (unsigned long long)(par(VP_RHI0 + h) - r_lo) * (unsigned long long)min(strip_cols, par(VP_M0 + h) - p * strip_cols);
             atomicAdd(cells_done, cells);
         }
-        const uint32_t my_flag = uint32_t(__builtin_amdgcn_readfirstlane(int(par(VP_FLAG))));
+        const uint32_t my_flag = uint32_t(__builtin_amdgcn_readfirstlane(int(par(VP_FLAG) + (par(VP_RUN_N) - 1u) * par(VP_NSTRIPS))));
         asm volatile("s_waitcnt vmcnt(0)" ::: "memory");
         __builtin_amdgcn_fence(__ATOMIC_RELEASE, "agent");
         asm volatile("s_waitcnt vmcnt(0)" ::: "memory");
@@ -660,14 +726,15 @@
     const AlnPairDev *__restrict__ pairs, const V2Couple *__restrict__ couples, const V2Item *__restrict__ items, uint32_t n_items,        \
         uint32_t *__restrict__ queue, uint32_t *__restrict__ flags, uint32_t *__restrict__ err, const uint8_t *__restrict__ pool, AlnParams P, \
         uint32_t *__restrict__ arena, int2 *__restrict__ lrow, int2 *__restrict__ bandbest, uint32_t *__restrict__ ovf_out, int guard,     \
-        const uint4 *__restrict__ prof, unsigned long long *__restrict__ cells_done, uint32_t *__restrict__ prog, uint32_t prog_every
+        const uint4 *__restrict__ prof, unsigned long long *__restrict__ cells_done, uint32_t *__restrict__ prog, uint32_t prog_every, \
+        uint32_t run_bands
 __global__ void __launch_bounds__(64 * V2_WAVES) __attribute__((amdgpu_waves_per_eu(3, 8))) k_fwd2(V2_FWD_ARGS)
 {
-    v2_fwd_body(pairs, couples, items, n_items, queue, flags, err, pool, P, arena, lrow, bandbest, ovf_out, guard, prof, cells_done, prog, prog_every);
+    v2_fwd_body(pairs, couples, items, n_items, queue, flags, err, pool, P, arena, lrow, bandbest, ovf_out, guard, prof, cells_done, prog, prog_every, run_bands);
 }
 __global__ void __launch_bounds__(64 * V2_WAVES) __attribute__((amdgpu_waves_per_eu(2, 2))) k_fwd2_w2(V2_FWD_ARGS)
 {
-    v2_fwd_body(pairs, couples, items, n_items, queue, flags, err, pool, P, arena, lrow, bandbest, ovf_out, guard, prof, cells_done, prog, prog_every);
+    v2_fwd_body(pairs, couples, items, n_items, queue, flags, err, pool, P, arena, lrow, bandbest, ovf_out, guard, prof, cells_done, prog, prog_every, run_bands);
 }
 
 
```
